# jhoobergs/Thesis-pbrt-v3

Measured on AMD Instinct MI355X. Metric: Mrays/s, higher is better.
Workload: dtype f32; 1 GPU; Sponza-class atrium STAND-IN (311,728 tris, matte+plastic, point light; the reference ships no Sponza geometry) 700x700, halton 1024 spp, path maxdepth 5, bvh; spp_total=1024, tiles=16x16 round-robin over 1 GPU(s), parallelism=tile-dp1, film_merge=none (single GPU)

## Files before the change

### thesis-pbrt-v3_amd/__init__.py

```python
import ctypes as C
import os

import numpy as np

_HERE = os.path.dirname(os.path.abspath(__file__))
LIB_PATH = os.environ.get("HPRT_LIB") or os.path.join(_HERE, "lib", "libhprt.so")


class HprtError(RuntimeError):
    def __init__(self, code, msg):
        super().__init__("hprt error %d: %s" % (code, msg))
        self.code = code


E_INVALID, E_IO, E_PARSE, E_NO_DEVICE, E_DEVICE, E_UNSUPPORTED = -1, -2, -3, -4, -5, -6
RENDER_COUNT_WORK = 1
RENDER_PIXEL_STATS = 2
RENDER_COUNT_TRACED = 4
RENDER_TRACE_ALL = 8
RENDER_EXPORT_FOREIGN = 16
ACCEL_BVH, ACCEL_KDTREE, ACCEL_RBSP = 0, 1, 2
ACCEL_BSP = ACCEL_RBSP
KD_MAX_DEPTH = 64
RBSP_MAX_DEPTH = 64
# ... 247 lines not shown
        "hprt_scene_reserve": (C.c_int, [vp, P(RenderDesc)]),
        "hprt_film_records_read": (C.c_int, [vp, vp, sz, P(sz)]),
        "hprt_film_records_merge": (C.c_int, [vp, sz, vp, sz]),
        "hprt_model_accelerator": (C.c_int, [vp, vp, sz]),
        "hprt_kdtree_build": (C.c_int, [vp, P(vp)]),
        "hprt_kdtree_build_from_bounds": (C.c_int, [sz, vp, vp, C.c_int, C.c_int, C.c_float, C.c_int, C.c_int, P(vp)]),
        "hprt_kdtree_info": (C.c_int, [vp, P(u32)]),
        "hprt_kdtree_copy": (C.c_int, [vp, vp, vp]),
        "hprt_kdtree_destroy": (None, [vp]),
        "hprt_scene_attach_kdtree": (C.c_int, [vp, vp]),
        "hprt_kdinst_build": (C.c_int, [vp, P(vp)]),
        "hprt_kdinst_info": (C.c_int, [vp, P(u32)]),
        "hprt_kdinst_object_info": (C.c_int, [vp, u32, P(u32)]),
        "hprt_kdinst_copy": (C.c_int, [vp, vp, vp]),
        "hprt_kdinst_object_copy": (C.c_int, [vp, u32, vp, vp]),
        "hprt_kdinst_destroy": (None, [vp]),
        "hprt_scene_attach_kdinst": (C.c_int, [vp, vp]),
        "hprt_write_pixel_stats_accel": (C.c_int, [cp, vp, C.c_int, C.c_int, C.c_int]),
        "hprt_rbsp_build": (C.c_int, [vp, vp, P(vp)]),
        "hprt_rbsp_build_from_triangles": (C.c_int, [sz, vp, vp, P(vp)]),
        "hprt_rbsp_info": (C.c_int, [vp, P(u32)]),
        "hprt_rbsp_copy": (C.c_int, [vp, vp, vp, vp]),
        "hprt_rbsp_destroy": (None, [vp]),
        "hprt_scene_attach_rbsp": (C.c_int, [vp, vp]),
        "hprt_rbspkd_build": (C.c_int, [vp, vp, P(vp)]),
        "hprt_rbspkd_build_from_triangles": (C.c_int, [sz, vp, vp, P(vp)]),
        "hprt_rbspkd_info": (C.c_int, [vp, P(u32)]),
        "hprt_rbspkd_copy": (C.c_int, [vp, vp, vp, vp]),
        "hprt_rbspkd_destroy": (None, [vp]),
        "hprt_scene_attach_rbspkd": (C.c_int, [vp, vp]),
        "hprt_rbspinst_build": (C.c_int, [vp, vp, P(vp)]),
        "hprt_rbspkdinst_build": (C.c_int, [vp, vp, P(vp)]),
        "hprt_rbspinst_info": (C.c_int, [vp, P(u32)]),
        "hprt_rbspinst_object_info": (C.c_int, [vp, u32, P(u32)]),
        "hprt_rbspinst_copy": (C.c_int, [vp, vp, vp, vp]),
        "hprt_rbspinst_object_copy": (C.c_int, [vp, u32, vp, vp]),
        "hprt_rbspinst_destroy": (None, [vp]),
        "hprt_scene_attach_rbspinst": (C.c_int, [vp, vp]),
        "hprt_rbsp_build_device": (C.c_int, [vp, vp, vp, vp, P(vp)]),
        "hprt_rbsp_build_from_triangles_device": (C.c_int, [sz, vp, vp, vp, vp, P(vp)]),
        "hprt_rbspkd_build_device": (C.c_int, [vp, vp, vp, vp, P(vp)]),
        "hprt_rbspkd_build_from_triangles_device": (C.c_int, [sz, vp, vp, vp, vp, P(vp)]),
        "hprt_bsppaper_build_device": (C.c_int, [vp, vp, vp, vp, P(vp)]),
        "hprt_bsppaper_build_from_triangles_device": (C.c_int, [sz, vp, vp, vp, vp, P(vp)]),
        "hprt_bsppaperkd_build_device": (C.c_int, [vp, vp, vp, vp, P(vp)]),
        "hprt_bsppaperkd_build_from_triangles_device": (C.c_int, [sz, vp, vp, vp, vp, P(vp)]),
        "hprt_bsppaper_build": (C.c_int, [vp, vp, P(vp)]),
        "hprt_bsppaper_build_from_triangles": (C.c_int, [sz, vp, vp, P(vp)]),
        "hprt_bsppaper_info": (C.c_int, [vp, P(u32)]),
        "hprt_bsppaper_copy": (C.c_int, [vp, vp, vp]),
        "hprt_bsppaper_destroy": (None, [vp]),
        "hprt_scene_attach_bsppaper": (C.c_int, [vp, vp]),
        "hprt_bsppaperkd_build": (C.c_int, [vp, vp, P(vp)]),
        "hprt_bsppaperkd_build_from_triangles": (C.c_int, [sz, vp, vp, P(vp)]),
        "hprt_bsppaperkd_info": (C.c_int, [vp, P(u32)]),
        "hprt_bsppaperkd_copy": (C.c_int, [vp, vp, vp]),
        "hprt_bsppaperkd_destroy": (None, [vp]),
        "hprt_scene_attach_bsppaperkd": (C.c_int, [vp, vp]),
        "hprt_bsppaperinst_build": (C.c_int, [vp, vp, P(vp)]),
        "hprt_bsppaperkdinst_build": (C.c_int, [vp, vp, P(vp)]),
        "hprt_bsppaperinst_info": (C.c_int, [vp, P(u32)]),
        "hprt_bsppaperinst_object_info": (C.c_int, [vp, u32, P(u32)]),
        "hprt_bsppaperinst_copy": (C.c_int, [vp, vp, vp]),
        "hprt_bsppaperinst_object_copy": (C.c_int, [vp, u32, vp, vp]),
        "hprt_bsppaperinst_destroy": (None, [vp]),
        "hprt_scene_attach_bsppaperinst": (C.c_int, [vp, vp]),
        "hprt_bspnode_build": (C.c_int, [vp, vp, P(vp)]),
        "hprt_bspnode_build_from_triangles": (C.c_int, [sz, vp, vp, P(vp)]),
        "hprt_bspnodekd_build": (C.c_int, [vp, vp, P(vp)]),
        "hprt_bspnodekd_build_from_triangles": (C.c_int, [sz, vp, vp, P(vp)]),
        "hprt_bspnode_build_device": (C.c_int, [vp, vp, vp, vp, P(vp)]),
        "hprt_bspnode_build_from_triangles_device": (C.c_int, [sz, vp, vp, vp, vp, P(vp)]),
        "hprt_bspnodekd_build_device": (C.c_int, [vp, vp, vp, vp, P(vp)]),
        "hprt_bspnodekd_build_from_triangles_device": (C.c_int, [sz, vp, vp, vp, vp, P(vp)]),
        "hprt_scene_kd_counters": (C.c_int, [vp, vp]),
        "hprt_pixel_kd_stats_read": (C.c_int, [vp, vp, sz]),
        "hprt_write_pixel_stats_rbspkd": (C.c_int, [cp, vp, vp, C.c_int, C.c_int]),
    }
    debug = {}
    for prefix in ("kdinst", "rbspinst", "bsppaperinst"):
        debug["hprt_debug_%s_bounds" % prefix] = (C.c_int, [vp, C.c_int, vp])
        debug["hprt_debug_%s_set_tree" % prefix] = (C.c_int, [vp, C.c_int, sz, vp, sz, vp, vp])
    debug["hprt_debug_halton_index"] = (C.c_int, [P(RenderOptions), sz, vp, vp, vp, vp, vp, vp])
    for name, (res, args) in list(sig.items()) + list(debug.items()):
        fn = getattr(lib, name)
        fn.restype = res
        fn.argtypes = args
    return lib, sorted(sig)


lib, EXPORTS = _load()


def _check(rc):
    if rc != 0:
        raise HprtError(rc, lib.hprt_last_error().decode("utf-8", "replace"))


def _ptr(a):
    return None if a is None else a.ctypes.data_as(C.c_void_p)


def version():
    return lib.hprt_version().decode()


_probe_lib = None


def _probe():
    global _probe_lib
    if _probe_lib is None:
        path = os.path.join(os.path.dirname(LIB_PATH), "libhprt_probe.so")
        if not os.path.exists(path):
            raise ImportError("hprt: %s is missing — run `python thesis-pbrt-v3_amd/build.py`" % path)
        p = C.CDLL(path)
        p.hprt_debug_device_halton.restype = C.c_int
        p.hprt_debug_device_halton.argtypes = [C.c_void_p, C.c_int, C.c_int, C.c_int, C.c_int, C.c_size_t, C.c_void_p, C.c_void_p, C.c_void_p]
        _probe_lib = p
    return _probe_lib


def debug_halton_index(opt, px, py, sample):
    px = np.ascontiguousarray(px, np.int32); py = np.ascontiguousarray(py, np.int32); sample = np.ascontiguousarray(sample, np.int64)
    a = np.zeros(px.shape[0], np.uint64); b = np.zeros(px.shape[0], np.uint64); bounds = np.zeros(4, np.int32)
    _check(lib.hprt_debug_halton_index(C.byref(opt), px.shape[0], _ptr(px), _ptr(py), _ptr(sample), _ptr(a), _ptr(b), _ptr(bounds)))
    return a, b, tuple(int(v) for v in bounds)


class Model:

    def __init__(self, handle):
        self._h = handle

    @staticmethod
    def parse(path, subst=None):
        kv = []
        for k, v in (subst or {}).items():
            kv += [k.encode(), v.encode()]
        arr = (C.c_char_p * max(1, len(kv)))(*kv)
        h = C.c_void_p()
        _check(lib.hprt_model_parse(path.encode(), arr, len(kv) // 2, C.byref(h)))
        return Model(h)

    @staticmethod
    def load(path):
        h = C.c_void_p()
        _check(lib.hprt_model_load(path.encode(), C.byref(h)))
        return Model(h)

    def save(self, path, compact=False):
        _check((lib.hprt_model_save_compact if compact else lib.hprt_model_save)(self._h, path.encode()))

    @property
    def options(self):
        o = RenderOptions()
        _check(lib.hprt_model_get_options(self._h, C.byref(o)))
        return o

    @options.setter
    def options(self, o):
        _check(lib.hprt_model_set_options(self._h, C.byref(o)))

    def counts(self):
        c = (C.c_uint64 * 7)()
        _check(lib.hprt_model_counts(self._h, c))
        return dict(zip(("shapes", "primitives", "triangles", "spheres", "materials", "lights", "textures"), [int(x) for x in c]))

    def texture(self, index):
        info = (C.c_int32 * 5)(); ma = C.c_float()
        _check(lib.hprt_model_texture_info(self._h, index, info, C.byref(ma)))
        levels = []
        for k in range(info[0]):
            wh = (C.c_int32 * 2)()
            _check(lib.hprt_model_texture_level(self._h, index, k, wh, None))
            a = np.zeros((wh[1], wh[0], 3), np.float32)
            _check(lib.hprt_model_texture_level(self._h, index, k, wh, _ptr(a)))
            levels.append(a)
        return {"levels": info[0], "trilinear": bool(info[1]), "wrap": info[2], "max_anisotropy": ma.value}, levels

    @property
    def accelerator(self):
        buf = C.create_string_buffer(256)
        _check(lib.hprt_model_accelerator(self._h, buf, 256))
        return buf.value.decode()

    def warnings(self):
        w = lib.hprt_model_warnings(self._h).decode()
        return [x for x in w.split("\n") if x]

    def __del__(self):
        if getattr(self, "_h", None) and lib is not None:
            lib.hprt_model_destroy(self._h)
            self._h = None


class Bvh:

    def __init__(self, model=None, handle=None):
        if handle is None:
            handle = C.c_void_p()
            _check(lib.hprt_bvh_build(model._h, C.byref(handle)))
        self._h = handle
# ... 387 lines not shown
    return (BspNodeKd if fastkd else BspNode)(model, accelerator, **kw), ("attach_bsppaperkd" if fastkd else "attach_bsppaper")


class Scene:

    def __init__(self, model, bvh, device=-1):
        h = C.c_void_p()
        _check(lib.hprt_scene_create_from_model(model._h, bvh._h, device, C.byref(h)))
        self._h = h
        self._model = model

    @staticmethod
    def from_desc(desc, device=-1):
        h = C.c_void_p()
        _check(lib.hprt_scene_create(C.byref(desc), device, C.byref(h)))
        sc = Scene.__new__(Scene)
        sc._h = h
        sc._model = None
        return sc

    def attach_kdtree(self, kdtree):
        _check(lib.hprt_scene_attach_kdtree(self._h, kdtree._h))
        self._kdtree = kdtree

    def attach_kdinst(self, kdinst):
        _check(lib.hprt_scene_attach_kdinst(self._h, kdinst._h))
        self._kdinst = kdinst

    def attach_rbspinst(self, rbspinst):
        _check(lib.hprt_scene_attach_rbspinst(self._h, rbspinst._h))
        self._rbspinst = rbspinst

    def attach_bsppaperinst(self, bsppaperinst):
        _check(lib.hprt_scene_attach_bsppaperinst(self._h, bsppaperinst._h))
        self._bsppaperinst = bsppaperinst

    def attach_rbsp(self, rbsp):
        _check(lib.hprt_scene_attach_rbsp(self._h, rbsp._h))
        self._rbsp = rbsp

    def attach_rbspkd(self, rbspkd):
        _check(lib.hprt_scene_attach_rbspkd(self._h, rbspkd._h))
        self._rbspkd = rbspkd

    def attach_bsppaper(self, bsppaper):
        _check(lib.hprt_scene_attach_bsppaper(self._h, bsppaper._h))
        self._bsppaper = bsppaper

    def attach_bsppaperkd(self, bsppaperkd):
        _check(lib.hprt_scene_attach_bsppaperkd(self._h, bsppaperkd._h))
        self._bsppaperkd = bsppaperkd

    def kd_counters(self):
        out = np.zeros(2, np.uint64)
        _check(lib.hprt_scene_kd_counters(self._h, _ptr(out)))
        return int(out[0]), int(out[1])

    def intersect(self, o, d, tmax, count=False):
        o = np.ascontiguousarray(o, np.float32); d = np.ascontiguousarray(d, np.float32)
        tmax = np.ascontiguousarray(tmax, np.float32)
        n = tmax.shape[0]
        t = np.zeros(n, np.float32); prim = np.zeros(n, np.int32); bary = np.zeros((n, 3), np.float32)
        ctr = np.zeros(4, np.uint64) if count else None
        _check(lib.hprt_intersect(self._h, n, _ptr(o), _ptr(d), _ptr(tmax), _ptr(t), _ptr(prim), _ptr(bary), _ptr(ctr)))
        return (t, prim, bary, ctr) if count else (t, prim, bary)

    def intersect_instanced(self, o, d, tmax, count=False):
        o = np.ascontiguousarray(o, np.float32); d = np.ascontiguousarray(d, np.float32)
        tmax = np.ascontiguousarray(tmax, np.float32)
        n = tmax.shape[0]
        t = np.zeros(n, np.float32); prim = np.zeros(n, np.int32); inst = np.zeros(n, np.int32); bary = np.zeros((n, 3), np.float32)
        ctr = np.zeros(4, np.uint64) if count else None
        _check(lib.hprt_intersect_instanced(self._h, n, _ptr(o), _ptr(d), _ptr(tmax), _ptr(t), _ptr(prim), _ptr(inst), _ptr(bary), _ptr(ctr)))
        return (t, prim, inst, bary, ctr) if count else (t, prim, inst, bary)

    def occluded(self, o, d, tmax, count=False):
        o = np.ascontiguousarray(o, np.float32); d = np.ascontiguousarray(d, np.float32)
        tmax = np.ascontiguousarray(tmax, np.float32)
        n = tmax.shape[0]
        occ = np.zeros(n, np.uint8)
        ctr = np.zeros(4, np.uint64) if count else None
        _check(lib.hprt_occluded(self._h, n, _ptr(o), _ptr(d), _ptr(tmax), _ptr(occ), _ptr(ctr)))
        return (occ, ctr) if count else occ

    def intersect_device(self, n, rays7_ptr, t_ptr, prim_ptr, bary_ptr=None, stream=None):
        _check(lib.hprt_intersect_device(self._h, n, rays7_ptr, t_ptr, prim_ptr, bary_ptr, stream))

    def occluded_device(self, n, rays7_ptr, occ_ptr, stream=None):
        _check(lib.hprt_occluded_device(self._h, n, rays7_ptr, occ_ptr, stream))

    def render(self, opt=None, tile_begin=0, tile_end=0, tile_stride=1, spp_chunk=0, count_work=False, film_ptr=None,
               stream=None, pixel_stats=False, count_traced=False, trace_all=False, export_foreign=False):
        opt = opt or self._model.options
        desc = RenderDesc()
        desc.opt = opt
        desc.tile_begin, desc.tile_end, desc.tile_stride = tile_begin, tile_end, tile_stride
        desc.spp_chunk = spp_chunk
        desc.flags = (RENDER_COUNT_WORK if count_work else 0) | (RENDER_PIXEL_STATS if pixel_stats else 0) | \
                     (RENDER_COUNT_TRACED if count_traced else 0) | (RENDER_TRACE_ALL if trace_all else 0) | \
                     (RENDER_EXPORT_FOREIGN if export_foreign else 0)
        self._film_shape = tuple(int(v) for v in (opt.film_bounds()[3] - opt.film_bounds()[1], opt.film_bounds()[2] - opt.film_bounds()[0]))
        st = RenderStats()
        _check(lib.hprt_render(self._h, C.byref(desc), film_ptr, stream, C.byref(st)))
        film = None
        if film_ptr is None:
            x0, y0, x1, y1 = opt.film_bounds()
            film = np.zeros((y1 - y0, x1 - x0, 4), np.float32)
            _check(lib.hprt_film_read(self._h, _ptr(film), film.shape[0] * film.shape[1]))
        return film, st.as_dict()

    def reserve(self, opt=None, tile_begin=0, tile_end=0, tile_stride=1, spp_chunk=0):
        desc = RenderDesc()
        desc.opt = opt or self._model.options
        desc.tile_begin, desc.tile_end, desc.tile_stride, desc.spp_chunk, desc.flags = tile_begin, tile_end, tile_stride, spp_chunk, 0
        _check(lib.hprt_scene_reserve(self._h, C.byref(desc)))

    def debug_poison(self, byte):
        lib.hprt_debug_poison_workspace.argtypes = [C.c_void_p, C.c_int]
        _check(lib.hprt_debug_poison_workspace(self._h, -1 if byte is None else int(byte)))

    def debug_device_halton(self, bounds_w, bounds_h, index, dim, sample_pixel_center=False, use_lds=False):
        index = np.ascontiguousarray(index, np.uint64); dim = np.ascontiguousarray(dim, np.int32)
        assert index.shape == dim.shape and index.ndim == 1
        out = np.zeros(index.shape[0], np.float32)
        _check(_probe().hprt_debug_device_halton(self._h, int(bounds_w), int(bounds_h), int(bool(sample_pixel_center)), int(bool(use_lds)),
                                                 index.shape[0], _ptr(index), _ptr(dim), _ptr(out)))
        return out

    def film_records(self):
        n = C.c_size_t()
        _check(lib.hprt_film_records_read(self._h, None, 0, C.byref(n)))
        out = np.zeros(n.value, FILM_RECORD)
        if n.value:
            _check(lib.hprt_film_records_read(self._h, _ptr(out), n.value, C.byref(n)))
        return out

    def pixel_stats(self):
        h, w = self._film_shape
        out = np.zeros((h, w, 7), np.uint64)
        _check(lib.hprt_pixel_stats_read(self._h, _ptr(out), h * w))
        return out

    def pixel_kd_stats(self):
        h, w = self._film_shape
        out = np.zeros((2, h, w), np.uint64)
        _check(lib.hprt_pixel_kd_stats_read(self._h, _ptr(out), h * w))
        return out

    def sample_radiance(self, px, py, sample, opt=None):
        opt = opt or self._model.options
        px = np.ascontiguousarray(px, np.int32); py = np.ascontiguousarray(py, np.int32)
        sample = np.ascontiguousarray(sample, np.int64)
        L = np.zeros((px.shape[0], 3), np.float32)
        _check(lib.hprt_sample_radiance(self._h, C.byref(opt), px.shape[0], _ptr(px), _ptr(py), _ptr(sample), _ptr(L)))
        return L

    def __del__(self):
        if getattr(self, "_h", None) and lib is not None:
            lib.hprt_scene_destroy(self._h)
            self._h = None


class Comm:

    @staticmethod
    def unique_id():
# ... 77 lines not shown
```

### thesis-pbrt-v3_amd/build.py

```python
import concurrent.futures
import os
import shutil
import subprocess
import sys

HERE = os.path.dirname(os.path.abspath(__file__))
CSRC = os.path.join(HERE, "csrc")
OBJ = os.path.join(HERE, "build")
LIB = os.path.join(HERE, "lib")
HOST_SRCS = ["pbrt_frontend.cpp", "loop_subdiv.cpp", "scene_io.cpp", "texture_io.cpp", "bvh_builder.cpp", "kdtree_builder.cpp", "rbsp_builder.cpp", "bsppaper_builder.cpp", "bspnode_builder.cpp", "bvhold_builder.cpp", "wide_bvh.cpp", "halton_tables.cpp", "capi_host.cpp"]
HIPCC_HOST_SRCS = ["scene_layout.cpp"]
HIP_SRCS = ["device/kernels.hip", "device/kd_walk.hip", "device/rbsp_walk.hip", "device/rbspkd_walk.hip", "device/bsppaper_walk.hip", "device/bsppaperkd_walk.hip", "device/kdinst_walk.hip", "device/kdop_cost.hip", "device/rbspinst_walk.hip", "device/bsppaperinst_walk.hip", "device/bsp_cost.hip", "device/bspnode_cost.hip", "device/hlbvh_build.hip", "capi_device.hip", "capi_gather.hip"]
CUIDS = {"device/kernels.hip": "a6cd736c50efffab", "device/kd_walk.hip": "5c0d2e7f41b3a916", "device/rbsp_walk.hip": "3e91a5c07d2b84f6",
         "device/rbspkd_walk.hip": "7a4f0c2e9b61d385", "device/bsppaper_walk.hip": "c52e8b1d06f3a794",
         "device/bsppaperkd_walk.hip": "e8136d4a9f07c2b5", "device/kdinst_walk.hip": "4d9b27f1a60c8e53", "device/kdop_cost.hip": "b7e20a5c93d1f468",
         "device/rbspinst_walk.hip": "9f3c61d8b2047ae5", "device/bsppaperinst_walk.hip": "2c7e5a90d4b18f63", "device/bsp_cost.hip": "6b1f94c3e7a0d258",
         "device/bspnode_cost.hip": "d3a7150c8e4f92b6", "device/hlbvh_build.hip": "58e2c9a4f1b7063d",
         "capi_device.hip": "1b24418c11488d5c", "capi_gather.hip": "89501e8167866ce2"}
PROBE_SRCS = ["device/halton_probe.hip"]
CUIDS["device/halton_probe.hip"] = "f04b8d61c2a79e35"
COMMON = ["-O3", "-std=c++17", "-fPIC", "-ffp-contract=off", "-fno-fast-math", "-Wall", "-Wno-unused-function"]


def _hipcc():
    for c in (shutil.which("hipcc"), "/opt/rocm/bin/hipcc"):
        if c and os.path.exists(c):
            return c
    raise RuntimeError("hipcc not found")


def _newer(src_files, out):
    if not os.path.exists(out):
        return True
    t = os.path.getmtime(out)
    return any(os.path.getmtime(f) > t for f in src_files)


def _headers():
    hs = []
    for root, _, files in os.walk(CSRC):
        hs += [os.path.join(root, f) for f in files if f.endswith(".h")]
    hs.append(os.path.join(HERE, "..", "include", "hprt.h"))
    return hs


def build(verbose=False, force=False):
    os.makedirs(OBJ, exist_ok=True)
    os.makedirs(LIB, exist_ok=True)
    hipcc = _hipcc()
    headers = _headers()
    jobs = []
    for s in HOST_SRCS + HIPCC_HOST_SRCS:
        src = os.path.join(CSRC, s)
        obj = os.path.join(OBJ, s.replace("/", "_") + ".o")
        cmd = [hipcc if s in HIPCC_HOST_SRCS else "g++"] + COMMON + ["-c", src, "-o", obj]
        jobs.append((src, obj, cmd))
    for s in HIP_SRCS + PROBE_SRCS:
        src = os.path.join(CSRC, s)
        obj = os.path.join(OBJ, s.replace("/", "_") + ".o")
        cmd = [hipcc, "--offload-arch=gfx950"] + COMMON + ["-Wno-unused-result", "-cuid=" + CUIDS[s], "-c", src, "-o", obj]
        jobs.append((src, obj, cmd))

    def run(job):
        src, obj, cmd = job
        if not force and not _newer([src, os.path.abspath(__file__)] + headers, obj):
            return None
        r = subprocess.run(cmd, capture_output=True, text=True)
        if r.returncode != 0:
            raise RuntimeError("compile failed: %s\n%s\n%s" % (" ".join(cmd), r.stdout, r.stderr))
        return r.stderr

    with concurrent.futures.ThreadPoolExecutor(max_workers=4) as ex:
        for out in ex.map(run, jobs):
            if verbose and out:
                print(out)
    lib = os.path.join(LIB, "libhprt.so")
    probe_objs = [j[1] for j in jobs[len(jobs) - len(PROBE_SRCS):]]
    objs = [j[1] for j in jobs[:len(jobs) - len(PROBE_SRCS)]]
    if force or _newer(objs, lib):
        cmd = [hipcc, "--offload-arch=gfx950", "-shared", "-o", lib] + objs + ["-lz", "-L/opt/rocm/lib", "-lrccl"]
        r = subprocess.run(cmd, capture_output=True, text=True)
        if r.returncode != 0:
            raise RuntimeError("link failed: %s\n%s" % (" ".join(cmd), r.stderr))
    probe = os.path.join(LIB, "libhprt_probe.so")
    if force or _newer(probe_objs + [lib], probe):
        cmd = [hipcc, "--offload-arch=gfx950", "-shared", "-o", probe] + probe_objs + ["-L" + LIB, "-lhprt", "-Wl,-rpath,$ORIGIN"]
        r = subprocess.run(cmd, capture_output=True, text=True)
        if r.returncode != 0:
            raise RuntimeError("link failed: %s\n%s" % (" ".join(cmd), r.stderr))
    return lib


if __name__ == "__main__":
    print(build(verbose="-v" in sys.argv, force="-f" in sys.argv))
```

### thesis-pbrt-v3_amd/csrc/capi_device.hip

```cpp
#include <hip/hip_runtime.h>
#include <algorithm>
#include <cassert>
#include <chrono>
#include <cmath>
#include <cstring>
#include <functional>
#include <map>
#include <memory>
#include <string>
#include <vector>
#include "../../include/hprt.h"
#include "device/kernels.h"
#include "halton_tables.h"
#include "host_transform.h"
#include "hprt_internal.h"
#include "device_state.h"
#include "scene_layout.h"
#include "wide_bvh.h"

using namespace hprt;


namespace {

// ... 59 lines not shown
    cam->dxCamera = xf_point(cam->rasterToCamera, vec3(1, 0, 0)) - xf_point(cam->rasterToCamera, vec3(0, 0, 0));
    cam->dyCamera = xf_point(cam->rasterToCamera, vec3(0, 1, 0)) - xf_point(cam->rasterToCamera, vec3(0, 0, 0));
}

int CheckDepth(int maxDepth) {
    if (5 + 8 * ((int64_t)maxDepth + 1) > 1000)
        return SetError(HPRT_E_UNSUPPORTED, "maxdepth above 123: a path could pass the 1,000 sampler dimensions of the reference's Halton tables");
    return HPRT_OK;
}

struct FrameSetup {
    FilmGeom fg; int ntx, nty; HaltonLayout hal; RenderParams rp;
    std::vector<uint32_t> pixelXY; std::vector<uint64_t> pixelOffset;
    std::vector<int32_t> localIndex;
    int W, H;
    uint64_t offX[128], offY[128];
};
int SetupFrame(const HprtRenderOptions &o, FrameSetup *f) {
    if (o.xres <= 0 || o.yres <= 0 || o.xres > 32768 || o.yres > 32768) return SetError(HPRT_E_INVALID, "film resolution out of range");
    if (o.filter_radius[0] != 0.5f || o.filter_radius[1] != 0.5f)
        return SetError(HPRT_E_UNSUPPORTED, "only the box filter with radius 0.5 is in the hot-path scope (SURVEY.md §2)");
    FilmGeom &fg = f->fg;
    fg.cx0 = (int)std::ceil(o.xres * o.crop[0]); fg.cx1 = (int)std::ceil(o.xres * o.crop[1]);
    fg.cy0 = (int)std::ceil(o.yres * o.crop[2]); fg.cy1 = (int)std::ceil(o.yres * o.crop[3]);
    fg.rx = o.filter_radius[0]; fg.ry = o.filter_radius[1];
    fg.sx0 = (int)std::floor((float)fg.cx0 + 0.5f - fg.rx); fg.sy0 = (int)std::floor((float)fg.cy0 + 0.5f - fg.ry);
    fg.sx1 = (int)std::ceil((float)fg.cx1 - 0.5f + fg.rx); fg.sy1 = (int)std::ceil((float)fg.cy1 - 0.5f + fg.ry);
    fg.maxSampleLuminance = o.max_sample_luminance;
    f->W = fg.cx1 - fg.cx0; f->H = fg.cy1 - fg.cy0;
    if (f->W <= 0 || f->H <= 0) return SetError(HPRT_E_INVALID, "empty crop window");
    f->ntx = (fg.sx1 - fg.sx0 + 15) / 16; f->nty = (fg.sy1 - fg.sy0 + 15) / 16;
    f->hal = MakeHaltonLayout(fg.sx1 - fg.sx0, fg.sy1 - fg.sy0);
    const uint64_t base = (uint64_t)HaltonPixelOffset(f->hal, 0, 0), stride = (uint64_t)std::max(1, f->hal.sampleStride);
    for (int m = 0; m < 128; ++m) {
        f->offX[m] = (uint64_t)HaltonPixelOffset(f->hal, m, 0);
        f->offY[m] = ((uint64_t)HaltonPixelOffset(f->hal, 0, m) + stride - base) % stride;
    }
    return HPRT_OK;
}
uint64_t TilePixelOffset(const FrameSetup &f, int x, int y) {
    const uint64_t stride = (uint64_t)std::max(1, f.hal.sampleStride);
    return f.hal.sampleStride > 1 ? (f.offX[((x % 128) + 128) % 128] + f.offY[((y % 128) + 128) % 128]) % stride : 0ull;
}
void AddTilePixels(FrameSetup *f, int tile) {
    const FilmGeom &fg = f->fg;
    int tx = tile % f->ntx, ty = tile / f->ntx;
    int x0 = fg.sx0 + tx * 16, x1 = std::min(x0 + 16, fg.sx1), y0 = fg.sy0 + ty * 16, y1 = std::min(y0 + 16, fg.sy1);
    for (int y = y0; y < y1; ++y)
        for (int x = x0; x < x1; ++x) {
            f->localIndex[(size_t)(y - fg.cy0) * f->W + (x - fg.cx0)] = (int32_t)f->pixelXY.size();
            f->pixelXY.push_back((uint32_t)x | ((uint32_t)y << 16));
            f->pixelOffset.push_back(TilePixelOffset(*f, x, y));
        }
}

}

extern "C" {

int hprt_scene_create(const HprtSceneDesc *d, int device, HprtScene **out) try {
    if (!d || !out) return SetError(HPRT_E_INVALID, "hprt_scene_create: null argument");
    SceneLayout L;
    if (int rc = BuildSceneLayout(*d, &L)) return rc;
    int dev;
    if (int rc = CheckDevice(device, &dev)) return rc;
    std::unique_ptr<HprtScene> sc(new HprtScene());
    sc->device = dev; sc->nPrims = L.nPrims;
    sc->topOrder = std::move(L.topOrder); sc->objectOrder = std::move(L.objectOrder); sc->objectPrimBase = std::move(L.objectPrimBase);
    sc->instanceObject = std::move(L.instanceObject); sc->instanced = L.instanced; sc->hasSubstrateBin = L.hasSubstrateBin;
    const std::vector<uint16_t> &perms = HaltonPermutations();
    std::vector<int32_t> primes(PrimeTable().begin(), PrimeTable().end()), primeSums(PrimeSumTable().begin(), PrimeSumTable().end());
    std::vector<uint64_t> magic(primes.size());
    for (size_t i = 0; i < primes.size(); ++i) magic[i] = 0xffffffffffffffffull / (uint64_t)primes[i] + 1ull;
    HIP_TRY(upload(sc->nodes, L.pairs)); HIP_TRY(upload(sc->tris, L.tris)); HIP_TRY(upload(sc->primVtx, L.primVtx));
    HIP_TRY(upload(sc->primN, L.primN)); HIP_TRY(upload(sc->vUV, L.vUV)); HIP_TRY(upload(sc->vS, L.vS));
    HIP_TRY(upload(sc->shapes, L.shapes)); HIP_TRY(upload(sc->materials, L.materials)); HIP_TRY(upload(sc->lights, L.lights));
    HIP_TRY(upload(sc->spheres, L.spheres)); HIP_TRY(upload(sc->instances, L.instances)); HIP_TRY(upload(sc->topEntry, L.topEntry));
    HIP_TRY(upload(sc->topEntryWide, L.topEntryWide)); HIP_TRY(upload(sc->lightFunc, L.lightFunc)); HIP_TRY(upload(sc->lightCdf, L.lightCdf));
    HIP_TRY(upload(sc->perms, perms)); HIP_TRY(upload(sc->primes, primes)); HIP_TRY(upload(sc->primeSums, primeSums));
    HIP_TRY(upload(sc->primeMagic, magic));
    HIP_TRY(upload(sc->textures, L.textures)); HIP_TRY(upload(sc->mipLevels, L.mipLevels)); HIP_TRY(upload(sc->texels, L.texels)); HIP_TRY(upload(sc->weightLut, L.weightLut));
    HIP_TRY(upload(sc->wide, L.wide)); HIP_TRY(upload(sc->leafBox, L.leafBox));
    HIP_TRY(upload(sc->envLights, L.envLights)); HIP_TRY(upload(sc->envData, L.envData));
    HIP_TRY(sc->counters.alloc(sizeof(DevCounters)));
    HIP_TRY(hipMemset(sc->counters.p, 0, sizeof(DevCounters)));
    HIP_TRY(sc->deepStack.alloc((size_t)HPRT_SPILL_STACK * HPRT_DEEP_THREADS * sizeof(uint2)));
    HIP_TRY(sc->workCounter.alloc(256));
    DevScene &dv = sc->dev;
    dv.pairs = sc->nodes.as<DevPair>(); dv.nPairs = (uint32_t)L.pairs.size();
    dv.wide = L.wide.empty() ? nullptr : sc->wide.as<DevWide>(); dv.nWide = (uint32_t)L.wide.size(); dv.leafBox = sc->leafBox.as<float4>();
    dv.tris = sc->tris.as<float4>(); dv.nPrims = L.nPrims;
    dv.primVtx = sc->primVtx.as<uint32_t>();
    dv.primN = sc->primN.as<float4>(); dv.vUV = sc->vUV.as<float>(); dv.vS = sc->vS.as<float>();
    dv.shapes = sc->shapes.as<DevShape>(); dv.nShapes = d->n_shapes;
    dv.materials = sc->materials.as<DevMaterial>();
    dv.lights = sc->lights.as<DevLight>(); dv.nLights = d->n_lights;
    dv.spheres = sc->spheres.as<DevSphere>(); dv.nSpheres = (uint32_t)L.spheres.size();
    dv.envLights = sc->envLights.as<DevEnvLight>(); dv.envData = sc->envData.as<float>(); dv.nEnvLights = (uint32_t)L.envLights.size();
    dv.textures = d->n_textures ? sc->textures.as<DevTexture>() : nullptr; dv.mipLevels = sc->mipLevels.as<DevMipLevel>();
    dv.texels = sc->texels.as<float>(); dv.weightLut = sc->weightLut.as<float>();
    dv.instances = sc->instances.as<DevInstance>(); dv.nInstances = d->n_instances;
    dv.topEntry = L.topEntry.empty() ? nullptr : sc->topEntry.as<float4>(); dv.nTopPrims = (uint32_t)L.topEntry.size();
    dv.topEntryWide = L.topEntryWide.empty() ? nullptr : sc->topEntryWide.as<float4>();
    dv.lightFunc = sc->lightFunc.as<float>(); dv.lightCdf = sc->lightCdf.as<float>(); dv.lightFuncInt = L.funcInt;
    dv.deepStack = sc->deepStack.as<uint2>();
    dv.perms = sc->perms.as<uint16_t>(); dv.primes = sc->primes.as<int32_t>(); dv.primeSums = sc->primeSums.as<int32_t>();
    dv.primeMagic = sc->primeMagic.as<uint64_t>();
    dv.worldRadius = L.worldRadius;
    dv.spatial = 0; dv.voxFunc = dv.voxCdf = dv.voxFuncInt = nullptr;
    dv.voxSlot = nullptr; dv.voxRequest = nullptr; dv.voxRequestCount = nullptr;
    for (int a = 0; a < 3; ++a) { dv.voxN[a] = L.voxN[a]; dv.wbMin[a] = L.wbMin[a]; dv.wbMax[a] = L.wbMax[a]; }
    if (L.lightStrategy == 2) {
        const uint64_t nVox = (uint64_t)dv.voxN[0] * (uint64_t)dv.voxN[1] * (uint64_t)dv.voxN[2];
        const uint64_t denseMaxFloats = [] { const char *e = getenv("HPRT_VOXEL_DENSE_MAX_MB"); return e ? (uint64_t)atoll(e) * (1ull << 18) : (1ull << 28); }();
        const uint64_t rowFloats = 2ull * d->n_lights + 2ull;
        const bool dense = nVox * rowFloats <= denseMaxFloats;
        uint64_t rows = nVox;
        if (!dense) {
            const uint64_t poolFloats = [] { const char *e = getenv("HPRT_VOXEL_POOL_MB"); return (e ? (uint64_t)atoll(e) : 4096ull) * (1ull << 18); }();
            rows = std::max<uint64_t>(1, std::min<uint64_t>(nVox, poolFloats / rowFloats));
        }
        HIP_TRY(sc->voxFunc.alloc(rows * d->n_lights * sizeof(float)));
        HIP_TRY(sc->voxCdf.alloc(rows * (d->n_lights + 1ull) * sizeof(float)));
        HIP_TRY(sc->voxFuncInt.alloc(rows * sizeof(float)));
        std::vector<float> ri(5 * 128);
        VoxelSamplePoints(ri.data());
        HIP_TRY(upload(sc->voxRi, ri));
        dv.spatial = 1;
        dv.voxFunc = sc->voxFunc.as<float>(); dv.voxCdf = sc->voxCdf.as<float>(); dv.voxFuncInt = sc->voxFuncInt.as<float>();
        sc->nVoxels = (uint32_t)nVox; sc->voxRows = (uint32_t)rows; sc->voxRowsUsed = 0;
        if (dense) LaunchVoxelDistributions(nullptr, dv, sc->voxRi.as<float>(), (uint32_t)nVox, sc->voxFunc.as<float>(), sc->voxCdf.as<float>(), sc->voxFuncInt.as<float>());
        else {
            HIP_TRY(sc->voxSlot.alloc(nVox * sizeof(int32_t)));
            HIP_TRY(hipMemset(sc->voxSlot.p, 0xff, nVox * sizeof(int32_t)));
            HIP_TRY(sc->voxRequest.alloc(nVox * sizeof(uint32_t)));
            HIP_TRY(sc->voxRequestCount.alloc(256));
            HIP_TRY(hipMemset(sc->voxRequestCount.p, 0, 256));
            dv.voxSlot = sc->voxSlot.as<int32_t>(); dv.voxRequest = sc->voxRequest.as<uint32_t>(); dv.voxRequestCount = sc->voxRequestCount.as<uint32_t>();
        }
        HIP_TRY(hipGetLastError());
        HIP_TRY(hipDeviceSynchronize());
    }
    HIP_TRY(hipHostMalloc((void **)&sc->hostCounts, (4096 + 256) * sizeof(uint32_t)));
    *out = sc.release();
    return HPRT_OK;
} catch (...) { return hprt::HandleException(); }

__attribute__((visibility("default"))) int hprt_debug_scene_walk(HprtScene *s) { return s && s->walk == HprtScene::Walk::Bvh && hprt::WideWalkInUse(s->dev) ? 1 : 0; }
__attribute__((visibility("default"))) int hprt_debug_shade_counts(HprtScene *s, int on, uint64_t *out2) {
    if (!s) return HPRT_E_INVALID;
    if (out2) { out2[0] = s->shadeDeferred; out2[1] = s->shadeRetried; }
    if (on && !s->shadeCountsOn) s->shadeDeferred = s->shadeRetried = s->shadeSpeculated = s->shadeRepaired = s->shadeFull = 0;
    s->shadeCountsOn = on != 0;
    return HPRT_OK;
}
__attribute__((visibility("default"))) int hprt_debug_speculated_counts(HprtScene *s, uint64_t *out3) {
    if (!s || !out3) return HPRT_E_INVALID;
    out3[0] = s->shadeSpeculated; out3[1] = s->shadeRepaired; out3[2] = s->shadeFull;
    return HPRT_OK;
}
static int g_speculateLight = -1;
static bool SpeculateLightEnabled() {
    static const bool fromEnv = [] { const char *e = getenv("HPRT_SPECULATE_LIGHT"); return !(e && atoi(e) == 0); }();
    return g_speculateLight < 0 ? fromEnv : g_speculateLight != 0;
}
__attribute__((visibility("default"))) int hprt_debug_speculate_light(int on) { const int was = SpeculateLightEnabled() ? 1 : 0; g_speculateLight = on; return was; }
static int g_foldRepair = -1;
static bool FoldRepairEnabled() {
    static const bool fromEnv = [] { const char *e = getenv("HPRT_FOLD_REPAIR"); return !(e && atoi(e) == 0); }();
    return g_foldRepair < 0 ? fromEnv : g_foldRepair != 0;
}
__attribute__((visibility("default"))) int hprt_debug_fold_repair(int on) { const int was = FoldRepairEnabled() ? 1 : 0; g_foldRepair = on; return was; }
__attribute__((visibility("default"))) int hprt_debug_poison_workspace(HprtScene *s, int byte) { if (!s) return HPRT_E_INVALID; s->poisonByte = byte < 0 ? -1 : (byte & 255); return HPRT_OK; }
__attribute__((visibility("default"))) int hprt_debug_capture_rays(HprtScene *s, int bounce, int kind, float *d_out7, size_t cap) {
    if (!s || kind < 0 || kind > 2 || cap > 0x7fffffffull) return HPRT_E_INVALID;
    s->capture.bounce = bounce; s->capture.kind = kind; s->capture.out7 = d_out7; s->capture.cap = cap; s->capture.n = 0;
    return HPRT_OK;
}
static int ApiStreams(HprtScene *s, size_t n, RayStream *rays, HitStream *hits);
static bool CountsKdShare(const HprtScene *s) {
    return s->walk == HprtScene::Walk::RbspKd || s->walk == HprtScene::Walk::BspPaperKd || s->walk == HprtScene::Walk::RbspKdInst ||
           s->walk == HprtScene::Walk::BspPaperKdInst;
}
static void Trace(HprtScene *s, hipStream_t st, bool anyHit, bool count, const uint32_t *queue, const uint32_t *countPtr, uint32_t countImm,
                  uint32_t gridItems, const RayStream &rays, const HitStream &hits, uint8_t *occ, DevCounters *counters, uint32_t *workCounter,
                  uint4 *rayStats = nullptr) {
    switch (s->walk) {
    case HprtScene::Walk::Kd: LaunchKdTrace(st, s->dev, s->kd, anyHit, count, queue, countPtr, countImm, gridItems, rays, hits, occ, counters, workCounter, rayStats); break;
    case HprtScene::Walk::Rbsp: LaunchRbspTrace(st, s->dev, s->rbsp, anyHit, count, queue, countPtr, countImm, gridItems, rays, hits, occ, counters, workCounter, rayStats); break;
    case HprtScene::Walk::RbspKd:
        LaunchRbspKdTrace(st, s->dev, DevRbspKd{s->rbsp, s->kdShare.as<unsigned long long>()}, anyHit, count, queue, countPtr, countImm, gridItems, rays,
                          hits, occ, counters, workCounter, rayStats);
        break;
    case HprtScene::Walk::BspPaper:
        LaunchBspPaperTrace(st, s->dev, s->bsppaper, anyHit, count, queue, countPtr, countImm, gridItems, rays, hits, occ, counters, workCounter, rayStats);
        break;
    case HprtScene::Walk::BspPaperKd:
        LaunchBspPaperKdTrace(st, s->dev, DevBspPaperKd{s->bsppaper, s->kdShare.as<unsigned long long>()}, anyHit, count, queue, countPtr, countImm,
                              gridItems, rays, hits, occ, counters, workCounter, rayStats);
        break;
    case HprtScene::Walk::KdInst:
        LaunchKdInstTrace(st, s->dev, s->kdinst, anyHit, count, queue, countPtr, countImm, gridItems, rays, hits, occ, counters, workCounter, rayStats);
        break;
    case HprtScene::Walk::RbspInst:
    case HprtScene::Walk::RbspKdInst:
        LaunchRbspInstTrace(st, s->dev, s->rbspinst, s->walk == HprtScene::Walk::RbspKdInst, anyHit, count, queue, countPtr, countImm, gridItems, rays, hits, occ,
                            counters, workCounter, rayStats);
        break;
    case HprtScene::Walk::BspPaperInst:
    case HprtScene::Walk::BspPaperKdInst:
        LaunchBspPaperInstTrace(st, s->dev, s->bsppaperinst, s->walk == HprtScene::Walk::BspPaperKdInst, anyHit, count, queue, countPtr, countImm, gridItems, rays,
                                hits, occ, counters, workCounter, rayStats);
        break;
    case HprtScene::Walk::Bvh: LaunchTrace(st, s->dev, anyHit, count, queue, countPtr, countImm, gridItems, rays, hits, occ, counters, workCounter, rayStats); break;
    }
}
__attribute__((visibility("default"))) int hprt_debug_trace_queued(HprtScene *s, size_t n, const float *d_rays7, const uint32_t *d_queue, int anyHit,
                                                                    float *d_scratch7, float ms[2]) try {
    if (!s || !d_rays7 || !d_queue || !d_scratch7 || !ms || n == 0 || n > 0x7ffffff0ull) return SetError(HPRT_E_INVALID, "hprt_debug_trace_queued: bad argument");
    HIP_TRY(hipSetDevice(s->device));
    SceneCall call(s, nullptr);
    RayStream rays; HitStream hits;
    if (int rc = ApiStreams(s, n, &rays, &hits)) return rc;
    DevBuf occ; HIP_TRY(occ.alloc(n));
    hipEvent_t e[3];
    for (auto &x : e) HIP_TRY(hipEventCreate(&x));
    LaunchPackRays(nullptr, d_rays7, (uint32_t)n, rays);
    HIP_TRY(hipEventRecord(e[0], nullptr));
    LaunchCaptureRays(nullptr, d_queue, (uint32_t)n, rays, d_scratch7, (uint32_t)n);
    HIP_TRY(hipEventRecord(e[1], nullptr));
    HitStream none; none.a = nullptr; none.b = nullptr;
    Trace(s, nullptr, anyHit != 0, false, d_queue, nullptr, (uint32_t)n, (uint32_t)n, rays, anyHit ? none : hits, anyHit ? occ.as<uint8_t>() : nullptr, nullptr, s->workCounter.as<uint32_t>());
    HIP_TRY(hipEventRecord(e[2], nullptr));
    HIP_TRY(hipDeviceSynchronize());
    HIP_TRY(hipEventElapsedTime(&ms[0], e[0], e[1])); HIP_TRY(hipEventElapsedTime(&ms[1], e[1], e[2]));
    for (auto &x : e) (void)hipEventDestroy(x);
    return HPRT_OK;
} catch (...) { return hprt::HandleException(); }
__attribute__((visibility("default"))) long long hprt_debug_captured(HprtScene *s) { return s ? (long long)s->capture.n : -1; }
__attribute__((visibility("default"))) int hprt_debug_stream_copy(int device, size_t bytes, int iters, double *best_gbs, double *mean_gbs) try {
    if (!best_gbs || !mean_gbs || iters < 1 || iters > 1000 || bytes < (1u << 20) || bytes > (64ull << 30)) return SetError(HPRT_E_INVALID, "hprt_debug_stream_copy: bad argument");
    int dev = 0;
    if (int rc = CheckDevice(device, &dev)) return rc;
    HIP_TRY(hipSetDevice(dev));
    DevBuf a, b;
    HIP_TRY(a.alloc(bytes)); HIP_TRY(b.alloc(bytes));
    HIP_TRY(hipMemset(a.p, 1, bytes)); HIP_TRY(hipMemset(b.p, 2, bytes));
    const size_t n = bytes / 16;
    hipEvent_t e0, e1;
    HIP_TRY(hipEventCreate(&e0)); HIP_TRY(hipEventCreate(&e1));
    LaunchStreamCopy(nullptr, a.as<float4>(), b.as<float4>(), n);
    HIP_TRY(hipDeviceSynchronize());
    double best = 0, sum = 0;
    for (int i = 0; i < iters; ++i) {
        HIP_TRY(hipEventRecord(e0, nullptr));
        LaunchStreamCopy(nullptr, a.as<float4>(), b.as<float4>(), n);
        HIP_TRY(hipEventRecord(e1, nullptr));
        HIP_TRY(hipEventSynchronize(e1));
        float ms = 0; HIP_TRY(hipEventElapsedTime(&ms, e0, e1));
        const double g = 2.0 * (double)(n * 16) / ((double)ms * 1e-3) / 1e9;
        best = std::max(best, g); sum += g;
    }
    (void)hipEventDestroy(e0); (void)hipEventDestroy(e1);
    *best_gbs = best; *mean_gbs = sum / iters;
    return HPRT_OK;
} catch (...) { return hprt::HandleException(); }
__attribute__((visibility("default"))) int hprt_debug_gather_probe(int device, int log2_records, int iters_per_lane, int launches, double *best_grecords_s, double *mean_grecords_s) try {
    if (!best_grecords_s || !mean_grecords_s || log2_records < 8 || log2_records > 26 || iters_per_lane < 1 || iters_per_lane > 100000 || launches < 1 || launches > 100)
        return SetError(HPRT_E_INVALID, "hprt_debug_gather_probe: bad argument");
    int dev = 0;
    if (int rc = CheckDevice(device, &dev)) return rc;
    HIP_TRY(hipSetDevice(dev));
    hipDeviceProp_t prop;
    HIP_TRY(hipGetDeviceProperties(&prop, dev));
    const uint32_t blocks = (uint32_t)prop.multiProcessorCount * 6u * 4u;
    DevBuf table, sink;
    const size_t bytes = (size_t)64 << log2_records;
    HIP_TRY(table.alloc(bytes)); HIP_TRY(sink.alloc(16));
    HIP_TRY(hipMemset(table.p, 0x5b, bytes));
    hipEvent_t e0, e1;
    HIP_TRY(hipEventCreate(&e0)); HIP_TRY(hipEventCreate(&e1));
    LaunchGatherProbe(nullptr, table.as<uint4>(), (uint32_t)log2_records, std::max(1, iters_per_lane / 10), blocks, sink.as<uint32_t>());
    HIP_TRY(hipDeviceSynchronize());
    double best = 0, sum = 0;
    for (int i = 0; i < launches; ++i) {
        HIP_TRY(hipEventRecord(e0, nullptr));
        LaunchGatherProbe(nullptr, table.as<uint4>(), (uint32_t)log2_records, iters_per_lane, blocks, sink.as<uint32_t>());
        HIP_TRY(hipEventRecord(e1, nullptr));
        HIP_TRY(hipEventSynchronize(e1));
        float ms = 0; HIP_TRY(hipEventElapsedTime(&ms, e0, e1));
        const double g = (double)blocks * 256.0 * (double)iters_per_lane / ((double)ms * 1e-3) / 1e9;
        best = std::max(best, g); sum += g;
    }
    (void)hipEventDestroy(e0); (void)hipEventDestroy(e1);
    *best_grecords_s = best; *mean_grecords_s = sum / launches;
    return HPRT_OK;
} catch (...) { return hprt::HandleException(); }

__global__ void k_debug_math(int fn, const float *x, const float *y, size_t n, double *o0, double *o1) {
// ... 417 lines not shown
int RunBatch(HprtScene *s, hipStream_t st, const RenderParams &rpIn, const Workspace &w, const QueueSet &qa, const QueueSet &qb,
             const BinSet &bins, uint32_t s0, uint32_t nSlots, bool count, EventTimer &ev, BatchTimers *bt, HprtRenderStats *stats,
             uint32_t *pixelStats = nullptr, const IrregularSink *irregular = nullptr) {
    uint4 *rayStats = pixelStats ? s->rayStats.as<uint4>() : nullptr;
    RenderParams rp = rpIn;
    rp.speculate = SpeculateLightEnabled() && !pixelStats && !rayStats && nSlots <= SPEC_MAX_PATHS ? 1 : 0;
    assert(!rp.speculate || nSlots <= SPEC_MAX_PATHS);
    rp.foldRepair = rp.speculate && FoldRepairEnabled() && !s->shadeCountsOn ? 1 : 0;
    uint32_t *specCounts = rp.speculate && s->shadeCountsOn ? s->queueCounts.as<uint32_t>() + kSpecCountsAt : nullptr;
    if (specCounts) HIP_TRY(hipMemsetAsync(specCounts, 0, 2 * sizeof(uint32_t), st));
    uint32_t *pixelKd = pixelStats && CountsKdShare(s) ? s->pixelKdLocal.as<uint32_t>() : nullptr;
    uint32_t *wcPath = s->workCounter.as<uint32_t>();
    LaunchGenerate(st, s->dev, rp, w.path[0], s0, nSlots, irregular);
    const uint32_t *activeQ = nullptr; uint32_t active = nSlots;
    QueueSet q[2] = {qa, qb};
    DevCounters *ctr = s->counters.as<DevCounters>();
    std::vector<std::pair<hipEvent_t, hipEvent_t>> evExt, evOcc;
    auto tracePath = [&](int bounce) -> int {
        const PathStream &in = w.path[bounce & 1];
        hipEvent_t e0 = ev.get(), e1 = ev.get();
        HIP_TRY(hipEventRecord(e0, st));
        Trace(s, st, false, count, activeQ, nullptr, active, active, in.ray, w.hit, nullptr, ctr, wcPath, rayStats);
        if (pixelStats) LaunchPixelStats(st, rayStats, bounce == 0 ? nullptr : in.beta, activeQ, nullptr, active, active, rp.nPix, false, pixelStats);
        if (pixelKd) LaunchPixelKdStats(st, rayStats, bounce == 0 ? nullptr : in.beta, activeQ, nullptr, active, active, rp.nPix, false, pixelKd);
        HIP_TRY(hipEventRecord(e1, st));
        evExt.push_back({e0, e1}); bt->extendRays += active; ++bt->extendLaunches;
        stats->rays += active;
        return HPRT_OK;
    };
    if (active > 0) { int rc = tracePath(0); if (rc != HPRT_OK) return rc; }
    for (int bounce = 0; active > 0; ++bounce) {
        const QueueSet &cur = q[bounce & 1];
        const PathStream &in = w.path[bounce & 1], &out = w.path[(bounce + 1) & 1];
        VertexStreams vs = w.vs;
        vs.pendBeta = w.pend[bounce & 1]; vs.pendPrev = w.pend[(bounce + 1) & 1];
        HIP_TRY(hipMemsetAsync(cur.nextCount, 0, 256 * sizeof(uint32_t), st));
        HIP_TRY(hipMemsetAsync(bins.count, 0, 8 * BIN_STRIDE * sizeof(uint32_t), st));
        LaunchBin(st, s->dev, in, w.hit, activeQ, nullptr, active, active, rp.maxDepth, bounce, bins, w.Lfinal, vs, rp.foldRepair != 0);
        HIP_TRY(hipMemcpyAsync(bins.count + 5 * BIN_STRIDE, bins.count + 2 * BIN_STRIDE, sizeof(uint32_t), hipMemcpyDeviceToDevice, st));
        static const int order[5] = {BIN_MATTE, BIN_PLASTIC, BIN_SUBSTRATE, BIN_GENERIC, BIN_TEXTURED};
        for (int k = 0; k < (s->dev.textures ? 5 : 4); ++k) {
            const int mode = order[k];
            if (mode == (int)BIN_SUBSTRATE && !s->hasSubstrateBin) continue;
            LaunchShade(st, mode, s->dev, rp, in, w.hit, active, s0, out, vs, cur, bins, w.Lfinal, bounce == 0);
        }
        HIP_TRY(hipMemcpyAsync(s->hostCounts + 4096, cur.nextCount, 256 * sizeof(uint32_t), hipMemcpyDeviceToHost, st));
        if (s->shadeCountsOn) {
            HIP_TRY(hipMemcpyAsync(s->hostCounts + 12, bins.count + 2 * BIN_STRIDE, sizeof(uint32_t), hipMemcpyDeviceToHost, st));
            HIP_TRY(hipMemcpyAsync(s->hostCounts + 13, bins.count + 5 * BIN_STRIDE, sizeof(uint32_t), hipMemcpyDeviceToHost, st));
        }
        if (s->dev.voxSlot) {
            HIP_TRY(hipMemcpyAsync(s->hostCounts + 16, bins.count + 6 * BIN_STRIDE, 2 * BIN_STRIDE * sizeof(uint32_t), hipMemcpyDeviceToHost, st));
            HIP_TRY(hipMemcpyAsync(s->hostCounts + 15, s->dev.voxRequestCount, sizeof(uint32_t), hipMemcpyDeviceToHost, st));
            HIP_TRY(hipStreamSynchronize(st));
            const uint32_t nRetry[2] = {s->hostCounts[16], s->hostCounts[16 + BIN_STRIDE]}, nReq = s->hostCounts[15];
            if (s->shadeCountsOn) s->shadeRetried += (uint64_t)nRetry[0] + nRetry[1];
            if (nRetry[0] + nRetry[1] > 0) {
                if ((uint64_t)s->voxRowsUsed + nReq > s->voxRows)
                    return SetError(HPRT_E_UNSUPPORTED, "spatial light distribution: the paths touch more voxels than the row pool holds (" + std::to_string(s->voxRows) +
                                                        " rows of " + std::to_string(s->dev.nLights) + " lights; HPRT_VOXEL_POOL_MB raises it, or use \"power\" / \"uniform\")");
                LaunchVoxelFill(st, s->dev, s->voxRi.as<float>(), nReq, s->voxRowsUsed, s->voxFunc.as<float>(), s->voxCdf.as<float>(), s->voxFuncInt.as<float>());
                s->voxRowsUsed += nReq;
                HIP_TRY(hipMemsetAsync(s->dev.voxRequestCount, 0, sizeof(uint32_t), st));
                for (int r = 0; r < 2; ++r)
                    if (nRetry[r]) LaunchShade(st, 2 + r, s->dev, rp, in, w.hit, nRetry[r], s0, out, vs, cur, bins, w.Lfinal, bounce == 0, true);
                HIP_TRY(hipMemcpyAsync(s->hostCounts + 4096, cur.nextCount, 256 * sizeof(uint32_t), hipMemcpyDeviceToHost, st));
            }
        }
        HIP_TRY(hipStreamSynchronize(st));
        if (s->shadeCountsOn) s->shadeDeferred += s->hostCounts[12] - s->hostCounts[13];
        const uint32_t nNext = s->hostCounts[4096], nShadow = s->hostCounts[4096 + 64], nMis = s->hostCounts[4096 + 128], nResolve = s->hostCounts[4096 + 192];
        const uint32_t nEnd = s->hostCounts[4096 + 32];
        if (s->capture.out7 && s->capture.bounce == bounce && s0 == 0) {
            const uint32_t *cq = s->capture.kind == 0 ? cur.next : s->capture.kind == 1 ? cur.shadow : cur.mis;
            const uint32_t cn = s->capture.kind == 0 ? nNext : s->capture.kind == 1 ? nShadow : nMis;
            const RayStream &cs = s->capture.kind == 0 ? out.ray : s->capture.kind == 1 ? vs.shadow : vs.mis;
            LaunchCaptureRays(st, cq, cn, cs, s->capture.out7, (uint32_t)s->capture.cap);
            s->capture.n = std::min<size_t>(cn, s->capture.cap);
        }
        if (nShadow) {
            hipEvent_t a = ev.get(), b = ev.get();
            HIP_TRY(hipEventRecord(a, st));
            HitStream none; none.a = nullptr; none.b = nullptr;
            Trace(s, st, true, count, cur.shadow, nullptr, nShadow, nShadow, vs.shadow, none, vs.occluded, ctr, wcPath, rayStats);
            if (pixelStats) LaunchPixelStats(st, rayStats, vs.pendBeta, cur.shadow, nullptr, nShadow, nShadow, rp.nPix, true, pixelStats);
            if (pixelKd) LaunchPixelKdStats(st, rayStats, vs.pendBeta, cur.shadow, nullptr, nShadow, nShadow, rp.nPix, true, pixelKd);
            HIP_TRY(hipEventRecord(b, st));
            evOcc.push_back({a, b}); bt->occludedRays += nShadow; ++bt->occludedLaunches;
            stats->shadow_rays += nShadow;
        }
        if (nMis) {
            hipEvent_t a = ev.get(), b = ev.get();
            HIP_TRY(hipEventRecord(a, st));
            Trace(s, st, false, count, cur.mis, nullptr, nMis, nMis, vs.mis, vs.misHit, nullptr, ctr, wcPath, rayStats);
            if (pixelStats) LaunchPixelStats(st, rayStats, vs.pendBeta, cur.mis, nullptr, nMis, nMis, rp.nPix, false, pixelStats);
            if (pixelKd) LaunchPixelKdStats(st, rayStats, vs.pendBeta, cur.mis, nullptr, nMis, nMis, rp.nPix, false, pixelKd);
            HIP_TRY(hipEventRecord(b, st));
            evExt.push_back({a, b}); bt->extendRays += nMis; ++bt->extendLaunches;
            stats->rays += nMis;
        }
        activeQ = cur.next; active = nNext;
        if (active > 0 && bounce > rp.maxDepth) return SetError(HPRT_E_DEVICE, "internal error: paths are still active beyond maxdepth");
        if (nResolve) LaunchResolve(st, s->dev, vs, out.L, w.Lfinal, cur.resolve, cur.resolveCount, nResolve);
        if (rp.foldRepair) { if (nEnd) LaunchRepair(st, vs, out.L, w.Lfinal, cur.end, nEnd, nullptr); }
        else if (rp.speculate && nShadow) LaunchRepair(st, vs, out.L, w.Lfinal, cur.shadow, nShadow, specCounts);
        if (s->shadeCountsOn) s->shadeFull += nResolve;
        if (active > 0) { int rc = tracePath(bounce + 1); if (rc != HPRT_OK) return rc; }
    }
    HIP_TRY(hipGetLastError());
    if (specCounts) HIP_TRY(hipMemcpyAsync(s->hostCounts + 256, specCounts, 2 * sizeof(uint32_t), hipMemcpyDeviceToHost, st));
    HIP_TRY(hipStreamSynchronize(st));
    if (specCounts) { s->shadeSpeculated += s->hostCounts[256]; s->shadeRepaired += s->hostCounts[257]; }
    for (auto &p : evExt) { float ms = 0; if (hipEventElapsedTime(&ms, p.first, p.second) == hipSuccess) bt->extendMs += ms; }
    for (auto &p : evOcc) { float ms = 0; if (hipEventElapsedTime(&ms, p.first, p.second) == hipSuccess) bt->occludedMs += ms; }
    ev.reset();
    return HPRT_OK;
}

constexpr size_t kQueueWordsPerSlot = 10 + 1 + 2 * N_BINS;
int EnsureWorkspace(HprtScene *s, size_t nSlots, Workspace *ps, QueueSet *qa, QueueSet *qb, BinSet *bins) {
    const bool instances = s->dev.nInstances != 0u;
    HIP_TRY(s->planes.alloc(PlaneBytes(nSlots, instances)));
    CarvePlanes(s->planes.as<char>(), nSlots, instances, ps);
    HIP_TRY(s->queues.alloc(kQueueWordsPerSlot * nSlots * sizeof(uint32_t) + 4096));
    HIP_TRY(s->queueCounts.alloc(2048 * sizeof(uint32_t)));
    uint32_t *qbase = s->queues.as<uint32_t>(), *cbase = s->queueCounts.as<uint32_t>();
    QueueSet *qs[2] = {qa, qb};
    for (int k = 0; k < 2; ++k) {
        qs[k]->next = qbase + (5 * k + 0) * nSlots; qs[k]->shadow = qbase + (5 * k + 1) * nSlots;
        qs[k]->mis = qbase + (5 * k + 2) * nSlots; qs[k]->resolve = qbase + (5 * k + 3) * nSlots; qs[k]->end = qbase + (5 * k + 4) * nSlots;
        qs[k]->nextCount = cbase + 256 * k; qs[k]->shadowCount = cbase + 256 * k + 64; qs[k]->misCount = cbase + 256 * k + 128; qs[k]->resolveCount = cbase + 256 * k + 192;
        qs[k]->endCount = cbase + 256 * k + 32;
    }
    bins->aux = qbase + 10 * nSlots;
    for (int k = 0; k < (int)N_BINS; ++k) bins->q[k] = reinterpret_cast<uint2 *>(qbase + (11 + 2 * k) * nSlots + (nSlots & 1u));
    bins->count = cbase + 512;
    bins->retry[0] = bins->retry[1] = nullptr;
    if (s->dev.voxSlot) {
        HIP_TRY(s->retryQueues.alloc(2 * nSlots * sizeof(uint2) + 256));
        bins->retry[0] = s->retryQueues.as<uint2>(); bins->retry[1] = bins->retry[0] + nSlots;
    }
    return HPRT_OK;
}

int PoisonWorkspace(HprtScene *s) {
    if (s->poisonByte < 0) return HPRT_OK;
    hprt::DevBuf *bufs[] = {&s->planes, &s->queues, &s->Lall, &s->deepStack, &s->rayStats, &s->irregular};
    for (hprt::DevBuf *b : bufs) if (b->p && b->bytes) HIP_TRY(hipMemset(b->p, s->poisonByte, b->bytes));
    HIP_TRY(hipDeviceSynchronize());
    return HPRT_OK;
}

int ChooseBatch(HprtScene *s, int32_t sppChunk, uint32_t nPix, uint32_t spp, uint32_t *out) {
    uint32_t chunk;
    if (sppChunk > 0) chunk = (uint32_t)sppChunk;
    else {
        size_t freeB = 0, totalB = 0;
        HIP_TRY(hipMemGetInfo(&freeB, &totalB));
        freeB += s->planes.bytes + s->queues.bytes;
        const size_t perPath = PlaneBytesPerSlot(s->dev.nInstances != 0u) + kQueueWordsPerSlot * sizeof(uint32_t);
        static const size_t capM = [] { const char *e = getenv("HPRT_BATCH_MPATHS"); return e ? (size_t)atoi(e) : (size_t)256; }();
        const size_t budget = std::min<size_t>(capM << 20, std::max<size_t>(freeB / 2 / perPath, 1ull << 20));
        chunk = std::max<uint32_t>(1u, (uint32_t)(budget / std::max<uint32_t>(nPix, 1u)));
        if ((uint64_t)chunk * nPix > 0x7fffffffull) chunk = (uint32_t)(0x7fffffffull / nPix);
        chunk = std::max(1u, std::min(chunk, spp));
        const uint32_t nBatches = (spp + chunk - 1) / chunk;
        chunk = (spp + nBatches - 1) / nBatches;
// ... 327 lines not shown
```

### thesis-pbrt-v3_amd/csrc/capi_host.cpp

```cpp
#include <algorithm>
#include <new>
#include <stdexcept>
#include <cmath>
#include <limits>
#include <vector>
#include <cstdio>
#include <cstring>
#include <map>
#include <memory>
#include <string>
#include <type_traits>
#include "../../include/hprt.h"
#include "bsp_cost_device.h"
#include "bspnode_cost_device.h"
#include "bspnode_builder.h"
#include "bvh_builder.h"
#include "halton_tables.h"
#include "hlbvh_build_device.h"
#include "hprt_internal.h"
#include "kdop_cost_device.h"
#include "scene_model.h"
#include "hprt_math.h"
#include "wide_bvh.h"

using namespace hprt;

namespace hprt {
thread_local std::string g_lastError;
int SetError(int code, const std::string &msg) { g_lastError = msg; return code; }
int HandleException() {
    try { throw; }
    catch (const std::bad_alloc &) { return SetError(HPRT_E_INVALID, "out of memory (or a size in the input that cannot be real)"); }
    catch (const std::length_error &e) { return SetError(HPRT_E_INVALID, std::string("a size in the input cannot be real: ") + e.what()); }
    catch (const std::exception &e) { return SetError(HPRT_E_INVALID, std::string("unexpected exception: ") + e.what()); }
    catch (...) { return SetError(HPRT_E_INVALID, "unexpected exception"); }
}
}

namespace {

void RbspModelPrims(const HprtModel *m, std::vector<float> *lo, std::vector<float> *hi, std::vector<float> *tri9, std::vector<uint8_t> *isTri) {
    ComputePrimBounds(m->sc, {}, lo, hi);
    const size_t n = lo->size() / 3;
    tri9->assign(9 * n, 0.f);
    isTri->assign(n, 0);
    size_t k = 0;
    for (const TopItem &ti : m->sc.top) {
        const ShapeDesc &sh = m->sc.shapes[ti.index];
        if (sh.kind != kTriangleMesh) { ++k; continue; }
        const MeshData &md = sh.mesh;
        for (uint32_t tr = 0; tr < md.nTris(); ++tr, ++k) {
            for (int v = 0; v < 3; ++v) memcpy(&(*tri9)[9 * k + 3 * v], &md.P[3 * (size_t)md.indices[3 * tr + v]], 12);
            (*isTri)[k] = 1;
        }
    }
}
void RbspTriangleBounds(size_t n, const float *p9, std::vector<float> *lo, std::vector<float> *hi) {
    lo->resize(3 * n); hi->resize(3 * n);
    for (size_t i = 0; i < n; ++i)
        for (int d = 0; d < 3; ++d) {
            const float a = p9[9 * i + d], b = p9[9 * i + 3 + d], c = p9[9 * i + 6 + d];
            const float l = std::min(a, b), h = std::max(a, b);
            (*lo)[3 * i + d] = std::min(l, c); (*hi)[3 * i + d] = std::max(h, c);
        }
}
template <typename Opts, typename Sink>
struct BuildHook {
    bool device = false;
    const Opts *opts = nullptr;
    HprtBuildDeviceStats *stats = nullptr;
    Sink sink = nullptr; void *user = nullptr; uint32_t maxNodes = 0;
};
constexpr uint32_t kDeviceMinCandidates = 1024;
struct HookState { BuildDeviceStats bs; int rc = HPRT_OK; uint32_t seen = 0; };
template <typename Request, typename Hook, typename Open, typename Cost, typename Emit>
int InstallHook(const Hook *hook, CostHook<Request> *p, HookState *st, Open open, Cost cost, Emit emit) {
    if (hook && hook->device) {
        if (hook->stats) *hook->stats = HprtBuildDeviceStats{0, 0, 0, 0, 0.0};
        if (const int rc = open()) return rc;
        p->costMinCandidates = hook->opts && hook->opts->min_candidates ? hook->opts->min_candidates : kDeviceMinCandidates;
        p->stats = &st->bs;
        p->costFn = cost;
    } else if (hook && hook->sink) {
        p->costMinCandidates = 1;
        p->costFn = [=](const Request &rq, std::string *) -> int {
            if (st->seen >= hook->maxNodes) return 1;
            memset(rq.overflow, 1, rq.n);
            return 0;
        };
        p->costDone = [=](const Request &rq) { emit(st->seen++, rq); };
    }
    return HPRT_OK;
}
std::string TooDeepMessage(const std::string &what, uint32_t depth, uint32_t todoMax = 0) {
    std::string msg = what + " of depth " + std::to_string(depth) + " is deeper than the device walk's todo list";
    if (todoMax) msg += " (" + std::to_string(todoMax) + " entries); lower \"maxdepth\"";
    return msg;
}
template <typename Hook, typename Handle>
int FinishBuild(const Hook *hook, const HookState &st, const std::string &err, const char *what, uint32_t todoMax, std::unique_ptr<Handle> &t, Handle **out) {
    if (hook && hook->stats)
        *hook->stats = HprtBuildDeviceStats{st.bs.nodesDevice, st.bs.candidatesDevice, st.bs.candidatesRecosted, st.bs.nodesHost, st.bs.secondsDevice};
    if (st.rc != HPRT_OK) return SetError(st.rc, err);
    if (!err.empty()) return SetError(HPRT_E_UNSUPPORTED, err);
    if (t->tree.depth > todoMax) return SetError(HPRT_E_UNSUPPORTED, TooDeepMessage(what, t->tree.depth, todoMax));
    *out = t.release();
// ... 1622 lines not shown
        float *px = xyzw + 4 * (size_t)rec[i].dest_pixel;
        px[0] += rec[i].xyz[0]; px[1] += rec[i].xyz[1]; px[2] += rec[i].xyz[2]; px[3] += rec[i].weight;
    }
    return HPRT_OK;
} catch (...) { return hprt::HandleException(); }

__attribute__((visibility("default"))) int hprt_debug_host_selftest(int failures[2]) try {
    if (!failures) return HPRT_E_INVALID;
    const float inf = std::numeric_limits<float>::infinity();
    int f = 0;
    if (!(next_up(-0.f) > 0.f)) ++f;
    if (!(next_down(0.f) < 0.f)) ++f;
    if (!(next_up(inf) == inf)) ++f;
    if (!(next_down(inf) < inf)) ++f;
    if (!(next_down(-inf) == -inf)) ++f;
    if (!(next_up(-inf) > -inf)) ++f;
    uint64_t state = 0x853c49e6748fea9bULL; const uint64_t inc = 0xda3e39cb94b95bdbULL;
    auto next32 = [&]() {
        uint64_t old = state;
        state = old * 0x5851f42d4c957f2dULL + inc;
        uint32_t xs = (uint32_t)(((old >> 18u) ^ old) >> 27u), rot = (uint32_t)(old >> 59u);
        return (xs >> rot) | (xs << ((~rot + 1u) & 31));
    };
    for (int i = 0; i < 100000; ++i) {
        float v;
        do { v = u2f(next32()); } while (std::isnan(v));
        if (std::isinf(v)) continue;
        if (std::nextafter(v, inf) != next_up(v)) ++f;
        if (std::nextafter(v, -inf) != next_down(v)) ++f;
    }
    failures[0] = f;
    f = 0;
    const float func[4] = {0, 1.f, 0.f, 3.f};
    float cdf[5], funcInt;
    dist1d_build(func, 4, cdf, &funcInt);
    float pdf;
    const float us[7] = {0.f, 0.125f, .24999f, .250001f, 0.625f, 0x1.fffffep-1f, 1.f};
    const int want[7] = {1, 1, 1, 3, 3, 3, 3};
    for (int k = 0; k < 7; ++k) {
        if (dist1d_sample_discrete(cdf, func, funcInt, 4, us[k], &pdf) != want[k]) ++f;
        if (pdf != (want[k] == 1 ? 0.25f : 0.75f)) ++f;
    }
    float u = .25f, uMax = .25f;
    for (int i = 0; i < 20; ++i) { u = next_down(u); uMax = next_up(uMax); }
    for (; u < uMax; u = next_up(u)) {
        int interval = dist1d_sample_discrete(cdf, func, funcInt, 4, u, &pdf);
        if (interval == 3) break;
        if (interval != 1) ++f;
    }
    if (!(u < uMax)) ++f;
    for (; u <= uMax; u = next_up(u))
        if (dist1d_sample_discrete(cdf, func, funcInt, 4, u, &pdf) != 3) ++f;
    failures[1] = f;
    return HPRT_OK;
} catch (...) { return hprt::HandleException(); }

__attribute__((visibility("default"))) int hprt_debug_wide_build(const void *nodes32, uint32_t n_nodes, void *out64, size_t cap, size_t *n_out, int *stack_need) try {
    if (!nodes32 || !n_out || !stack_need) return SetError(HPRT_E_INVALID, "hprt_debug_wide_build: null argument");
    const BvhNode *nd = (const BvhNode *)nodes32;
    const char *bad = CheckBvhNodes(nd, n_nodes, UINT32_MAX, nullptr);
    if (*bad) return SetError(HPRT_E_INVALID, std::string("hprt_debug_wide_build: ") + bad);
    std::vector<int32_t> leafRef(n_nodes, WIDE_NONE);
    for (uint32_t i = 0; i < n_nodes; ++i)
        if ((nd[i].countAxis & 3u) == 3u) leafRef[i] = (int32_t)(~(uint32_t)nd[i].offset & ~WIDE_LEAF_BOXED);
    std::vector<DevWide> wide;
    if (!BuildWide(nd, n_nodes, leafRef.data(), &wide, stack_need)) return SetError(HPRT_E_UNSUPPORTED, "the tree does not fit the four-wide grid");
    *n_out = wide.size();
    if (out64 && cap >= wide.size()) memcpy(out64, wide.data(), wide.size() * sizeof(DevWide));
    return HPRT_OK;
} catch (...) { return hprt::HandleException(); }

__attribute__((visibility("default"))) int hprt_debug_shape_inline(const HprtSceneDesc *d, uint32_t *tags, uint32_t *prim_shape, size_t prim_cap, size_t *n_prims,
                                                                    uint32_t *shape_flags, int32_t *shape_material, size_t shape_cap, size_t *n_shapes) try {
    if (!d || !n_prims || !n_shapes) return SetError(HPRT_E_INVALID, "hprt_debug_shape_inline: null argument");
    std::vector<uint32_t> t, ps, sf;
    std::vector<int32_t> smat;
    if (int rc = LayoutTagsForDebug(*d, &t, &ps, &sf, &smat)) return rc;
    *n_prims = t.size(); *n_shapes = sf.size();
    if (tags && prim_shape && prim_cap >= t.size()) { memcpy(tags, t.data(), 4 * t.size()); memcpy(prim_shape, ps.data(), 4 * ps.size()); }
    if (shape_flags && shape_material && shape_cap >= sf.size()) { memcpy(shape_flags, sf.data(), 4 * sf.size()); memcpy(shape_material, smat.data(), 4 * smat.size()); }
    return HPRT_OK;
} catch (...) { return hprt::HandleException(); }

}
```

### thesis-pbrt-v3_amd/csrc/device/dev_intersect.h

```cpp
#pragma once
#include "dev_scene.h"

namespace hprt {

struct DRay { vec3 o, d; float tMax; };

struct RayShear { bool k0, k1; float Sx, Sy, Sz; };
__device__ __forceinline__ RayShear ray_shear(vec3 rd, vec3 invDir) {
    RayShear s;
    const int kz = max_dim(vabs(rd));
    int kx = kz + 1; if (kx == 3) kx = 0;
    int ky = kx + 1; if (ky == 3) ky = 0;
    const float dx = rd.get(kx), dy = rd.get(ky), dz = rd.get(kz);
    s.k0 = kz == 0; s.k1 = kz == 1;
    s.Sx = -dx / dz; s.Sy = -dy / dz; s.Sz = invDir.get(kz);
    return s;
}
__device__ __forceinline__ RayShear ray_shear(vec3 rd) {
    RayShear s;
    const int kz = max_dim(vabs(rd));
    int kx = kz + 1; if (kx == 3) kx = 0;
    int ky = kx + 1; if (ky == 3) ky = 0;
    const float dx = rd.get(kx), dy = rd.get(ky), dz = rd.get(kz);
    s.k0 = kz == 0; s.k1 = kz == 1;
    s.Sx = -dx / dz; s.Sy = -dy / dz; s.Sz = 1.f / dz;
    return s;
}
__device__ __forceinline__ vec3 permute3(vec3 v, bool k0, bool k1) {
    const float a = k1 ? v.z : v.x, b = k1 ? v.x : v.y, c = k1 ? v.y : v.z;
    return vec3(k0 ? v.y : a, k0 ? v.z : b, k0 ? v.x : c);
}
__device__ __forceinline__ bool tri_test(vec3 p0, vec3 p1, vec3 p2, vec3 rayO, float rayTMax, const RayShear &sh, float *b0o,
                                         float *b1o, float *b2o, float *to) {
    vec3 p0t = p0 - rayO, p1t = p1 - rayO, p2t = p2 - rayO;
    p0t = permute3(p0t, sh.k0, sh.k1);
    p1t = permute3(p1t, sh.k0, sh.k1);
    p2t = permute3(p2t, sh.k0, sh.k1);
    const float Sx = sh.Sx, Sy = sh.Sy, Sz = sh.Sz;
    p0t.x += Sx * p0t.z; p0t.y += Sy * p0t.z;
    p1t.x += Sx * p1t.z; p1t.y += Sy * p1t.z;
    p2t.x += Sx * p2t.z; p2t.y += Sy * p2t.z;
    float e0 = p1t.x * p2t.y - p1t.y * p2t.x;
    float e1 = p2t.x * p0t.y - p2t.y * p0t.x;
    float e2 = p0t.x * p1t.y - p0t.y * p1t.x;
    if (e0 == 0.0f || e1 == 0.0f || e2 == 0.0f) {
        double p2txp1ty = (double)p2t.x * (double)p1t.y;
        double p2typ1tx = (double)p2t.y * (double)p1t.x;
        e0 = (float)(p2typ1tx - p2txp1ty);
        double p0txp2ty = (double)p0t.x * (double)p2t.y;
        double p0typ2tx = (double)p0t.y * (double)p2t.x;
        e1 = (float)(p0typ2tx - p0txp2ty);
        double p1txp0ty = (double)p1t.x * (double)p0t.y;
        double p1typ0tx = (double)p1t.y * (double)p0t.x;
        e2 = (float)(p1typ0tx - p1txp0ty);
    }
    if ((e0 < 0 || e1 < 0 || e2 < 0) && (e0 > 0 || e1 > 0 || e2 > 0)) return false;
    float det = e0 + e1 + e2;
    if (det == 0) return false;
    p0t.z *= Sz; p1t.z *= Sz; p2t.z *= Sz;
    float tScaled = e0 * p0t.z + e1 * p1t.z + e2 * p2t.z;
    if (det < 0 && (tScaled >= 0 || tScaled < rayTMax * det)) return false;
    else if (det > 0 && (tScaled <= 0 || tScaled > rayTMax * det)) return false;
    float invDet = 1 / det;
    float b0 = e0 * invDet, b1 = e1 * invDet, b2 = e2 * invDet;
    float t = tScaled * invDet;
    float maxZt = max_comp(vabs(vec3(p0t.z, p1t.z, p2t.z)));
    float deltaZ = gamma_n(3) * maxZt;
    float maxXt = max_comp(vabs(vec3(p0t.x, p1t.x, p2t.x)));
    float maxYt = max_comp(vabs(vec3(p0t.y, p1t.y, p2t.y)));
    float deltaX = gamma_n(5) * (maxXt + maxZt);
    float deltaY = gamma_n(5) * (maxYt + maxZt);
    float deltaE = 2 * (gamma_n(2) * maxXt * maxYt + deltaY * maxXt + deltaX * maxYt);
    float maxE = max_comp(vabs(vec3(e0, e1, e2)));
    float deltaT = 3 * (gamma_n(3) * maxE * maxZt + deltaE * maxZt + deltaZ * maxE) * fabsf(invDet);
    if (t <= deltaT) return false;
    *b0o = b0; *b1o = b1; *b2o = b2; *to = t;
    return true;
}

struct efloat { float v, lo, hi; };
__device__ __forceinline__ efloat ef(float v) { efloat r; r.v = v; r.lo = v; r.hi = v; return r; }
__device__ __forceinline__ efloat ef(float v, float err) {
    efloat r; r.v = v;
    if (err == 0.f) { r.lo = v; r.hi = v; } else { r.lo = next_down(v - err); r.hi = next_up(v + err); }
    return r;
}
#ifdef HPRT_EF_INLINE
#define HPRT_EF_FN __device__ __forceinline__
#else
#define HPRT_EF_FN __device__ __noinline__
#endif
HPRT_EF_FN efloat ef_add(efloat a, efloat b) { efloat r; r.v = a.v + b.v; r.lo = next_down(a.lo + b.lo); r.hi = next_up(a.hi + b.hi); return r; }
HPRT_EF_FN efloat ef_sub(efloat a, efloat b) { efloat r; r.v = a.v - b.v; r.lo = next_down(a.lo - b.hi); r.hi = next_up(a.hi - b.lo); return r; }
HPRT_EF_FN efloat ef_mul(efloat a, efloat b) {
    efloat r; r.v = a.v * b.v;
    float p0 = a.lo * b.lo, p1 = a.hi * b.lo, p2 = a.lo * b.hi, p3 = a.hi * b.hi;
    r.lo = next_down(sel_min(sel_min(p0, p1), sel_min(p2, p3)));
    r.hi = next_up(sel_max(sel_max(p0, p1), sel_max(p2, p3)));
    return r;
}
HPRT_EF_FN efloat ef_div(efloat a, efloat b) {
    efloat r; r.v = a.v / b.v;
    if (b.lo < 0 && b.hi > 0) { r.lo = -HPRT_INF; r.hi = HPRT_INF; }
    else {
        float d0 = a.lo / b.lo, d1 = a.hi / b.lo, d2 = a.lo / b.hi, d3 = a.hi / b.hi;
        r.lo = next_down(sel_min(sel_min(d0, d1), sel_min(d2, d3)));
        r.hi = next_up(sel_max(sel_max(d0, d1), sel_max(d2, d3)));
    }
    return r;
}
__device__ __forceinline__ bool ef_quadratic(efloat A, efloat B, efloat C, efloat *t0, efloat *t1) {
    double discrim = (double)B.v * (double)B.v - 4. * (double)A.v * (double)C.v;
    if (discrim < 0.) return false;
    double rootDiscrim = sqrt(discrim);
    efloat fr = ef((float)rootDiscrim, (float)((double)HPRT_MACHINE_EPS * rootDiscrim));
    efloat q;
    if (B.v < 0) q = ef_mul(ef(-.5f), ef_sub(B, fr));
    else q = ef_mul(ef(-.5f), ef_add(B, fr));
    *t0 = ef_div(q, A);
    *t1 = ef_div(C, q);
    if (t0->v > t1->v) { efloat tmp = *t0; *t0 = *t1; *t1 = tmp; }
    return true;
}

__device__ __forceinline__ bool sphere_phi_exceeds(const DevSphere &s, vec3 pHit) {
    if (s.phiMax > 6.283f) {
        if (pHit.y >= 0.f) return false;
        if (pHit.x <= 0.f) return false;
        if (-pHit.y > 1e-3f * pHit.x) return false;
    }
    float phi = det_atan2f(pHit.y, pHit.x);
    if (phi < 0) phi += 2 * HPRT_PI;
    return phi > s.phiMax;
}

__device__ __forceinline__ bool sphere_may_hit(const DevSphere &s, const DRay &r) {
    vec3 oErr;
    vec3 o = xf_point_err(s.w2o, r.o, &oErr);
    const vec3 d = xf_vector(s.w2o, r.d);
    const float len2 = length2(d);
    if (len2 > 0) { const float dt = dot(vabs(d), oErr) / len2; o = o + d * dt; }
    const float a = (d.x * d.x + d.y * d.y) + d.z * d.z;
    const float b = 2.f * ((d.x * o.x + d.y * o.y) + d.z * o.z);
    const float c = ((o.x * o.x + o.y * o.y) + o.z * o.z) - s.radius * s.radius;
    const double discrim = (double)b * (double)b - 4. * (double)a * (double)c;
    if (discrim < 0.) return false;
    const float fr = (float)sqrt(discrim);
    const float q = b < 0 ? -.5f * (b - fr) : -.5f * (b + fr);
    float t0 = q / a, t1 = c / q;
    if (t0 > t1) { const float tmp = t0; t0 = t1; t1 = tmp; }
    if (t0 > r.tMax || t1 <= 0) return false;
    return true;
}

__device__ __noinline__ bool sphere_test(const DevSphere &s, const DRay &r, DRay *rayObj, vec3 *pHitOut, float *phiOut,
                                         float *tOut) {
    vec3 oErr, dErr;
    vec3 o = xf_point_err(s.w2o, r.o, &oErr);
    vec3 d = xf_vector_err(s.w2o, r.d, &dErr);
    float len2 = length2(d);
// ... 68 lines not shown
```

### thesis-pbrt-v3_amd/csrc/device/kernels.h

```cpp
#pragma once
#include <hip/hip_runtime.h>
#include <algorithm>
#include <type_traits>
#include "dev_shading.h"

namespace hprt {

struct RayStream { float4 *a, *b; };
struct HitStream { float4 *a; float2 *b; };
__device__ __forceinline__ void hit_store(const HitStream &h, uint32_t slot, int32_t word, float b0, float b1, float b2, float t, int32_t inst) {
    h.a[slot] = make_float4(b0, b1, b2, __int_as_float(word));
    if (h.b) h.b[slot] = make_float2(t, __int_as_float(inst));
}
__device__ __forceinline__ void hit_store_miss(const HitStream &h, uint32_t slot, float tMax) { hit_store(h, slot, -1, 0.f, 0.f, 0.f, tMax, -1); }
__device__ __forceinline__ float4 hit_load(const HitStream &h, uint32_t slot) { return h.a[slot]; }
__device__ __forceinline__ float2 hit_load_aux(const HitStream &h, uint32_t slot) { return h.b[slot]; }
__device__ __forceinline__ float2 hit_no_aux() { return make_float2(0.f, __int_as_float(-1)); }
__host__ __device__ __forceinline__ int32_t hit_word(const float4 &rec) { return __builtin_bit_cast(int32_t, rec.w); }
__host__ __device__ __forceinline__ float hit_b0(const float4 &rec) { return rec.x; }
__host__ __device__ __forceinline__ float hit_b1(const float4 &rec) { return rec.y; }
__host__ __device__ __forceinline__ float hit_b2(const float4 &rec) { return rec.z; }
__host__ __device__ __forceinline__ float hit_t(const float2 &aux) { return aux.x; }
__host__ __device__ __forceinline__ int32_t hit_inst(const float2 &aux) { return __builtin_bit_cast(int32_t, aux.y); }
struct PathStream {
    RayStream ray;
    float4 *beta;
    float4 *L;
};
enum : uint32_t { RAY_DIM_MASK = 0xffffu, RAY_BOUNCE_SHIFT = 16u, RAY_BOUNCE_MASK = 0x3fffu, RAY_FOLD_MARK = 0x40000000u, RAY_SPECULAR = 0x80000000u };
struct VertexStreams {
    RayStream shadow; uint8_t *occluded;
    RayStream mis; HitStream misHit;
    float4 *pendLight;
    float4 *pendMis;
    float4 *pendBeta;
    const float4 *pendPrev;
};
enum : uint32_t { SPEC_RECORD = 0x80000000u, SPEC_END = 0x40000000u, SPEC_ID_MASK = 0x0fffffffu, SPEC_MAX_PATHS = 1u << 28 };
struct QueueSet {
    uint32_t *next, *shadow, *mis, *resolve, *end;
    uint32_t *nextCount, *shadowCount, *misCount, *resolveCount, *endCount;
};
enum : uint32_t { BIN_STRIDE = 64u };
struct BinSet { uint2 *q[5]; uint32_t *aux; uint32_t *count; uint2 *retry[2]; };
struct RenderParams {
    DevCamera cam;
    DevHalton hal;
    const uint32_t *pixelXY;
    const uint64_t *pixelOffset;
    uint32_t nPix;
    int32_t maxDepth;
    float rrThreshold;
    float invSqrtSpp;
    int32_t cullMis;
    int32_t speculate;
    int32_t foldRepair;
};
struct FilmGeom {
    int32_t cx0, cy0, cx1, cy1;
    int32_t sx0, sy0, sx1, sy1;
    float rx, ry;
    float maxSampleLuminance;
};
struct IrregularSample { uint32_t pix, sample; int16_t x0, x1, y0, y1; };
struct IrregularSink { FilmGeom fg; uint32_t *count; uint32_t capacity; IrregularSample *out; };
struct FilmExtras {
    const uint32_t *ownBegin; const uint32_t *ownSrcPix; const uint32_t *ownSample; const uint8_t *ownIsPre;
    uint32_t nForeignDest;
    const uint32_t *foreignDestFilmIndex; const uint32_t *foreignDestBegin; const uint32_t *foreignGroupBegin;
    const uint32_t *foreignSrcPix; const uint32_t *foreignSample;
};

struct FilmRecord { uint32_t dest, srcTile; float xyz[3]; float w; };

bool WideWalkInUse(const DevScene &sc);
void LaunchTrace(hipStream_t st, const DevScene &sc, bool anyHit, bool count, const uint32_t *queue, const uint32_t *countPtr,
                 uint32_t countImm, uint32_t gridItems, const RayStream &rays, const HitStream &hits, uint8_t *occ,
                 DevCounters *counters, uint32_t *workCounter, uint4 *rayStats = nullptr);
template <uint32_t BLOCK, uint32_t WAVES, uint32_t QUAD_WAVES, typename Launch>
void LaunchTreeWalk(hipStream_t st, const DevScene &sc, bool anyHit, bool count, uint32_t gridItems, uint32_t *workCounter, Launch launch) {
    if (gridItems == 0) return;
    (void)hipMemsetAsync(workCounter, 0, sizeof(uint32_t), st);
    const bool quad = sc.nSpheres != 0u;
    const dim3 grid(std::min((uint32_t)(((size_t)gridItems + BLOCK - 1) / BLOCK), 256u * (quad ? QUAD_WAVES : WAVES))), block(BLOCK);
    auto pickQuad = [&](auto a, auto c) { if (quad) launch(grid, block, a, c, std::true_type{}); else launch(grid, block, a, c, std::false_type{}); };
    auto pickCount = [&](auto a) { if (count) pickQuad(a, std::true_type{}); else pickQuad(a, std::false_type{}); };
    if (anyHit) pickCount(std::true_type{}); else pickCount(std::false_type{});
}
void LaunchPixelStats(hipStream_t st, const uint4 *rayStats, const float4 *ids, const uint32_t *queue, const uint32_t *countPtr,
                      uint32_t countImm, uint32_t gridItems, uint32_t nPix, bool anyHit, uint32_t *pix);
void LaunchPixelStatsToFilm(hipStream_t st, const uint32_t *pix, const uint32_t *pixelXY, uint32_t nPix, uint32_t spp, int cx0, int cy0, int width,
                            unsigned long long *out7);
void LaunchGenerate(hipStream_t st, const DevScene &sc, const RenderParams &rp, const PathStream &out, uint32_t s0, uint32_t nSlots,
                    const IrregularSink *irr = nullptr);
void LaunchBin(hipStream_t st, const DevScene &sc, const PathStream &in, const HitStream &hit, const uint32_t *queue,
               const uint32_t *countPtr, uint32_t countImm, uint32_t gridItems, int32_t maxDepth, int32_t bounces, const BinSet &bins,
               float4 *Lfinal, const VertexStreams &vs, bool foldRepair);
void LaunchShade(hipStream_t st, int mode, const DevScene &sc, const RenderParams &rp, const PathStream &in, const HitStream &hit,
                 uint32_t gridItems, uint32_t s0, const PathStream &out, const VertexStreams &vs, const QueueSet &q,
                 const BinSet &bins, float4 *Lfinal, bool firstBounce, bool retryPass = false);
void LaunchResolve(hipStream_t st, const DevScene &sc, const VertexStreams &vs, float4 *L, float4 *Lfinal, const uint32_t *queue,
                   const uint32_t *countPtr, uint32_t gridItems);
void LaunchRepair(hipStream_t st, const VertexStreams &vs, float4 *L, float4 *Lfinal, const uint32_t *queue, uint32_t n, uint32_t *counts);
void LaunchStoreRadiance(hipStream_t st, const float4 *Lfinal, float *LallR, float *LallG, float *LallB, uint32_t nPix, uint32_t s0,
                         uint32_t nSlots);
void LaunchPackRays(hipStream_t st, const float *rays7, uint32_t n, const RayStream &out);
void LaunchUnpackHits(hipStream_t st, const HitStream &hits, uint32_t n, float *t, int32_t *prim, float *bary3);
void LaunchFindIrregular(hipStream_t st, const DevScene &sc, const RenderParams &rp, const FilmGeom &fg, uint32_t spp, uint32_t *count,
                         uint32_t capacity, IrregularSample *out);
void LaunchFilmOwn(hipStream_t st, const RenderParams &rp, const FilmGeom &fg, const float *LallR, const float *LallG, const float *LallB,
                   uint32_t spp, const FilmExtras &ex, float *film);
void LaunchFilmForeign(hipStream_t st, const RenderParams &rp, const FilmGeom &fg, const float *LallR, const float *LallG,
                       const float *LallB, const FilmExtras &ex, float *film);
void LaunchFilmForeignExport(hipStream_t st, const RenderParams &rp, const FilmGeom &fg, const float *LallR, const float *LallG,
                             const float *LallB, const FilmExtras &ex, uint32_t nGroups, const uint32_t *groupDest, const uint32_t *groupTile,
                             FilmRecord *out);
void LaunchVoxelDistributions(hipStream_t st, const DevScene &sc, const float *ri, uint32_t nVox, float *func, float *cdf, float *funcInt);
void LaunchVoxelFill(hipStream_t st, const DevScene &sc, const float *ri, uint32_t n, uint32_t rowBase, float *func, float *cdf, float *funcInt);
void LaunchStreamCopy(hipStream_t st, const float4 *src, float4 *dst, size_t n);
void LaunchGatherProbe(hipStream_t st, const uint4 *records, uint32_t log2Records, int itersPerLane, uint32_t blocks, uint32_t *sink);
void LaunchCaptureRays(hipStream_t st, const uint32_t *queue, uint32_t n, const RayStream &rays, float *out7, uint32_t cap);
void LaunchFilmApplyRecords(hipStream_t st, const FilmRecord *rec, const uint32_t *destBegin, uint32_t nDest, float *film);

}
```

### thesis-pbrt-v3_amd/csrc/device/kernels.hip

```cpp
#include <hip/hip_runtime.h>
#include <algorithm>
#include <cstdio>
#include <cstdlib>
#include <string>
#include "dev_shading.h"
#include "kernels.h"
#ifndef HPRT_QUAD_ANY_WAVES
#define HPRT_QUAD_ANY_WAVES 5
#endif
#define HPRT_QUAD_CLOSEST_WAVES 4
#ifndef HPRT_LDS_STACK_QUAD_ANY
#define HPRT_LDS_STACK_QUAD_ANY 12
#endif
#define HPRT_LDS_STACK_INST_ANY 7
#define HPRT_LDS_STACK_INST_CLOSEST 9
#ifndef HPRT_ANY_WAVES
#define HPRT_ANY_WAVES 7
#endif
#ifndef HPRT_CLOSEST_WAVES
#define HPRT_CLOSEST_WAVES 6
#endif
#ifndef HPRT_LDS_STACK_CLOSEST
#define HPRT_LDS_STACK_CLOSEST 12
#endif

namespace hprt {

typedef unsigned int u32x4 __attribute__((ext_vector_type(4)));
typedef unsigned int u32x2 __attribute__((ext_vector_type(2)));
typedef float f32x2 __attribute__((ext_vector_type(2)));

__device__ __forceinline__ uint32_t wave_append(uint32_t *counter, bool pred) {
    const unsigned long long mask = __ballot(pred);
    if (mask == 0ull) return 0u;
    const uint32_t lane = __lane_id();
    const uint32_t prefix = __builtin_amdgcn_mbcnt_hi((uint32_t)(mask >> 32), __builtin_amdgcn_mbcnt_lo((uint32_t)mask, 0u));
    const int leader = __ffsll((long long)mask) - 1;
    uint32_t base = 0u;
    if ((int)lane == leader) base = atomicAdd(counter, (uint32_t)__popcll(mask));
    base = __shfl(base, leader);
    return base + prefix;
}

struct BlockAppendLds { uint32_t waveCount[5][16]; uint32_t base[5]; };
template <int NQ>
__device__ __forceinline__ void block_append(BlockAppendLds *lds, uint32_t *const counter[NQ], const bool pred[NQ], uint32_t pos[NQ]) {
    const uint32_t lane = __lane_id(), wave = threadIdx.x >> 6, nWaves = (blockDim.x + 63) >> 6;
    unsigned long long mask[NQ];
#pragma unroll
    for (int k = 0; k < NQ; ++k) {
        mask[k] = __ballot(pred[k]);
        if (lane == 0) lds->waveCount[k][wave] = (uint32_t)__popcll(mask[k]);
    }
    __syncthreads();
    if (threadIdx.x < NQ) {
        const int k = threadIdx.x;
        uint32_t total = 0;
        for (uint32_t w = 0; w < nWaves; ++w) { const uint32_t c = lds->waveCount[k][w]; lds->waveCount[k][w] = total; total += c; }
        lds->base[k] = total ? atomicAdd(counter[k], total) : 0u;
    }
    __syncthreads();
#pragma unroll
    for (int k = 0; k < NQ; ++k)
        pos[k] = lds->base[k] + lds->waveCount[k][wave] +
                 __builtin_amdgcn_mbcnt_hi((uint32_t)(mask[k] >> 32), __builtin_amdgcn_mbcnt_lo((uint32_t)mask[k], 0u));
}

struct TraceTune { int refillBelow, parkLimit, stepLimit, sphereLimit, primMin; };
static TraceTune DefaultTraceTune(bool anyHit) {
    TraceTune t = anyHit ? TraceTune{40, 24, 10, 4, 3} : TraceTune{52, 24, 6, 4, 8};
    if (const char *e = getenv(anyHit ? "HPRT_TRACE_TUNE_ANY" : "HPRT_TRACE_TUNE"))
        sscanf(e, "%d,%d,%d,%d,%d", &t.refillBelow, &t.parkLimit, &t.stepLimit, &t.sphereLimit, &t.primMin);
    return t;
}

__device__ __forceinline__ bool slab_test(float lox, float hix, float loy, float hiy, float loz, float hiz, vec3 ro, vec3 invDir,
                                          bool negX, bool negY, bool negZ, float robust, float *tEntry) {
    float tMin = ((negX ? hix : lox) - ro.x) * invDir.x;
    float tMax = ((negX ? lox : hix) - ro.x) * invDir.x;
    const float tyMin = ((negY ? hiy : loy) - ro.y) * invDir.y;
    float tyMax = ((negY ? loy : hiy) - ro.y) * invDir.y;
    tMax *= robust; tyMax *= robust;
    bool ok = !(tMin > tyMax || tyMin > tMax);
    if (tyMin > tMin) tMin = tyMin;
    if (tyMax < tMax) tMax = tyMax;
    const float tzMin = ((negZ ? hiz : loz) - ro.z) * invDir.z;
    float tzMax = ((negZ ? loz : hiz) - ro.z) * invDir.z;
    tzMax *= robust;
    ok = ok && !(tMin > tzMax || tzMin > tMax);
    if (tzMin > tMin) tMin = tzMin;
    if (tzMax < tMax) tMax = tzMax;
    *tEntry = tMin;
    return ok && (tMax > 0);
}

__device__ __forceinline__ void slab_test_pair(f32x2 nx, f32x2 fx, f32x2 ny, f32x2 fy, f32x2 nz, f32x2 fz, float rox, float roy, float roz,
                                               float ivx, float ivy, float ivz, float robust, bool *s0, bool *s1, float *t0, float *t1) {
    f32x2 tMin = (nx - rox) * ivx;
    f32x2 tMax = (fx - rox) * ivx;
    const f32x2 tyMin = (ny - roy) * ivy;
    f32x2 tyMax = (fy - roy) * ivy;
    tMax = tMax * robust; tyMax = tyMax * robust;
    const f32x2 tzMin = (nz - roz) * ivz;
    f32x2 tzMax = (fz - roz) * ivz;
    tzMax = tzMax * robust;
    bool ok0 = !(tMin.x > tyMax.x || tyMin.x > tMax.x), ok1 = !(tMin.y > tyMax.y || tyMin.y > tMax.y);
    if (tyMin.x > tMin.x) tMin.x = tyMin.x;
    if (tyMin.y > tMin.y) tMin.y = tyMin.y;
    if (tyMax.x < tMax.x) tMax.x = tyMax.x;
    if (tyMax.y < tMax.y) tMax.y = tyMax.y;
    ok0 = ok0 && !(tMin.x > tzMax.x || tzMin.x > tMax.x); ok1 = ok1 && !(tMin.y > tzMax.y || tzMin.y > tMax.y);
    if (tzMin.x > tMin.x) tMin.x = tzMin.x;
    if (tzMin.y > tMin.y) tMin.y = tzMin.y;
    if (tzMax.x < tMax.x) tMax.x = tzMax.x;
    if (tzMax.y < tMax.y) tMax.y = tzMax.y;
    *t0 = tMin.x; *t1 = tMin.y;
    *s0 = ok0 && (tMax.x > 0); *s1 = ok1 && (tMax.y > 0);
}

__device__ unsigned long long g_traceProf[32];
#ifdef HPRT_SHADE_PROF
__device__ unsigned long long g_shadeProf[4 * 8];
__device__ unsigned long long g_shadeLanes[4 * 8 * 2];
#define SP_MARK(k) do { asm volatile("s_waitcnt vmcnt(0) lgkmcnt(0)" ::: "memory"); const unsigned long long t_ = clock64(); spT[k] += t_ - spLast; spLast = t_; \
                        const unsigned long long m_ = __ballot(1); if (__lane_id() == (uint32_t)(__ffsll((long long)m_) - 1)) { atomicAdd(&g_shadeLanes[(MODE * 8 + k) * 2], (unsigned long long)__popcll(m_)); atomicAdd(&g_shadeLanes[(MODE * 8 + k) * 2 + 1], 1ull); } } while (0)
#else
#define SP_MARK(k) do { } while (0)
#endif

template <bool ANY_HIT, int MODE, bool INST, bool QUAD>
__global__ __launch_bounds__(HPRT_TRACE_BLOCK, MODE == 0 ? (QUAD ? (ANY_HIT ? HPRT_QUAD_ANY_WAVES : HPRT_QUAD_CLOSEST_WAVES) : ANY_HIT ? HPRT_ANY_WAVES : HPRT_CLOSEST_WAVES) : 1024 / HPRT_TRACE_BLOCK) void k_trace(DevScene sc, const uint32_t *queue, const uint32_t *countPtr,
                                                            uint32_t countImm, RayStream rays, HitStream hits, uint8_t *occ,
                                                            DevCounters *counters, uint4 *rayStats, uint32_t *workCounter, uint32_t chunk,
                                                            TraceTune tune) {
    constexpr bool COUNT = MODE == 1, PROF = MODE == 2;
    constexpr bool PACKED = !QUAD;
    constexpr bool FREE_ORDER = ANY_HIT && MODE == 0;
#ifdef HPRT_DEFER_LEAF
    constexpr bool DEFER = FREE_ORDER && !INST && !QUAD;
#else
    constexpr bool DEFER = false;
#endif
    int pend = REF_NONE;
    constexpr bool HPRT_INLINE_PRETEST = true;
    unsigned long long pf[13] = {0, 0, 0, 0, 0, 0, 0, 0, 0, 0, 0, 0, 0};
    unsigned int pfPush = 0u, pfSpill = 0u;
    const unsigned long long pfStart = PROF ? clock64() : 0ull;
    constexpr int LDS_N = MODE != 0 ? HPRT_LDS_STACK
                        : !INST ? (QUAD ? (ANY_HIT ? HPRT_LDS_STACK_QUAD_ANY : HPRT_LDS_STACK) : ANY_HIT ? HPRT_LDS_STACK_ANY : HPRT_LDS_STACK_CLOSEST)
                                : (QUAD ? HPRT_LDS_STACK_QUAD_ANY : ANY_HIT ? HPRT_LDS_STACK_INST_ANY : HPRT_LDS_STACK_INST_CLOSEST);
    __shared__ uint2 stackMem[LDS_N * HPRT_TRACE_BLOCK];
    uint2 *const ldsStack = &stackMem[threadIdx.x];
    __shared__ float worldRayMem[INST ? 6 * HPRT_TRACE_BLOCK : 1];
    float *const worldRay = &worldRayMem[INST ? threadIdx.x : 0];
    const uint32_t n = countPtr ? *countPtr : countImm;
    const uint32_t lane = __lane_id();
    const auto pairRsrc = __builtin_amdgcn_make_buffer_rsrc((void *)sc.pairs, 0, (int)(sc.nPairs * 64u), 0x00020000);
    const auto triRsrc = __builtin_amdgcn_make_buffer_rsrc((void *)sc.tris, 0, (int)(sc.nPrims * 48u), 0x00020000);
    const auto entryRsrc = __builtin_amdgcn_make_buffer_rsrc((void *)(INST ? sc.topEntry : nullptr), 0, (int)(INST ? sc.nTopPrims * 16u : 0u), 0x00020000);
    const float robust = 1 + 2 * gamma_n(3);
    TraceCount cnt = {0u, 0u, 0u, 0u, 0u};
    unsigned int snapEntered = 0u, snapLeaf = 0u, snapPrim = 0u;
    bool active = false, hit = false;
    uint32_t slot = 0;
    vec3 ro, invDir;
    float rayTMax = 0.f;
    RayShear shear; shear.k0 = shear.k1 = false; shear.Sx = shear.Sy = shear.Sz = 0.f;
    bool ngX = false, ngY = false, ngZ = false;
    uint32_t negMask = 0u;
    int sp = 0, cur = REF_NONE;
    int32_t prim = -1; float hb0 = 0.f, hb1 = 0.f, hb2 = 0.f;
    uint32_t wait = 0u, waitInfo = 0u;
    int inst = -1, hitInst = -1;
    bool instHit = false;
    uint32_t instPrim = 0u;
    float savedTMax = 0.f;
// ... 1262 lines not shown
    for (uint32_t e = ex.foreignGroupBegin[g]; e < ex.foreignGroupBegin[g + 1]; ++e) {
        const size_t o = (size_t)ex.foreignSample[e] * rp.nPix + ex.foreignSrcPix[e];
        c = c + clamp_luminance(rgb(LallR[o], LallG[o], LallB[o]), fg.maxSampleLuminance) * 1.0f * 1.0f;
        w += 1.f;
    }
    FilmRecord r;
    r.dest = groupDest[g]; r.srcTile = groupTile[g];
    rgb_to_xyz(c, r.xyz);
    r.w = w;
    out[g] = r;
}
__global__ __launch_bounds__(64) void k_film_apply_records(const FilmRecord *rec, const uint32_t *destBegin, uint32_t nDest, float *filmXYZW) {
    const uint32_t d = blockIdx.x * blockDim.x + threadIdx.x;
    if (d >= nDest) return;
    const size_t fo = 4 * (size_t)rec[destBegin[d]].dest;
    for (uint32_t k = destBegin[d]; k < destBegin[d + 1]; ++k) {
        filmXYZW[fo] += rec[k].xyz[0]; filmXYZW[fo + 1] += rec[k].xyz[1]; filmXYZW[fo + 2] += rec[k].xyz[2]; filmXYZW[fo + 3] += rec[k].w;
    }
}

__global__ __launch_bounds__(256) void k_voxel_contrib(DevScene sc, const float *ri, uint32_t nVox, float *contrib, const uint32_t *voxList) {
    const size_t g = (size_t)blockIdx.x * blockDim.x + threadIdx.x;
    const uint32_t n = sc.nLights;
    if (g >= (size_t)nVox * n) return;
    const uint32_t row = (uint32_t)(g / n), j = (uint32_t)(g % n);
    const uint32_t v = voxList ? voxList[row] : row;
    int pi[3]; pi[2] = (int)(v % (uint32_t)sc.voxN[2]); pi[1] = (int)((v / (uint32_t)sc.voxN[2]) % (uint32_t)sc.voxN[1]); pi[0] = (int)(v / ((uint32_t)sc.voxN[2] * (uint32_t)sc.voxN[1]));
    float vMin[3], vMax[3];
#pragma unroll
    for (int a = 0; a < 3; ++a) {
        const float t0 = (float)pi[a] / (float)sc.voxN[a], t1 = (float)(pi[a] + 1) / (float)sc.voxN[a];
        vMin[a] = (1 - t0) * sc.wbMin[a] + t0 * sc.wbMax[a];
        vMax[a] = (1 - t1) * sc.wbMin[a] + t1 * sc.wbMax[a];
    }
    const DevLight light = sc.lights[j];
    float acc = 0.f;
    for (int i = 0; i < 128; ++i) {
        DevIt ref;
        ref.p = vec3((1 - ri[i]) * vMin[0] + ri[i] * vMax[0], (1 - ri[128 + i]) * vMin[1] + ri[128 + i] * vMax[1], (1 - ri[256 + i]) * vMin[2] + ri[256 + i] * vMax[2]);
        ref.pErr = vec3(); ref.n = vec3();
        vec3 wi; float pdf = 0.f; DevIt pl;
        const rgb Li = light_sample<true>(sc, light, ref, ri[384 + i], ri[512 + i], &wi, &pdf, &pl);
        if (pdf > 0) acc += luminance(Li) / pdf;
    }
    contrib[g] = acc;
}
__global__ __launch_bounds__(256) void k_voxel_dist(uint32_t nLights, uint32_t nVox, float *func, float *cdf, float *funcInt) {
    const uint32_t v = blockIdx.x * blockDim.x + threadIdx.x;
    if (v >= nVox) return;
    float *f = func + (size_t)v * nLights, *c = cdf + (size_t)v * (nLights + 1);
    float sum = 0.f;
    for (uint32_t i = 0; i < nLights; ++i) sum += f[i];
    const float avg = sum / (float)(128ull * nLights);
    const float minContrib = (avg > 0) ? (float)(.001 * (double)avg) : 1.f;
    for (uint32_t i = 0; i < nLights; ++i) f[i] = sel_max(f[i], minContrib);
    const int n = (int)nLights;
    c[0] = 0;
    for (int i = 1; i < n + 1; ++i) c[i] = c[i - 1] + f[i - 1] / n;
    const float fi = c[n];
    if (fi == 0) for (int i = 1; i < n + 1; ++i) c[i] = float(i) / float(n);
    else for (int i = 1; i < n + 1; ++i) c[i] /= fi;
    funcInt[v] = fi;
}

__global__ void k_fill_u32(uint32_t *p, uint32_t v, size_t n) {
    const size_t i = (size_t)blockIdx.x * blockDim.x + threadIdx.x;
    if (i < n) p[i] = v;
}

static inline uint32_t blocks_for(size_t n, uint32_t bs) { return (uint32_t)((n + bs - 1) / bs); }

static int g_wideWalk = -1;
static bool WideWalkEnabled() {
    static const bool fromEnv = [] { const char *e = getenv("HPRT_WIDE_WALK"); return !(e && atoi(e) == 0); }();
    return g_wideWalk < 0 ? fromEnv : g_wideWalk != 0;
}
static int g_traceProfileMode = -1;
static bool TraceProfileEnabled() {
    static const bool fromEnv = getenv("HPRT_TRACE_PROFILE") != nullptr;
    return g_traceProfileMode < 0 ? fromEnv : g_traceProfileMode != 0;
}
extern "C" __attribute__((visibility("default"))) int hprt_debug_trace_profile_mode(int on) { const int was = TraceProfileEnabled() ? 1 : 0; g_traceProfileMode = on; return was; }
bool WideWalkInUse(const DevScene &sc) { return sc.wide != nullptr && WideWalkEnabled(); }
extern "C" __attribute__((visibility("default"))) int hprt_debug_wide_walk(int on) { const int was = WideWalkEnabled() ? 1 : 0; g_wideWalk = on; return was; }
void LaunchTrace(hipStream_t st, const DevScene &sc, bool anyHit, bool count, const uint32_t *queue, const uint32_t *countPtr,
                 uint32_t countImm, uint32_t gridItems, const RayStream &rays, const HitStream &hits, uint8_t *occ,
                 DevCounters *counters, uint32_t *workCounter, uint4 *rayStats) {
    if (gridItems == 0) return;
    (void)hipMemsetAsync(workCounter, 0, sizeof(uint32_t), st);
    static const uint32_t blockCap = [] { const char *e = getenv("HPRT_TRACE_MAX_BLOCKS"); return e ? (uint32_t)std::max(1, atoi(e)) : 0xffffffffu; }();
    static const uint32_t anyPerCu = [] { const char *e = getenv("HPRT_TRACE_ANY_PER_CU"); return e ? (uint32_t)std::min((int)(HPRT_DEEP_THREADS / (256u * HPRT_TRACE_BLOCK)), std::max(1, atoi(e))) : (uint32_t)HPRT_ANY_WAVES; }();
    const bool profile = TraceProfileEnabled();
    const bool plain = !count && !profile;
    const bool hasQuad = sc.nSpheres != 0u;
    static const uint32_t closestPerCu = [] { const char *e = getenv("HPRT_TRACE_CLOSEST_PER_CU"); return e ? (uint32_t)std::min(7, std::max(1, atoi(e))) : (uint32_t)HPRT_CLOSEST_WAVES; }();
    const uint32_t perCu = !plain ? 4u : hasQuad ? (anyHit ? (uint32_t)HPRT_QUAD_ANY_WAVES : (uint32_t)HPRT_QUAD_CLOSEST_WAVES) : (anyHit ? anyPerCu : closestPerCu);
    const uint32_t maxBlocks = std::min(256u * perCu, blockCap);
    static_assert(HPRT_DEEP_THREADS >= 256u * HPRT_TRACE_BLOCK * HPRT_ANY_WAVES && HPRT_DEEP_THREADS >= 256u * HPRT_TRACE_BLOCK * HPRT_CLOSEST_WAVES &&
                  HPRT_DEEP_THREADS >= 256u * HPRT_TRACE_BLOCK * HPRT_QUAD_ANY_WAVES, "the deep-stack area must cover the largest trace grid");
    dim3 grid(std::min(blocks_for(gridItems, HPRT_TRACE_BLOCK), maxBlocks)), block(HPRT_TRACE_BLOCK);
    const uint32_t nWaves = grid.x * (HPRT_TRACE_BLOCK / 64);
    static const uint32_t chunkMax = [] { const char *e = getenv("HPRT_TRACE_CHUNK_MAX"); return e ? (uint32_t)atoi(e) : 512u; }();
    static const uint32_t chunkDiv = [] { const char *e = getenv("HPRT_TRACE_CHUNK_DIV"); return e ? (uint32_t)atoi(e) : 4u; }();
    uint32_t chunk = gridItems / (nWaves * chunkDiv);
    chunk = std::max(64u, std::min(chunkMax, chunk)) & ~63u;
    static const TraceTune tuneClosest = DefaultTraceTune(false), tuneAny = DefaultTraceTune(true);
    TraceTune tune = anyHit ? tuneAny : tuneClosest;
    static const bool tuneFromEnv = getenv("HPRT_TRACE_TUNE") != nullptr;
    if (!anyHit && !tuneFromEnv && sc.nPairs > 100000u) { tune.parkLimit = 32; tune.stepLimit = 14; tune.primMin = 12; }
    const bool inst = sc.nInstances != 0u, quad = sc.nSpheres != 0u;
    static const bool tuneAnyFromEnv = getenv("HPRT_TRACE_TUNE_ANY") != nullptr;
    if (inst && !anyHit && !tuneFromEnv) { tune.parkLimit = 32; tune.stepLimit = 10; tune.primMin = 12; }
    if (inst && anyHit && !tuneAnyFromEnv) { tune.refillBelow = 48; tune.parkLimit = 32; tune.stepLimit = 10; tune.primMin = 6; }
    if (!count && sc.wide != nullptr && WideWalkEnabled()) {
        static const uint32_t wClosestPerCu = [] { const char *e = getenv("HPRT_WALK4_CLOSEST_PER_CU"); return e ? (uint32_t)std::min((int)HPRT_WALK4_CLOSEST_WAVES, std::max(1, atoi(e))) : (uint32_t)HPRT_WALK4_CLOSEST_WAVES; }();
        static const uint32_t wAnyPerCu = [] { const char *e = getenv("HPRT_WALK4_ANY_PER_CU"); return e ? (uint32_t)std::min((int)HPRT_WALK4_ANY_WAVES, std::max(1, atoi(e))) : (uint32_t)HPRT_WALK4_ANY_WAVES; }();
        static const TraceTune wTuneClosest = [] { TraceTune t{52, 32, 8, 4, 12}; if (const char *e = getenv("HPRT_WALK4_TUNE")) sscanf(e, "%d,%d,%d,%d,%d", &t.refillBelow, &t.parkLimit, &t.stepLimit, &t.sphereLimit, &t.primMin); return t; }();
        static const TraceTune wTuneAny = [] { TraceTune t{52, 28, 6, 4, 4}; if (const char *e = getenv("HPRT_WALK4_TUNE_ANY")) sscanf(e, "%d,%d,%d,%d,%d", &t.refillBelow, &t.parkLimit, &t.stepLimit, &t.sphereLimit, &t.primMin); return t; }();
        const uint32_t wPerCu = profile ? 4u : quad ? (anyHit ? (uint32_t)HPRT_QUAD_ANY_WAVES : (uint32_t)HPRT_QUAD_CLOSEST_WAVES) : inst ? (anyHit ? (uint32_t)HPRT_WALK4_INST_ANY_WAVES : (uint32_t)HPRT_WALK4_INST_CLOSEST_WAVES) : anyHit ? wAnyPerCu : wClosestPerCu;
        const uint32_t wBlocks = std::min(256u * wPerCu, blockCap);
        dim3 wGrid(std::min(blocks_for(gridItems, HPRT_TRACE_BLOCK), wBlocks));
        const uint32_t wWaves = wGrid.x * (HPRT_TRACE_BLOCK / 64);
        uint32_t wChunk = gridItems / (wWaves * chunkDiv);
        wChunk = std::max(64u, std::min(chunkMax, wChunk)) & ~63u;
        TraceTune wTune = anyHit ? wTuneAny : wTuneClosest;
        static const bool wTuneEnv = getenv("HPRT_WALK4_TUNE") != nullptr, wTuneAnyEnv = getenv("HPRT_WALK4_TUNE_ANY") != nullptr;
        if (inst && !anyHit && !wTuneEnv) wTune = TraceTune{52, 40, 14, 4, 16};
        if (inst && anyHit && !wTuneAnyEnv) wTune = TraceTune{48, 40, 14, 4, 8};
#define HPRT_WALK4_LAUNCH(A, P, I, Q) hipLaunchKernelGGL((k_walk4<A, P, I, Q>), wGrid, block, 0, st, sc, queue, countPtr, countImm, rays, hits, occ, workCounter, wChunk, wTune)
#define HPRT_WALK4_PICK(A) do { if (profile) { if (inst) HPRT_WALK4_LAUNCH(A, true, true, true); else HPRT_WALK4_LAUNCH(A, true, false, true); } \
                                else if (inst) { if (quad) HPRT_WALK4_LAUNCH(A, false, true, true); else HPRT_WALK4_LAUNCH(A, false, true, false); } \
                                else { if (quad) HPRT_WALK4_LAUNCH(A, false, false, true); else HPRT_WALK4_LAUNCH(A, false, false, false); } } while (0)
        if (anyHit) HPRT_WALK4_PICK(true); else HPRT_WALK4_PICK(false);
#undef HPRT_WALK4_PICK
#undef HPRT_WALK4_LAUNCH
        return;
    }
#define HPRT_TRACE_LAUNCH(A, M, I, Q) hipLaunchKernelGGL((k_trace<A, M, I, Q>), grid, block, 0, st, sc, queue, countPtr, countImm, rays, hits, occ, counters, rayStats, workCounter, chunk, tune)
#define HPRT_TRACE_PICK(A, M) do { if (inst) { if (quad || M == 2) HPRT_TRACE_LAUNCH(A, M, true, true); else HPRT_TRACE_LAUNCH(A, M, true, (M == 2)); } \
                                   else { if (quad || M == 2) HPRT_TRACE_LAUNCH(A, M, false, true); else HPRT_TRACE_LAUNCH(A, M, false, (M == 2)); } } while (0)
    if (anyHit) {
        if (count) HPRT_TRACE_PICK(true, 1); else if (profile) HPRT_TRACE_PICK(true, 2); else HPRT_TRACE_PICK(true, 0);
    } else {
        if (count) HPRT_TRACE_PICK(false, 1); else if (profile) HPRT_TRACE_PICK(false, 2); else HPRT_TRACE_PICK(false, 0);
    }
#undef HPRT_TRACE_PICK
#undef HPRT_TRACE_LAUNCH
}
#ifdef HPRT_SHADE_PROF
extern "C" __attribute__((visibility("default"))) int hprt_debug_shade_profile(unsigned long long out[24 + 48]) {
    if (hipMemcpyFromSymbol(out, HIP_SYMBOL(g_shadeProf), sizeof(unsigned long long) * 24) != hipSuccess) return -1;
    return hipMemcpyFromSymbol(out + 24, HIP_SYMBOL(g_shadeLanes), sizeof(unsigned long long) * 48) == hipSuccess ? 0 : -1;
}
#endif
extern "C" __attribute__((visibility("default"))) int hprt_debug_trace_profile(unsigned long long out[32], int reset) {
    if (hipMemcpyFromSymbol(out, HIP_SYMBOL(g_traceProf), sizeof(unsigned long long) * 32) != hipSuccess) return -1;
    if (reset) { unsigned long long z[32] = {0}; if (hipMemcpyToSymbol(HIP_SYMBOL(g_traceProf), z, sizeof(z)) != hipSuccess) return -1; }
    return 0;
}
void LaunchGenerate(hipStream_t st, const DevScene &sc, const RenderParams &rp, const PathStream &out, uint32_t s0, uint32_t nSlots,
                    const IrregularSink *irr) {
    IrregularSink sink; memset(&sink, 0, sizeof(sink));
    if (irr) sink = *irr;
    if (nSlots) hipLaunchKernelGGL(k_generate, dim3(blocks_for(nSlots, 256)), dim3(256), 0, st, sc, rp, out, s0, nSlots, sink);
}
void LaunchBin(hipStream_t st, const DevScene &sc, const PathStream &in, const HitStream &hit, const uint32_t *queue,
// ... 174 lines not shown
```

### thesis-pbrt-v3_amd/csrc/device_state.h

```cpp
#pragma once
#include <hip/hip_runtime.h>
#include <algorithm>
#include <mutex>
#include <string>
#include <vector>
#include "../../include/hprt.h"
#include "device/kernels.h"
#include "device/kd_walk.h"
#include "device/rbsp_walk.h"
#include "device/rbspkd_walk.h"
#include "device/bsppaper_walk.h"
#include "device/bsppaperkd_walk.h"
#include "device/kdinst_walk.h"
#include "device/rbspinst_walk.h"
#include "device/bsppaperinst_walk.h"
#include "hprt_internal.h"

#define HIP_TRY(expr)                                                                                   \
    do {                                                                                                \
        hipError_t e__ = (expr);                                                                        \
        if (e__ != hipSuccess)                                                                          \
            return hprt::SetError(HPRT_E_DEVICE, std::string(#expr) + ": " + hipGetErrorString(e__));   \
    } while (0)

namespace hprt {

struct DevBuf {
    void *p = nullptr; size_t bytes = 0;
    ~DevBuf() { if (p) (void)hipFree(p); }
    hipError_t alloc(size_t n) {
        if (p && bytes >= n) return hipSuccess;
        if (p) { (void)hipFree(p); p = nullptr; bytes = 0; }
        if (n == 0) return hipSuccess;
        hipError_t e = hipMalloc(&p, n);
        if (e == hipSuccess) bytes = n;
        return e;
    }
    template <typename T> T *as() const { return (T *)p; }
};
template <typename T> hipError_t upload(DevBuf &b, const std::vector<T> &v) {
    hipError_t e = b.alloc(std::max<size_t>(v.size() * sizeof(T), 16));
    if (e != hipSuccess || v.empty()) return e;
    return hipMemcpy(b.p, v.data(), v.size() * sizeof(T), hipMemcpyHostToDevice);
}

}

struct HprtScene;
namespace hprt {
struct SceneCall {
    std::unique_lock<std::mutex> lk; HprtScene *s; hipStream_t st;
    SceneCall(HprtScene *scene, hipStream_t stream);
    void leave_async();
};
}

struct HprtScene {
    int device = 0;
    std::mutex mu;
    hipEvent_t lastUse = nullptr; bool lastUsePending = false;
    hprt::DevScene dev;
    hprt::DevBuf textures, mipLevels, texels, weightLut;
    hprt::DevBuf nodes, tris, primVtx, primN, vUV, vS, shapes, materials, lights, spheres, instances, topEntry, topEntryWide, lightFunc, lightCdf, perms, primes, primeSums, primeMagic;
    hprt::DevBuf envLights, envData;
    hprt::DevBuf wide, leafBox;
    hprt::DevBuf counters, workCounter, deepStack;
    struct Capture { int bounce = -1, kind = 0; float *out7 = nullptr; size_t cap = 0, n = 0; } capture;
    bool shadeCountsOn = false; uint64_t shadeDeferred = 0, shadeRetried = 0;
    uint64_t shadeSpeculated = 0, shadeRepaired = 0, shadeFull = 0;
    int poisonByte = -1;
    hprt::DevBuf voxFunc, voxCdf, voxFuncInt, voxRi;
    hprt::DevBuf voxSlot, voxRequest, voxRequestCount, retryQueues;
    uint32_t voxRows = 0, voxRowsUsed = 0, nVoxels = 0;
    hprt::DevBuf rayStats, pixelStatsLocal, pixelStatsFilm; bool pixelStatsValid = false;
    hprt::DevBuf planes;
    hprt::DevBuf apiRays, apiHits;
    hprt::DevBuf queues, queueCounts;
    hprt::DevBuf pixelXY, pixelOffset, Lall, film, irregular, irregularCount;
    hprt::DevBuf exOwnBegin, exOwnSrc, exOwnSample, exOwnPre, exFDest, exFDestBegin, exFGroupBegin, exFSrc, exFSample;
    hprt::DevBuf foreignRecords, exGroupDest, exGroupTile; uint32_t nForeignRecords = 0; bool foreignExported = false;
    int filmW = 0, filmH = 0;
    float *lastFilm = nullptr;
    uint32_t *hostCounts = nullptr;
    size_t filmPixels = 0;
    uint32_t nPrims = 0;
    enum class Walk { Bvh, Kd, Rbsp, RbspKd, BspPaper, BspPaperKd, KdInst, RbspInst, RbspKdInst, BspPaperInst, BspPaperKdInst } walk = Walk::Bvh;
    hprt::DevBuf treeNodes, treePrims, treeAxes; hprt::DevKd kd{}; hprt::DevRbsp rbsp{}; hprt::DevBspPaper bsppaper{};
    hprt::DevBuf kdShare, pixelKdLocal, pixelKdFilm; bool pixelKdValid = false;
    std::vector<uint32_t> topOrder; bool instanced = false;
    bool hasSubstrateBin = false;
    hprt::DevBuf instEntries; hprt::DevKdInst kdinst{}; hprt::DevRbspInst rbspinst{}; hprt::DevBspPaperInst bsppaperinst{};
    std::vector<std::vector<uint32_t>> objectOrder; std::vector<uint32_t> objectPrimBase; std::vector<int32_t> instanceObject;
    ~HprtScene() { if (hostCounts) (void)hipHostFree(hostCounts); if (lastUse) (void)hipEventDestroy(lastUse); }
};

inline hprt::SceneCall::SceneCall(HprtScene *scene, hipStream_t stream) : lk(scene->mu), s(scene), st(stream) {
    if (s->lastUsePending && s->lastUse) (void)hipStreamWaitEvent(st, s->lastUse, 0);
}
inline void hprt::SceneCall::leave_async() {
    if (!s->lastUse && hipEventCreateWithFlags(&s->lastUse, hipEventDisableTiming) != hipSuccess) { s->lastUse = nullptr; (void)hipStreamSynchronize(st); s->lastUsePending = false; return; }
    s->lastUsePending = hipEventRecord(s->lastUse, st) == hipSuccess;
    if (!s->lastUsePending) (void)hipStreamSynchronize(st);
}
```

### thesis-pbrt-v3_amd/csrc/scene_layout.cpp

```cpp
#include <algorithm>
#include <cmath>
#include <cstdlib>
#include <cstring>
#include <utility>
#include "scene_layout.h"
#include "bvh_builder.h"
#include "device/dev_intersect.h"
#include "hprt_internal.h"
#include "wide_bvh.h"

namespace hprt {
namespace {

float RoughnessToAlpha(float roughness) {
    roughness = sel_max(roughness, (float)1e-3);
    float x = std::log(roughness);
    return 1.62142f + 0.819955f * x + 0.1734f * x * x + 0.0171201f * x * x * x + 0.000640711f * x * x * x * x;
}

bool TriangleIsBogus(vec3 p0, vec3 p1, vec3 p2, const float *uv0, const float *uv1, const float *uv2) {
    float u0x = 0, u0y = 0, u1x = 1, u1y = 0, u2x = 1, u2y = 1;
    if (uv0) { u0x = uv0[0]; u0y = uv0[1]; u1x = uv1[0]; u1y = uv1[1]; u2x = uv2[0]; u2y = uv2[1]; }
    float duv02x = u0x - u2x, duv02y = u0y - u2y, duv12x = u1x - u2x, duv12y = u1y - u2y;
    vec3 dp02 = p0 - p2, dp12 = p1 - p2;
// ... 387 lines not shown
    if (d->n_nodes) {
        const BvhNode &root = ((const BvhNode *)d->nodes)[0];
        wbLo = vec3(root.bmin[0], root.bmin[1], root.bmin[2]); wbHi = vec3(root.bmax[0], root.bmax[1], root.bmax[2]);
        vec3 c = div_by(wbLo + wbHi, 2.f);
        bool inside = c.x >= wbLo.x && c.x <= wbHi.x && c.y >= wbLo.y && c.y <= wbHi.y && c.z >= wbLo.z && c.z <= wbHi.z;
        L.worldRadius = inside ? dist(c, wbHi) : 0.f;
    }
    for (int a = 0; a < 3; ++a) { L.wbMin[a] = wbLo.get(a); L.wbMax[a] = wbHi.get(a); }
    L.lightFunc.assign(std::max<uint32_t>(1, d->n_lights), 1.f); L.lightCdf.assign(d->n_lights + 1, 0.f);
    if (L.lightStrategy == 1)
        for (uint32_t l = 0; l < d->n_lights; ++l) {
            const HprtLightDesc &in = d->lights[l];
            const rgb I(in.I[0], in.I[1], in.I[2]);
            rgb power;
            if (in.type == 0) power = I * (4 * HPRT_PI);
            else if (in.type == 1) power = I * HPRT_PI * L.worldRadius * L.worldRadius;
            else if (in.type == 3) power = HPRT_PI * L.worldRadius * L.worldRadius * HostMipLookupWidth(d->textures[in.texture], .5f, .5f, .5f);
            else {
                const HprtShapeDesc &ls = d->shapes[in.shape];
                float area;
                if (ls.kind == 1) area = ls.phi_max * ls.radius * (ls.z_max - ls.z_min);
                else {
                    const int32_t *v = &ls.indices[3 * (size_t)((int32_t)l - ls.area_light)];
                    const vec3 p0(ls.P[3 * v[0]], ls.P[3 * v[0] + 1], ls.P[3 * v[0] + 2]), p1(ls.P[3 * v[1]], ls.P[3 * v[1] + 1], ls.P[3 * v[1] + 2]),
                               p2(ls.P[3 * v[2]], ls.P[3 * v[2] + 1], ls.P[3 * v[2] + 2]);
                    area = (float)(0.5 * (double)length(cross(p1 - p0, p2 - p0)));
                }
                power = I * (float)(in.two_sided ? 2 : 1) * area * HPRT_PI;
            }
            L.lightFunc[l] = luminance(power);
        }
    if (d->n_lights) dist1d_build(L.lightFunc.data(), (int)d->n_lights, L.lightCdf.data(), &L.funcInt);
    if (L.lightStrategy == 2) {
        const vec3 diag = wbHi - wbLo;
        const int me = (diag.x > diag.y && diag.x > diag.z) ? 0 : (diag.y > diag.z ? 1 : 2);
        const float bmax = diag.get(me);
        for (int a = 0; a < 3; ++a) L.voxN[a] = std::max(1, int(std::round(diag.get(a) / bmax * 64)));
    }
    return HPRT_OK;
}

int LayoutPairs(Work &w) {
    SceneLayout &L = w.L;
    L.pairs.resize((size_t)w.pairBase[w.aggs.size()]);
    for (size_t ai = 0; ai < w.aggs.size(); ++ai) {
        const Agg &g = w.aggs[ai];
        if (g.nNodes == 0) continue;
        const BvhNode *nd = g.nodes;
        std::vector<int32_t> ref(g.nNodes);
        int32_t nextPair = (int32_t)w.pairBase[ai] + 1;
        for (uint32_t i = 0; i < g.nNodes; ++i) {
            if ((nd[i].countAxis & 3u) == 3u) {
                ref[i] = ~(int32_t)(w.primBase[ai] + (uint32_t)nd[i].offset);
                const size_t last = (size_t)w.primBase[ai] + (uint32_t)nd[i].offset + (nd[i].countAxis >> 2) - 1u;
                L.tris[3 * last].w = u2f(f2u(L.tris[3 * last].w) | TAG_LAST);
            } else ref[i] = nextPair++;
        }
        auto fill = [&](DevPair &p, uint32_t c0, uint32_t c1, uint32_t meta) {
            const BvhNode &a = nd[c0], &b = nd[c1];
            p.x[0] = a.bmin[0]; p.x[1] = b.bmin[0]; p.x[2] = a.bmax[0]; p.x[3] = b.bmax[0];
            p.y[0] = a.bmin[1]; p.y[1] = b.bmin[1]; p.y[2] = a.bmax[1]; p.y[3] = b.bmax[1];
            p.z[0] = a.bmin[2]; p.z[1] = b.bmin[2]; p.z[2] = a.bmax[2]; p.z[3] = b.bmax[2];
            p.ref0 = ref[c0]; p.ref1 = ref[c1]; p.meta = meta; p.pad = 0u;
        };
        fill(L.pairs[w.pairBase[ai]], 0u, 0u, PAIR_SINGLE);
        for (uint32_t i = 0; i < g.nNodes; ++i) {
            if ((nd[i].countAxis & 3u) == 3u) continue;
            fill(L.pairs[(size_t)ref[i]], i + 1u, (uint32_t)nd[i].offset, nd[i].countAxis & 3u);
        }
    }
    return HPRT_OK;
}

int LayoutWide(Work &w) {
    SceneLayout &L = w.L;
    w.wideBase.assign(w.aggs.size(), -1);
    bool wideOk = L.nPrims < (1u << 28);
    int wideNeedTop = 0, wideNeedObject = 0;
    for (size_t ai = 0; ai < w.aggs.size() && wideOk; ++ai) {
        const Agg &g = w.aggs[ai];
        if (g.nNodes == 0) continue;
        const BvhNode *nd = g.nodes;
        std::vector<int32_t> leafRefW(g.nNodes, WIDE_NONE);
        if (L.leafBox.empty()) L.leafBox.assign(2 * (size_t)L.nPrims, make_float4(0.f, 0.f, 0.f, 0.f));
        for (uint32_t i = 0; i < g.nNodes; ++i) {
            if ((nd[i].countAxis & 3u) != 3u) continue;
            const uint32_t firstPrim = w.primBase[ai] + (uint32_t)nd[i].offset, count = nd[i].countAxis >> 2;
            bool single = count == 1u && (f2u(L.tris[3 * (size_t)firstPrim].w) & TAG_KIND_MASK) == 0u;
            if (single) {
                const float4 *v = &L.tris[3 * (size_t)firstPrim];
                const float c[3][3] = {{v[0].x, v[1].x, v[2].x}, {v[0].y, v[1].y, v[2].y}, {v[0].z, v[1].z, v[2].z}};
                for (int a = 0; a < 3 && single; ++a) {
                    bool posZero = false, negZero = false;
                    for (int k = 0; k < 3; ++k) { if (c[a][k] != c[a][k]) single = false; if (c[a][k] == 0.f) { if (f2u(c[a][k]) >> 31) negZero = true; else posZero = true; } }
                    const float mn = std::min(std::min(c[a][0], c[a][1]), c[a][2]), mx = std::max(std::max(c[a][0], c[a][1]), c[a][2]);
                    if ((posZero && negZero) || f2u(mn) != f2u(nd[i].bmin[a]) || f2u(mx) != f2u(nd[i].bmax[a])) single = false;
                }
            }
            uint32_t r = ~firstPrim;
            if (!single) r &= ~WIDE_LEAF_BOXED;
            leafRefW[i] = (int32_t)r;
            for (uint32_t k = 0; k < count; ++k) {
                L.leafBox[2 * (size_t)(firstPrim + k)] = make_float4(nd[i].bmin[0], nd[i].bmin[1], nd[i].bmin[2], nd[i].bmax[0]);
                L.leafBox[2 * (size_t)(firstPrim + k) + 1] = make_float4(nd[i].bmax[1], nd[i].bmax[2], 0.f, 0.f);
            }
        }
        int need = 0;
        w.wideBase[ai] = (int32_t)L.wide.size();
        if (!BuildWide(nd, g.nNodes, leafRefW.data(), &L.wide, &need)) wideOk = false;
        if (ai == 0) wideNeedTop = need; else wideNeedObject = std::max(wideNeedObject, need);
    }
    if (!wideOk || wideNeedTop + (w.d.n_instances ? 1 + wideNeedObject : 0) > HPRT_WIDE_STACK_MAX || w.wideBase[0] != 0) { L.wide.clear(); L.leafBox.clear(); }
    return HPRT_OK;
}

int LayoutInstances(Work &w) {
    const HprtSceneDesc *d = &w.d;
    SceneLayout &L = w.L;
    L.instances.resize(d->n_instances);
    for (uint32_t i = 0; i < d->n_instances; ++i) {
        const HprtInstanceDesc &in = d->instances[i];
        DevInstance &o = L.instances[i];
        memcpy(o.i2w.m, in.instance_to_world, 64); memcpy(o.w2i.m, in.world_to_instance, 64);
        const size_t ai = 1 + (size_t)in.object;
        o.root = w.aggs[ai].nPrims > 1 ? (int32_t)w.pairBase[ai] : ~(int32_t)w.primBase[ai];
        bool ident = true;
        for (int r = 0; r < 4; ++r) for (int c = 0; c < 4; ++c) if (o.i2w.m[r][c] != (r == c ? 1.f : 0.f)) ident = false;
        o.identity = ident ? 1u : 0u; o.pad[0] = o.pad[1] = 0u;
        if (!L.wide.empty()) o.pad[0] = w.aggs[ai].nPrims > 1 ? (uint32_t)w.wideBase[ai] : ((~(uint32_t)w.primBase[ai]) & ~WIDE_LEAF_FIRST);
    }
    if (!d->n_instances) return HPRT_OK;
    const uint32_t nTop = w.aggs[0].nPrims;
    L.topEntry.assign(nTop, make_float4(0.f, 0.f, 0.f, 0.f));
    if (!L.wide.empty()) L.topEntryWide.assign(nTop, make_float4(0.f, 0.f, 0.f, 0.f));
    for (uint32_t oi = 0; oi < nTop; ++oi) {
        float4 *r = &L.tris[3 * ((size_t)w.primBase[0] + oi)];
        const uint32_t tag = f2u(r[0].w);
        if ((tag & TAG_KIND_MASK) != TAG_INSTANCE) continue;
        const DevInstance &in = L.instances[f2u(r[2].w)];
        const float (*m)[4] = in.w2i.m;
        if (!(m[3][0] == 0.f && m[3][1] == 0.f && m[3][2] == 0.f && m[3][3] == 1.f)) continue;
        r[0] = make_float4(m[0][0], m[0][1], m[0][2], u2f(tag | TAG_INST_INLINE));
        r[1] = make_float4(m[1][0], m[1][1], m[1][2], r[1].w);
        r[2] = make_float4(m[2][0], m[2][1], m[2][2], r[2].w);
        L.topEntry[oi] = make_float4(m[0][3], m[1][3], m[2][3], u2f((uint32_t)in.root));
        if (!L.wide.empty()) L.topEntryWide[oi] = make_float4(m[0][3], m[1][3], m[2][3], u2f(in.pad[0]));
    }
    return HPRT_OK;
}

}

int BuildSceneLayout(const HprtSceneDesc &d, SceneLayout *out) {
    Work w{d, *out};
    w.inlineMaterialMax = TAG_MATERIAL_MAX;
    if (const char *e = getenv("HPRT_INLINE_MATERIAL_MAX")) { const long v = atol(e); w.inlineMaterialMax = v < 0 ? 0u : (uint32_t)std::min<long>(v, (long)TAG_MATERIAL_MAX); }
    for (int (*stage)(Work &) : {ValidateArrays, ValidateShapes, GatherAggregates, CheckAggregates, ValidateLights}) if (int rc = stage(w)) return rc;
    out->nPrims = w.primBase.back();
    out->topOrder.assign(d.prim_order, d.prim_order + d.n_prims);
    out->instanced = d.n_instances != 0;
    for (uint32_t k = 0; k < d.n_objects; ++k) {
        out->objectOrder.emplace_back(d.objects[k].prim_order, d.objects[k].prim_order + d.objects[k].n_prims);
        out->objectPrimBase.push_back(w.primBase[1 + (size_t)k]);
    }
    for (uint32_t i = 0; i < d.n_instances; ++i) out->instanceObject.push_back(d.instances[i].object);
    for (int (*stage)(Work &) : {LayoutShapes, LayoutPrimitives, LayoutMaterials, LayoutTextures, LayoutLights, LayoutEnvLights,
                                 LayoutLightDistribution, LayoutPairs, LayoutWide, LayoutInstances})
        if (int rc = stage(w)) return rc;
    return HPRT_OK;
}

int LayoutTagsForDebug(const HprtSceneDesc &d, std::vector<uint32_t> *tags, std::vector<uint32_t> *primShape, std::vector<uint32_t> *shapeFlags,
                       std::vector<int32_t> *shapeMaterial) {
    SceneLayout L;
    if (int rc = BuildSceneLayout(d, &L)) return rc;
    for (uint32_t i = 0; i < L.nPrims; ++i) { tags->push_back(f2u(L.tris[3 * (size_t)i].w)); primShape->push_back(f2u(L.tris[3 * (size_t)i + 1].w)); }
    for (const DevShape &s : L.shapes) { shapeFlags->push_back(s.flags); shapeMaterial->push_back(s.material); }
    return HPRT_OK;
}

void VoxelSamplePoints(float *out) {
    const int bases[5] = {2, 3, 5, 7, 11};
    for (int b = 0; b < 5; ++b)
        for (uint32_t i = 0; i < 128; ++i) {
            float v;
            if (b == 0) {
                uint32_t n = i;
                n = (n << 16) | (n >> 16); n = ((n & 0x00ff00ffu) << 8) | ((n & 0xff00ff00u) >> 8); n = ((n & 0x0f0f0f0fu) << 4) | ((n & 0xf0f0f0f0u) >> 4);
                n = ((n & 0x33333333u) << 2) | ((n & 0xccccccccu) >> 2); n = ((n & 0x55555555u) << 1) | ((n & 0xaaaaaaaau) >> 1);
                v = (float)((double)n * 0x1p-32);
            } else {
                const int base = bases[b];
                const float invBase = (float)1 / (float)base;
                uint64_t reversedDigits = 0, a = i;
                float invBaseN = 1;
                while (a) { uint64_t next = a / base, digit = a - next * base; reversedDigits = reversedDigits * base + digit; invBaseN *= invBase; a = next; }
                v = sel_min((float)reversedDigits * invBaseN, HPRT_ONE_MINUS_EPS);
            }
            out[128 * b + i] = v;
        }
}

}

extern "C" __attribute__((visibility("default"))) int hprt_debug_voxel_points(float out[640]) { if (!out) return HPRT_E_INVALID; hprt::VoxelSamplePoints(out); return HPRT_OK; }
```

### thesis-pbrt-v3_amd/csrc/scene_layout.h

```cpp
#pragma once
#include <cstdint>
#include <vector>
#include "../../include/hprt.h"
#include "device/dev_scene.h"

namespace hprt {

struct SceneLayout {
    std::vector<DevPair> pairs;
    std::vector<DevWide> wide;
    std::vector<float4> leafBox, tris, primN;
    std::vector<uint32_t> primVtx;
    std::vector<float> vUV, vS;
    std::vector<DevShape> shapes;
    std::vector<DevSphere> spheres;
    std::vector<DevMaterial> materials;
    std::vector<DevTexture> textures;
    std::vector<DevMipLevel> mipLevels;
    std::vector<float> texels, weightLut;
    std::vector<DevLight> lights;
    std::vector<DevEnvLight> envLights;
    std::vector<float> envData;
    std::vector<DevInstance> instances;
    std::vector<float4> topEntry, topEntryWide;
    std::vector<float> lightFunc, lightCdf;
    float funcInt = 0.f, worldRadius = 0.f;
    float wbMin[3] = {0, 0, 0}, wbMax[3] = {0, 0, 0};
    int lightStrategy = 0;
    int voxN[3] = {1, 1, 1};
    uint32_t nPrims = 0;
    std::vector<uint32_t> topOrder;
    std::vector<std::vector<uint32_t>> objectOrder;
    std::vector<uint32_t> objectPrimBase;
    std::vector<int32_t> instanceObject;
    bool instanced = false, hasSubstrateBin = false;
};

int BuildSceneLayout(const HprtSceneDesc &d, SceneLayout *out);

void VoxelSamplePoints(float *out);

}
```

Measured before the change: 6331 Mrays/s.

## Add light-centered cube-map shadow grid for point-light occlusion rays

Builds a cube-map grid around the single point light at scene load. Each cell lists the triangles that can occlude rays leaving through that direction, sorted by a distance key. Shadow rays in path rendering then use a dedicated grid kernel instead of BVH any-hit traversal, which is meant to cut traversal cost for occlusion queries. This adds build time and memory, and the result depends on conservative margins for correctness. Eligibility checks fall back to the BVH when the lists grow too large.

Result: faster. 6564 Mrays/s, median of 6 (+3.7%).

```diff
diff --git a/thesis-pbrt-v3_amd/__init__.py b/thesis-pbrt-v3_amd/__init__.py
--- a/thesis-pbrt-v3_amd/__init__.py
+++ b/thesis-pbrt-v3_amd/__init__.py
@@ -353,6 +353,10 @@
         debug["hprt_debug_%s_bounds" % prefix] = (C.c_int, [vp, C.c_int, vp])
         debug["hprt_debug_%s_set_tree" % prefix] = (C.c_int, [vp, C.c_int, sz, vp, sz, vp, vp])
     debug["hprt_debug_halton_index"] = (C.c_int, [P(RenderOptions), sz, vp, vp, vp, vp, vp, vp])
+    debug["hprt_debug_shadow_grid"] = (C.c_int, [C.c_int])
+    debug["hprt_debug_shadow_grid_info"] = (C.c_int, [vp, vp])
+    debug["hprt_debug_shadow_grid_occluded"] = (C.c_int, [vp, sz, vp, vp, vp])
+    debug["hprt_debug_shadow_grid_build"] = (C.c_int, [sz, vp, vp, C.c_uint32, vp, vp, sz, vp, sz])
     for name, (res, args) in list(sig.items()) + list(debug.items()):
         fn = getattr(lib, name)
         fn.restype = res
@@ -390,6 +394,27 @@
         p.hprt_debug_device_halton.argtypes = [C.c_void_p, C.c_int, C.c_int, C.c_int, C.c_int, C.c_size_t, C.c_void_p, C.c_void_p, C.c_void_p]
         _probe_lib = p
     return _probe_lib
+
+
+SG_SINGLE, SG_PRIM_MASK = 0x80000000, 0x0fffffff
+
+
+def debug_shadow_grid(on):
+    return lib.hprt_debug_shadow_grid(int(on))
+
+
+def shadow_grid_build(p9, light, res):
+    p9 = np.ascontiguousarray(p9, np.float32).reshape(-1, 9)
+    light = np.ascontiguousarray(light, np.float32)
+    info = np.zeros(6, np.float64)
+    _check(lib.hprt_debug_shadow_grid_build(p9.shape[0], _ptr(p9), _ptr(light), int(res), _ptr(info), None, 0, None, 0))
+    R, n_entries = int(info[0]), int(info[1])
+    cell_start = np.zeros(6 * R * R + 1, np.uint32); entries = np.zeros((max(1, n_entries), 2), np.uint32)
+    _check(lib.hprt_debug_shadow_grid_build(p9.shape[0], _ptr(p9), _ptr(light), int(res), _ptr(info), _ptr(cell_start), cell_start.size, _ptr(entries), entries.shape[0]))
+    entries = entries[:n_entries]
+    return {"R": R, "eps": float(info[3]), "near": int(info[2]), "longest": int(info[4]), "seconds": float(info[5]), "cell_start": cell_start,
+            "prim": (entries[:, 0] & SG_PRIM_MASK).astype(np.int64), "single": (entries[:, 0] & SG_SINGLE) != 0, "key": (entries[:, 1] & np.uint32(0xffff0000)).view(np.float32),
+            "rect": np.stack([(entries[:, 1] >> s) & 15 for s in (0, 4, 8, 12)], axis=1).astype(np.int64)}
 
 
 def debug_halton_index(opt, px, py, sample):
@@ -943,6 +968,17 @@
         ctr = np.zeros(4, np.uint64) if count else None
         _check(lib.hprt_occluded(self._h, n, _ptr(o), _ptr(d), _ptr(tmax), _ptr(occ), _ptr(ctr)))
         return (occ, ctr) if count else occ
+
+    def shadow_grid_info(self):
+        out = np.zeros(12, np.float64)
+        _check(lib.hprt_debug_shadow_grid_info(self._h, _ptr(out)))
+        return {"eligible": bool(out[0]), "R": int(out[1]), "entries": int(out[2]), "near": int(out[3]), "bytes": int(out[4]), "build_seconds": float(out[5]),
+                "longest": int(out[6]), "mean": float(out[7]), "light": out[8:11].astype(np.float32), "render_launches": int(out[11])}
+
+    def shadow_grid_occluded_device(self, n, rays7_ptr, occ_ptr):
+        ms = C.c_float()
+        _check(lib.hprt_debug_shadow_grid_occluded(self._h, n, rays7_ptr, occ_ptr, C.byref(ms)))
+        return float(ms.value)
 
     def intersect_device(self, n, rays7_ptr, t_ptr, prim_ptr, bary_ptr=None, stream=None):
         _check(lib.hprt_intersect_device(self._h, n, rays7_ptr, t_ptr, prim_ptr, bary_ptr, stream))
diff --git a/thesis-pbrt-v3_amd/build.py b/thesis-pbrt-v3_amd/build.py
--- a/thesis-pbrt-v3_amd/build.py
+++ b/thesis-pbrt-v3_amd/build.py
@@ -8,14 +8,14 @@
 CSRC = os.path.join(HERE, "csrc")
 OBJ = os.path.join(HERE, "build")
 LIB = os.path.join(HERE, "lib")
-HOST_SRCS = ["pbrt_frontend.cpp", "loop_subdiv.cpp", "scene_io.cpp", "texture_io.cpp", "bvh_builder.cpp", "kdtree_builder.cpp", "rbsp_builder.cpp", "bsppaper_builder.cpp", "bspnode_builder.cpp", "bvhold_builder.cpp", "wide_bvh.cpp", "halton_tables.cpp", "capi_host.cpp"]
+HOST_SRCS = ["pbrt_frontend.cpp", "loop_subdiv.cpp", "scene_io.cpp", "texture_io.cpp", "bvh_builder.cpp", "kdtree_builder.cpp", "rbsp_builder.cpp", "bsppaper_builder.cpp", "bspnode_builder.cpp", "bvhold_builder.cpp", "wide_bvh.cpp", "shadow_grid.cpp", "halton_tables.cpp", "capi_host.cpp"]
 HIPCC_HOST_SRCS = ["scene_layout.cpp"]
-HIP_SRCS = ["device/kernels.hip", "device/kd_walk.hip", "device/rbsp_walk.hip", "device/rbspkd_walk.hip", "device/bsppaper_walk.hip", "device/bsppaperkd_walk.hip", "device/kdinst_walk.hip", "device/kdop_cost.hip", "device/rbspinst_walk.hip", "device/bsppaperinst_walk.hip", "device/bsp_cost.hip", "device/bspnode_cost.hip", "device/hlbvh_build.hip", "capi_device.hip", "capi_gather.hip"]
+HIP_SRCS = ["device/kernels.hip", "device/kd_walk.hip", "device/rbsp_walk.hip", "device/rbspkd_walk.hip", "device/bsppaper_walk.hip", "device/bsppaperkd_walk.hip", "device/kdinst_walk.hip", "device/kdop_cost.hip", "device/rbspinst_walk.hip", "device/bsppaperinst_walk.hip", "device/bsp_cost.hip", "device/bspnode_cost.hip", "device/hlbvh_build.hip", "device/shadow_grid.hip", "capi_device.hip", "capi_gather.hip"]
 CUIDS = {"device/kernels.hip": "a6cd736c50efffab", "device/kd_walk.hip": "5c0d2e7f41b3a916", "device/rbsp_walk.hip": "3e91a5c07d2b84f6",
          "device/rbspkd_walk.hip": "7a4f0c2e9b61d385", "device/bsppaper_walk.hip": "c52e8b1d06f3a794",
          "device/bsppaperkd_walk.hip": "e8136d4a9f07c2b5", "device/kdinst_walk.hip": "4d9b27f1a60c8e53", "device/kdop_cost.hip": "b7e20a5c93d1f468",
          "device/rbspinst_walk.hip": "9f3c61d8b2047ae5", "device/bsppaperinst_walk.hip": "2c7e5a90d4b18f63", "device/bsp_cost.hip": "6b1f94c3e7a0d258",
-         "device/bspnode_cost.hip": "d3a7150c8e4f92b6", "device/hlbvh_build.hip": "58e2c9a4f1b7063d",
+         "device/bspnode_cost.hip": "d3a7150c8e4f92b6", "device/hlbvh_build.hip": "58e2c9a4f1b7063d", "device/shadow_grid.hip": "a17c3e58d90b24f6",
          "capi_device.hip": "1b24418c11488d5c", "capi_gather.hip": "89501e8167866ce2"}
 PROBE_SRCS = ["device/halton_probe.hip"]
 CUIDS["device/halton_probe.hip"] = "f04b8d61c2a79e35"
diff --git a/thesis-pbrt-v3_amd/csrc/capi_device.hip b/thesis-pbrt-v3_amd/csrc/capi_device.hip
--- a/thesis-pbrt-v3_amd/csrc/capi_device.hip
+++ b/thesis-pbrt-v3_amd/csrc/capi_device.hip
@@ -165,6 +165,16 @@
     HIP_TRY(upload(sc->textures, L.textures)); HIP_TRY(upload(sc->mipLevels, L.mipLevels)); HIP_TRY(upload(sc->texels, L.texels)); HIP_TRY(upload(sc->weightLut, L.weightLut));
     HIP_TRY(upload(sc->wide, L.wide)); HIP_TRY(upload(sc->leafBox, L.leafBox));
     HIP_TRY(upload(sc->envLights, L.envLights)); HIP_TRY(upload(sc->envData, L.envData));
+    if (L.shadowGrid.eligible) {
+        const ShadowGrid &sg = L.shadowGrid;
+        static_assert(sizeof(SgEntry) == sizeof(uint2), "grid entries are read as 8-byte words");
+        std::vector<SgEntry> padded(sg.entries);
+        padded.push_back(SgEntry{0u, 0u});
+        HIP_TRY(upload(sc->sgCells, sg.cellStart)); HIP_TRY(upload(sc->sgEntries, padded));
+        sc->sg = DevShadowGrid{sc->sgCells.as<uint32_t>(), sc->sgEntries.as<uint2>(), (uint32_t)sg.entries.size(), sg.nNear, sg.R};
+        sc->sgInfo.longest = sg.longest; sc->sgInfo.buildSeconds = sg.buildSeconds; sc->sgInfo.eps = sg.eps; sc->sgInfo.bytes = sg.bytes();
+        for (int a = 0; a < 3; ++a) sc->sgInfo.light[a] = sg.light[a];
+    }
     HIP_TRY(sc->counters.alloc(sizeof(DevCounters)));
     HIP_TRY(hipMemset(sc->counters.p, 0, sizeof(DevCounters)));
     HIP_TRY(sc->deepStack.alloc((size_t)HPRT_SPILL_STACK * HPRT_DEEP_THREADS * sizeof(uint2)));
@@ -298,6 +308,39 @@
     case HprtScene::Walk::Bvh: LaunchTrace(st, s->dev, anyHit, count, queue, countPtr, countImm, gridItems, rays, hits, occ, counters, workCounter, rayStats); break;
     }
 }
+static int g_shadowGrid = -1;
+static bool ShadowGridInUse(const HprtScene *s) {
+    return s->sg.entries != nullptr && g_shadowGrid != 0 && s->walk == HprtScene::Walk::Bvh && hprt::WideWalkInUse(s->dev) && !hprt::TraceProfileInUse();
+}
+__attribute__((visibility("default"))) int hprt_debug_shadow_grid(int on) { const int was = g_shadowGrid; g_shadowGrid = on; return was; }
+__attribute__((visibility("default"))) int hprt_debug_shadow_grid_info(HprtScene *s, double out[12]) {
+    if (!s || !out) return HPRT_E_INVALID;
+    for (int a = 0; a < 3; ++a) out[8 + a] = s->sgInfo.light[a];
+    out[11] = (double)s->sgInfo.renderLaunches;
+    const bool has = s->sg.entries != nullptr;
+    const double nCells = has ? 6.0 * s->sg.R * s->sg.R : 1.0;
+    out[0] = has ? 1 : 0; out[1] = s->sg.R; out[2] = s->sg.nEntries; out[3] = s->sg.nNear; out[4] = (double)s->sgInfo.bytes;
+    out[5] = s->sgInfo.buildSeconds; out[6] = s->sgInfo.longest; out[7] = has ? (s->sg.nEntries - s->sg.nNear) / nCells : 0.0;
+    return HPRT_OK;
+}
+__attribute__((visibility("default"))) int hprt_debug_shadow_grid_occluded(HprtScene *s, size_t n, const float *d_rays7, uint8_t *d_occ, float *ms) try {
+    if (!s || !d_rays7 || !d_occ || n == 0 || n > 0x7ffffff0ull) return SetError(HPRT_E_INVALID, "hprt_debug_shadow_grid_occluded: bad argument");
+    if (!s->sg.entries) return SetError(HPRT_E_UNSUPPORTED, "hprt_debug_shadow_grid_occluded: the scene has no shadow grid");
+    HIP_TRY(hipSetDevice(s->device));
+    SceneCall call(s, nullptr);
+    RayStream rays; HitStream hits;
+    if (int rc = ApiStreams(s, n, &rays, &hits)) return rc;
+    struct Events { hipEvent_t e[2] = {nullptr, nullptr}; ~Events() { for (auto x : e) if (x) (void)hipEventDestroy(x); } } ev;
+    for (auto &x : ev.e) HIP_TRY(hipEventCreate(&x));
+    LaunchPackRays(nullptr, d_rays7, (uint32_t)n, rays);
+    HIP_TRY(hipEventRecord(ev.e[0], nullptr));
+    LaunchShadowGrid(nullptr, s->dev, s->sg, nullptr, nullptr, (uint32_t)n, (uint32_t)n, rays, d_occ, s->workCounter.as<uint32_t>());
+    HIP_TRY(hipEventRecord(ev.e[1], nullptr));
+    HIP_TRY(hipGetLastError());
+    HIP_TRY(hipDeviceSynchronize());
+    if (ms) HIP_TRY(hipEventElapsedTime(ms, ev.e[0], ev.e[1]));
+    return HPRT_OK;
+} catch (...) { return hprt::HandleException(); }
 __attribute__((visibility("default"))) int hprt_debug_trace_queued(HprtScene *s, size_t n, const float *d_rays7, const uint32_t *d_queue, int anyHit,
                                                                     float *d_scratch7, float ms[2]) try {
     if (!s || !d_rays7 || !d_queue || !d_scratch7 || !ms || n == 0 || n > 0x7ffffff0ull) return SetError(HPRT_E_INVALID, "hprt_debug_trace_queued: bad argument");
@@ -881,7 +924,11 @@
             hipEvent_t a = ev.get(), b = ev.get();
             HIP_TRY(hipEventRecord(a, st));
             HitStream none; none.a = nullptr; none.b = nullptr;
-            Trace(s, st, true, count, cur.shadow, nullptr, nShadow, nShadow, vs.shadow, none, vs.occluded, ctr, wcPath, rayStats);
+            if (ShadowGridInUse(s) && !count && !rayStats && rp.cullMis) {
+                LaunchShadowGrid(st, s->dev, s->sg, cur.shadow, nullptr, nShadow, nShadow, vs.shadow, vs.occluded, wcPath);
+                ++s->sgInfo.renderLaunches;
+            }
+            else Trace(s, st, true, count, cur.shadow, nullptr, nShadow, nShadow, vs.shadow, none, vs.occluded, ctr, wcPath, rayStats);
             if (pixelStats) LaunchPixelStats(st, rayStats, vs.pendBeta, cur.shadow, nullptr, nShadow, nShadow, rp.nPix, true, pixelStats);
             if (pixelKd) LaunchPixelKdStats(st, rayStats, vs.pendBeta, cur.shadow, nullptr, nShadow, nShadow, rp.nPix, true, pixelKd);
             HIP_TRY(hipEventRecord(b, st));
diff --git a/thesis-pbrt-v3_amd/csrc/capi_host.cpp b/thesis-pbrt-v3_amd/csrc/capi_host.cpp
--- a/thesis-pbrt-v3_amd/csrc/capi_host.cpp
+++ b/thesis-pbrt-v3_amd/csrc/capi_host.cpp
@@ -22,6 +22,7 @@
 #include "scene_model.h"
 #include "hprt_math.h"
 #include "wide_bvh.h"
+#include "shadow_grid.h"
 
 using namespace hprt;
 
@@ -1810,4 +1811,27 @@
     return HPRT_OK;
 } catch (...) { return hprt::HandleException(); }
 
-}
+__attribute__((visibility("default"))) int hprt_debug_shadow_grid_build(size_t n, const float *p9, const float light[3], uint32_t R, double info6[6],
+                                                                         uint32_t *cell_start, size_t cell_cap, uint32_t *entries, size_t entry_cap) try {
+    if (!n || !p9 || !light || !info6 || R == 0 || n >= (1u << 28)) return SetError(HPRT_E_INVALID, "hprt_debug_shadow_grid_build: bad argument");
+    std::vector<float> tris(12 * n, 0.f);
+    std::vector<uint8_t> single(n, 1);
+    float lo[3] = {HPRT_INF, HPRT_INF, HPRT_INF}, hi[3] = {-HPRT_INF, -HPRT_INF, -HPRT_INF};
+    for (size_t i = 0; i < n; ++i)
+        for (int v = 0; v < 3; ++v)
+            for (int a = 0; a < 3; ++a) {
+                const float x = p9[9 * i + 3 * v + a];
+                tris[12 * i + 4 * v + a] = x;
+                if (x < lo[a]) lo[a] = x;
+                if (x > hi[a]) hi[a] = x;
+            }
+    ShadowGrid g;
+    BuildShadowGrid(tris.data(), single.data(), (uint32_t)n, light, lo, hi, R, (size_t)1 << 27, 0.0, &g);
+    if (!g.eligible) return SetError(HPRT_E_UNSUPPORTED, "hprt_debug_shadow_grid_build: the lists do not fit");
+    info6[0] = g.R; info6[1] = (double)g.entries.size(); info6[2] = g.nNear; info6[3] = g.eps; info6[4] = g.longest; info6[5] = g.buildSeconds;
+    if (cell_start && cell_cap >= g.cellStart.size()) memcpy(cell_start, g.cellStart.data(), 4 * g.cellStart.size());
+    if (entries && entry_cap >= g.entries.size()) memcpy(entries, g.entries.data(), 8 * g.entries.size());
+    return HPRT_OK;
+} catch (...) { return hprt::HandleException(); }
+
+}
diff --git a/thesis-pbrt-v3_amd/csrc/device/dev_intersect.h b/thesis-pbrt-v3_amd/csrc/device/dev_intersect.h
--- a/thesis-pbrt-v3_amd/csrc/device/dev_intersect.h
+++ b/thesis-pbrt-v3_amd/csrc/device/dev_intersect.h
@@ -76,6 +76,26 @@
     if (t <= deltaT) return false;
     *b0o = b0; *b1o = b1; *b2o = b2; *to = t;
     return true;
+}
+
+__device__ __forceinline__ bool slab_test(float lox, float hix, float loy, float hiy, float loz, float hiz, vec3 ro, vec3 invDir,
+                                          bool negX, bool negY, bool negZ, float robust, float *tEntry) {
+    float tMin = ((negX ? hix : lox) - ro.x) * invDir.x;
+    float tMax = ((negX ? lox : hix) - ro.x) * invDir.x;
+    const float tyMin = ((negY ? hiy : loy) - ro.y) * invDir.y;
+    float tyMax = ((negY ? loy : hiy) - ro.y) * invDir.y;
+    tMax *= robust; tyMax *= robust;
+    bool ok = !(tMin > tyMax || tyMin > tMax);
+    if (tyMin > tMin) tMin = tyMin;
+    if (tyMax < tMax) tMax = tyMax;
+    const float tzMin = ((negZ ? hiz : loz) - ro.z) * invDir.z;
+    float tzMax = ((negZ ? loz : hiz) - ro.z) * invDir.z;
+    tzMax *= robust;
+    ok = ok && !(tMin > tzMax || tzMin > tMax);
+    if (tzMin > tMin) tMin = tzMin;
+    if (tzMax < tMax) tMax = tzMax;
+    *tEntry = tMin;
+    return ok && (tMax > 0);
 }
 
 struct efloat { float v, lo, hi; };
diff --git a/thesis-pbrt-v3_amd/csrc/device/kernels.h b/thesis-pbrt-v3_amd/csrc/device/kernels.h
--- a/thesis-pbrt-v3_amd/csrc/device/kernels.h
+++ b/thesis-pbrt-v3_amd/csrc/device/kernels.h
@@ -73,6 +73,7 @@
 
 struct FilmRecord { uint32_t dest, srcTile; float xyz[3]; float w; };
 
+bool TraceProfileInUse();
 bool WideWalkInUse(const DevScene &sc);
 void LaunchTrace(hipStream_t st, const DevScene &sc, bool anyHit, bool count, const uint32_t *queue, const uint32_t *countPtr,
                  uint32_t countImm, uint32_t gridItems, const RayStream &rays, const HitStream &hits, uint8_t *occ,
diff --git a/thesis-pbrt-v3_amd/csrc/device/kernels.hip b/thesis-pbrt-v3_amd/csrc/device/kernels.hip
--- a/thesis-pbrt-v3_amd/csrc/device/kernels.hip
+++ b/thesis-pbrt-v3_amd/csrc/device/kernels.hip
@@ -72,26 +72,6 @@
     if (const char *e = getenv(anyHit ? "HPRT_TRACE_TUNE_ANY" : "HPRT_TRACE_TUNE"))
         sscanf(e, "%d,%d,%d,%d,%d", &t.refillBelow, &t.parkLimit, &t.stepLimit, &t.sphereLimit, &t.primMin);
     return t;
-}
-
-__device__ __forceinline__ bool slab_test(float lox, float hix, float loy, float hiy, float loz, float hiz, vec3 ro, vec3 invDir,
-                                          bool negX, bool negY, bool negZ, float robust, float *tEntry) {
-    float tMin = ((negX ? hix : lox) - ro.x) * invDir.x;
-    float tMax = ((negX ? lox : hix) - ro.x) * invDir.x;
-    const float tyMin = ((negY ? hiy : loy) - ro.y) * invDir.y;
-    float tyMax = ((negY ? loy : hiy) - ro.y) * invDir.y;
-    tMax *= robust; tyMax *= robust;
-    bool ok = !(tMin > tyMax || tyMin > tMax);
-    if (tyMin > tMin) tMin = tyMin;
-    if (tyMax < tMax) tMax = tyMax;
-    const float tzMin = ((negZ ? hiz : loz) - ro.z) * invDir.z;
-    float tzMax = ((negZ ? loz : hiz) - ro.z) * invDir.z;
-    tzMax *= robust;
-    ok = ok && !(tMin > tzMax || tzMin > tMax);
-    if (tzMin > tMin) tMin = tzMin;
-    if (tzMax < tMax) tMax = tzMax;
-    *tEntry = tMin;
-    return ok && (tMax > 0);
 }
 
 __device__ __forceinline__ void slab_test_pair(f32x2 nx, f32x2 fx, f32x2 ny, f32x2 fy, f32x2 nz, f32x2 fz, float rox, float roy, float roz,
@@ -1520,6 +1500,7 @@
 }
 extern "C" __attribute__((visibility("default"))) int hprt_debug_trace_profile_mode(int on) { const int was = TraceProfileEnabled() ? 1 : 0; g_traceProfileMode = on; return was; }
 bool WideWalkInUse(const DevScene &sc) { return sc.wide != nullptr && WideWalkEnabled(); }
+bool TraceProfileInUse() { return TraceProfileEnabled(); }
 extern "C" __attribute__((visibility("default"))) int hprt_debug_wide_walk(int on) { const int was = WideWalkEnabled() ? 1 : 0; g_wideWalk = on; return was; }
 void LaunchTrace(hipStream_t st, const DevScene &sc, bool anyHit, bool count, const uint32_t *queue, const uint32_t *countPtr,
                  uint32_t countImm, uint32_t gridItems, const RayStream &rays, const HitStream &hits, uint8_t *occ,
diff --git a/thesis-pbrt-v3_amd/csrc/device/shadow_grid.h b/thesis-pbrt-v3_amd/csrc/device/shadow_grid.h
--- /dev/null
+++ b/thesis-pbrt-v3_amd/csrc/device/shadow_grid.h
@@ -0,0 +1,11 @@
+#pragma once
+#include "kernels.h"
+
+namespace hprt {
+
+struct DevShadowGrid { const uint32_t *cellStart; const uint2 *entries; uint32_t nEntries, nNear, R; };
+
+void LaunchShadowGrid(hipStream_t st, const DevScene &sc, const DevShadowGrid &g, const uint32_t *queue, const uint32_t *countPtr,
+                      uint32_t countImm, uint32_t gridItems, const RayStream &rays, uint8_t *occ, uint32_t *workCounter);
+
+}
diff --git a/thesis-pbrt-v3_amd/csrc/device/shadow_grid.hip b/thesis-pbrt-v3_amd/csrc/device/shadow_grid.hip
--- /dev/null
+++ b/thesis-pbrt-v3_amd/csrc/device/shadow_grid.hip
@@ -0,0 +1,181 @@
+#include <hip/hip_runtime.h>
+#include <algorithm>
+#include <cstdlib>
+#include "shadow_grid.h"
+#include "dev_intersect.h"
+#include "../shadow_grid.h"
+
+namespace hprt {
+
+typedef unsigned int u32x4 __attribute__((ext_vector_type(4)));
+typedef unsigned int u32x2 __attribute__((ext_vector_type(2)));
+
+#ifndef HPRT_SHADOW_GRID_WAVES
+#define HPRT_SHADOW_GRID_WAVES 5
+#endif
+
+__device__ __forceinline__ uint32_t sg_cell(vec3 d, uint32_t R, float fineScale, uint32_t *sub) {
+    const float x = -d.x, y = -d.y, z = -d.z;
+    const float ax = fabsf(x), ay = fabsf(y), az = fabsf(z);
+    const bool a0 = ax >= ay && ax >= az, a1 = !a0 && ay >= az;
+    const float mj = a0 ? x : a1 ? y : z, a = a0 ? y : a1 ? z : x, b = a0 ? z : a1 ? x : y;
+    const float m = fabsf(mj);
+    const float u = a / m, v = b / m;
+    int fu = (int)floorf((u + 1.f) * fineScale), fv = (int)floorf((v + 1.f) * fineScale);
+    fu = sel_max(0, sel_min(16 * (int)R - 1, fu)); fv = sel_max(0, sel_min(16 * (int)R - 1, fv));
+    const uint32_t face = (a0 ? 0u : a1 ? 2u : 4u) + (mj < 0 ? 1u : 0u);
+    *sub = ((uint32_t)fu & 15u) | (((uint32_t)fv & 15u) << 4);
+    return (face * R + ((uint32_t)fv >> 4)) * R + ((uint32_t)fu >> 4);
+}
+__device__ __forceinline__ bool sg_reaches(uint32_t w, uint32_t sub) {
+    const uint32_t su = sub & 15u, sv = sub >> 4;
+    return su >= (w & 15u) && su <= ((w >> 4) & 15u) && sv >= ((w >> 8) & 15u) && sv <= ((w >> 12) & 15u);
+}
+
+enum : int { SG_IDLE = 0, SG_RAY = 1, SG_HEAD = 2, SG_FIRST = 3, SG_TEST = 4, SG_BOX = 5 };
+
+__global__ __launch_bounds__(HPRT_TRACE_BLOCK, HPRT_SHADOW_GRID_WAVES)
+void k_shadow_grid(DevScene sc, DevShadowGrid g, const uint32_t *queue, const uint32_t *countPtr, uint32_t countImm, RayStream rays, uint8_t *occ,
+                   uint32_t *workCounter, uint32_t chunk, uint32_t refillMin) {
+    const uint32_t n = countPtr ? *countPtr : countImm;
+    const uint32_t lane = __lane_id();
+    const auto triRsrc = __builtin_amdgcn_make_buffer_rsrc((void *)sc.tris, 0, (int)(sc.nPrims * 48u), 0x00020000);
+    const auto boxRsrc = __builtin_amdgcn_make_buffer_rsrc((void *)sc.leafBox, 0, (int)(sc.nPrims * 32u), 0x00020000);
+    const auto entRsrc = __builtin_amdgcn_make_buffer_rsrc((void *)g.entries, 0, (int)((g.nEntries + 1u) * 8u), 0x00020000);
+    const auto cellRsrc = __builtin_amdgcn_make_buffer_rsrc((void *)g.cellStart, 0, (int)((6u * g.R * g.R + 1u) * 4u), 0x00020000);
+    const float robust = 1 + 2 * gamma_n(3);
+    const float fineScale = 8.f * (float)g.R;
+    int st = SG_IDLE;
+    bool hit = false;
+    uint32_t slot = 0u;
+    uint32_t i = 0u, end = 0u, i2 = 0u, end2 = 0u;
+    uint32_t ePrim = 0u;
+    uint32_t sub = 0u;
+    vec3 ro, invDir;
+    float rayTMax = 0.f, lim = 0.f;
+    RayShear shear; shear.k0 = shear.k1 = false; shear.Sx = shear.Sy = shear.Sz = 0.f;
+    bool moreWork = n > 0;
+    uint32_t localNext = 0u, localEnd = 0u;
+    uint32_t window = 0u, windowBase = 0xffffffffu;
+    while (true) {
+        const unsigned long long idle = __ballot(st == SG_IDLE);
+        if (moreWork && ((uint32_t)__popcll(idle) >= refillMin || idle == ~0ull)) {
+            if (localNext >= localEnd) {
+                uint32_t base = 0u;
+                if (lane == 0) base = atomicAdd(workCounter, chunk);
+                base = __builtin_amdgcn_readfirstlane(base);
+                localNext = base < n ? base : n;
+                localEnd = (base + chunk < n) ? base + chunk : n;
+                if (localNext >= localEnd) moreWork = false;
+                windowBase = 0xffffffffu;
+            }
+            const uint32_t want = (uint32_t)__popcll(idle);
+            const uint32_t base = localNext;
+            localNext = (localNext + want < localEnd) ? localNext + want : localEnd;
+            const uint32_t rank = __builtin_amdgcn_mbcnt_hi((uint32_t)(idle >> 32), __builtin_amdgcn_mbcnt_lo((uint32_t)idle, 0u));
+            uint32_t slotW = 0u;
+            if (queue) {
+                if (windowBase != base) { window = (base + lane < localEnd) ? queue[base + lane] : 0u; windowBase = base; }
+                slotW = __shfl(window, (int)rank);
+                window = (localNext + lane < localEnd) ? queue[localNext + lane] : 0u;
+                windowBase = localNext;
+            }
+            if (st == SG_IDLE) {
+                const uint32_t idx = base + rank;
+                if (idx < localEnd) { slot = queue ? slotW : idx; hit = false; st = SG_RAY; }
+            }
+        }
+        if (__ballot(st != SG_IDLE) == 0ull) {
+            if (!moreWork) break;
+            continue;
+        }
+        u32x4 r0 = {0u, 0u, 0u, 0u}, r1 = {0u, 0u, 0u, 0u}, r2 = {0u, 0u, 0u, 0u};
+        u32x4 r3 = {0u, 0u, 0u, 0u};
+        const uint32_t pi = ePrim & SG_PRIM_MASK;
+        if (st == SG_TEST) {
+            r0 = __builtin_amdgcn_raw_buffer_load_b128(triRsrc, pi * 48u, 0, 0);
+            r1 = __builtin_amdgcn_raw_buffer_load_b128(triRsrc, pi * 48u + 16u, 0, 0);
+            r2 = __builtin_amdgcn_raw_buffer_load_b128(triRsrc, pi * 48u + 32u, 0, 0);
+            if (i + 1u < end) r3 = __builtin_amdgcn_raw_buffer_load_b128(entRsrc, (i + 1u) * 8u, 0, 0);
+        } else if (st == SG_RAY) {
+            r0 = __builtin_bit_cast(u32x4, rays.a[slot]);
+            r1 = __builtin_bit_cast(u32x4, rays.b[slot]);
+        } else if (st == SG_HEAD) {
+            const u32x2 h = __builtin_amdgcn_raw_buffer_load_b64(cellRsrc, i * 4u, 0, 0);
+            r3.x = h.x; r3.y = h.y;
+        } else if (st == SG_FIRST) {
+            r3 = __builtin_amdgcn_raw_buffer_load_b128(entRsrc, i * 8u, 0, 0);
+        } else if (st == SG_BOX) {
+            r0 = __builtin_amdgcn_raw_buffer_load_b128(boxRsrc, pi * 32u, 0, 0);
+            r1 = __builtin_amdgcn_raw_buffer_load_b128(boxRsrc, pi * 32u + 16u, 0, 0);
+        }
+        asm volatile("" : "+v"(r0), "+v"(r1), "+v"(r2), "+v"(r3));
+        auto leaf_reached = [&](float lx, float ly, float lz, float hx, float hy, float hz) -> bool {
+            float tEn;
+            return slab_test(lx, hx, ly, hy, lz, hz, ro, invDir, invDir.x < 0, invDir.y < 0, invDir.z < 0, robust, &tEn) && tEn < rayTMax;
+        };
+        bool done = false;
+        bool haveNext = false;
+        if (st == SG_RAY) {
+            ro = vec3(__uint_as_float(r0.x), __uint_as_float(r0.y), __uint_as_float(r0.z));
+            rayTMax = __uint_as_float(r0.w);
+            const vec3 d(__uint_as_float(r1.x), __uint_as_float(r1.y), __uint_as_float(r1.z));
+            invDir = vec3(1 / d.x, 1 / d.y, 1 / d.z);
+            shear = ray_shear(d, invDir);
+            const float dist2 = d.x * d.x + d.y * d.y + d.z * d.z;
+            lim = rayTMax <= 1.f ? dist2 * (1.f + 0x1p-20f) : HPRT_INF;
+            i = sg_cell(d, g.R, fineScale, &sub);
+            st = SG_HEAD;
+        } else if (st == SG_HEAD) {
+            if (g.nNear != 0u) { i = 0u; end = g.nNear; i2 = r3.x; end2 = r3.y; }
+            else { i = r3.x; end = r3.y; i2 = end2 = 0u; }
+            st = SG_FIRST;
+            if (i >= end) done = true;
+        } else if (st == SG_FIRST) {
+            haveNext = true;
+        } else if (st == SG_TEST) {
+            asm volatile("" : "+v"(r0), "+v"(r1), "+v"(r2));
+            const vec3 p0(__uint_as_float(r0.x), __uint_as_float(r0.y), __uint_as_float(r0.z)), p1(__uint_as_float(r1.x), __uint_as_float(r1.y), __uint_as_float(r1.z)),
+                       p2(__uint_as_float(r2.x), __uint_as_float(r2.y), __uint_as_float(r2.z));
+            float b0, b1, b2, t;
+            bool boxWanted = false;
+            if (tri_test(p0, p1, p2, ro, rayTMax, shear, &b0, &b1, &b2, &t)) {
+                if (ePrim & SG_SINGLE) {
+                    if (leaf_reached(fminf(fminf(p0.x, p1.x), p2.x), fminf(fminf(p0.y, p1.y), p2.y), fminf(fminf(p0.z, p1.z), p2.z),
+                                     fmaxf(fmaxf(p0.x, p1.x), p2.x), fmaxf(fmaxf(p0.y, p1.y), p2.y), fmaxf(fmaxf(p0.z, p1.z), p2.z))) { hit = true; done = true; }
+                } else boxWanted = true;
+            }
+            if (boxWanted) st = SG_BOX;
+            else if (!done) { ++i; haveNext = true; }
+        } else if (st == SG_BOX) {
+            if (leaf_reached(__uint_as_float(r0.x), __uint_as_float(r0.y), __uint_as_float(r0.z), __uint_as_float(r0.w), __uint_as_float(r1.x), __uint_as_float(r1.y))) { hit = true; done = true; }
+            else { ++i; st = SG_FIRST; if (i >= end) { i = i2; end = end2; i2 = end2 = 0u; if (i >= end) done = true; } }
+        }
+        if (haveNext) {
+            const bool in0 = i < end && !(__uint_as_float(r3.y & SG_KEY_MASK) > lim);
+            const bool in1 = in0 && i + 1u < end && !(__uint_as_float(r3.w & SG_KEY_MASK) > lim);
+            if (in0 && sg_reaches(r3.y, sub)) { ePrim = r3.x; st = SG_TEST; }
+            else if (in1 && sg_reaches(r3.w, sub)) { ePrim = r3.z; ++i; st = SG_TEST; }
+            else if (in1) { i += 2u; st = SG_FIRST; if (i >= end) { i = i2; end = end2; i2 = end2 = 0u; if (i >= end) done = true; } }
+            else { i = i2; end = end2; i2 = end2 = 0u; st = SG_FIRST; if (i >= end) done = true; }
+        }
+        if (done) { occ[slot] = hit ? 1 : 0; st = SG_IDLE; }
+    }
+}
+
+void LaunchShadowGrid(hipStream_t st, const DevScene &sc, const DevShadowGrid &g, const uint32_t *queue, const uint32_t *countPtr,
+                      uint32_t countImm, uint32_t gridItems, const RayStream &rays, uint8_t *occ, uint32_t *workCounter) {
+    if (gridItems == 0) return;
+    (void)hipMemsetAsync(workCounter, 0, sizeof(uint32_t), st);
+    static const uint32_t blockCap = [] { const char *e = getenv("HPRT_TRACE_MAX_BLOCKS"); return e ? (uint32_t)std::max(1, atoi(e)) : 0xffffffffu; }();
+    static const uint32_t perCu = [] { const char *e = getenv("HPRT_SHADOW_GRID_PER_CU"); return e ? (uint32_t)std::min((int)HPRT_SHADOW_GRID_WAVES, std::max(1, atoi(e))) : (uint32_t)HPRT_SHADOW_GRID_WAVES; }();
+    static const uint32_t chunkMax = [] { const char *e = getenv("HPRT_TRACE_CHUNK_MAX"); return e ? (uint32_t)atoi(e) : 512u; }();
+    static const uint32_t refillMin = [] { const char *e = getenv("HPRT_SHADOW_GRID_REFILL"); return e ? (uint32_t)std::min(64, std::max(1, atoi(e))) : 32u; }();
+    const uint32_t blocks = std::min((uint32_t)(((size_t)gridItems + HPRT_TRACE_BLOCK - 1) / HPRT_TRACE_BLOCK), std::min(256u * perCu, blockCap));
+    const uint32_t nWaves = blocks * (HPRT_TRACE_BLOCK / 64);
+    uint32_t chunk = gridItems / (nWaves * 4u);
+    chunk = std::max(64u, std::min(chunkMax, chunk)) & ~63u;
+    hipLaunchKernelGGL(k_shadow_grid, dim3(blocks), dim3(HPRT_TRACE_BLOCK), 0, st, sc, g, queue, countPtr, countImm, rays, occ, workCounter, chunk, refillMin);
+}
+
+}
diff --git a/thesis-pbrt-v3_amd/csrc/device_state.h b/thesis-pbrt-v3_amd/csrc/device_state.h
--- a/thesis-pbrt-v3_amd/csrc/device_state.h
+++ b/thesis-pbrt-v3_amd/csrc/device_state.h
@@ -14,6 +14,7 @@
 #include "device/kdinst_walk.h"
 #include "device/rbspinst_walk.h"
 #include "device/bsppaperinst_walk.h"
+#include "device/shadow_grid.h"
 #include "hprt_internal.h"
 
 #define HIP_TRY(expr)                                                                                   \
@@ -64,6 +65,8 @@
     hprt::DevBuf nodes, tris, primVtx, primN, vUV, vS, shapes, materials, lights, spheres, instances, topEntry, topEntryWide, lightFunc, lightCdf, perms, primes, primeSums, primeMagic;
     hprt::DevBuf envLights, envData;
     hprt::DevBuf wide, leafBox;
+    hprt::DevBuf sgCells, sgEntries; hprt::DevShadowGrid sg{};
+    struct ShadowGridInfo { uint32_t longest = 0; double buildSeconds = 0, eps = 0; size_t bytes = 0; float light[3] = {0, 0, 0}; uint64_t renderLaunches = 0; } sgInfo;
     hprt::DevBuf counters, workCounter, deepStack;
     struct Capture { int bounce = -1, kind = 0; float *out7 = nullptr; size_t cap = 0, n = 0; } capture;
     bool shadeCountsOn = false; uint64_t shadeDeferred = 0, shadeRetried = 0;
diff --git a/thesis-pbrt-v3_amd/csrc/scene_layout.cpp b/thesis-pbrt-v3_amd/csrc/scene_layout.cpp
--- a/thesis-pbrt-v3_amd/csrc/scene_layout.cpp
+++ b/thesis-pbrt-v3_amd/csrc/scene_layout.cpp
@@ -493,7 +493,7 @@
         if (g.nNodes == 0) continue;
         const BvhNode *nd = g.nodes;
         std::vector<int32_t> leafRefW(g.nNodes, WIDE_NONE);
-        if (L.leafBox.empty()) L.leafBox.assign(2 * (size_t)L.nPrims, make_float4(0.f, 0.f, 0.f, 0.f));
+        if (L.leafBox.empty()) { L.leafBox.assign(2 * (size_t)L.nPrims, make_float4(0.f, 0.f, 0.f, 0.f)); L.primSingle.assign(L.nPrims, 0); }
         for (uint32_t i = 0; i < g.nNodes; ++i) {
             if ((nd[i].countAxis & 3u) != 3u) continue;
             const uint32_t firstPrim = w.primBase[ai] + (uint32_t)nd[i].offset, count = nd[i].countAxis >> 2;
@@ -510,6 +510,7 @@
             }
             uint32_t r = ~firstPrim;
             if (!single) r &= ~WIDE_LEAF_BOXED;
+            else L.primSingle[firstPrim] = 1;
             leafRefW[i] = (int32_t)r;
             for (uint32_t k = 0; k < count; ++k) {
                 L.leafBox[2 * (size_t)(firstPrim + k)] = make_float4(nd[i].bmin[0], nd[i].bmin[1], nd[i].bmin[2], nd[i].bmax[0]);
@@ -521,7 +522,20 @@
         if (!BuildWide(nd, g.nNodes, leafRefW.data(), &L.wide, &need)) wideOk = false;
         if (ai == 0) wideNeedTop = need; else wideNeedObject = std::max(wideNeedObject, need);
     }
-    if (!wideOk || wideNeedTop + (w.d.n_instances ? 1 + wideNeedObject : 0) > HPRT_WIDE_STACK_MAX || w.wideBase[0] != 0) { L.wide.clear(); L.leafBox.clear(); }
+    if (!wideOk || wideNeedTop + (w.d.n_instances ? 1 + wideNeedObject : 0) > HPRT_WIDE_STACK_MAX || w.wideBase[0] != 0) { L.wide.clear(); L.leafBox.clear(); L.primSingle.clear(); }
+    return HPRT_OK;
+}
+
+int LayoutShadowGrid(Work &w) {
+    SceneLayout &L = w.L;
+    const int mode = ShadowGridModeFromEnv();
+    if (mode == 0 || w.d.n_lights != 1 || L.lights.size() != 1 || L.lights[0].type != 0 || w.d.n_instances != 0 || w.d.n_objects != 0 ||
+        !L.spheres.empty() || L.wide.empty() || L.nPrims == 0 || L.nPrims >= (1u << 28))
+        return HPRT_OK;
+    for (uint32_t i = 0; i < L.nPrims; ++i) if ((f2u(L.tris[3 * (size_t)i].w) & TAG_KIND_MASK) != 0u) return HPRT_OK;
+    static_assert(sizeof(float4) == 16, "triangle records are read as 12 floats per primitive");
+    const size_t capMb = [] { const char *e = getenv("HPRT_SHADOW_GRID_MAX_MB"); return e ? (size_t)std::max(1l, atol(e)) : (size_t)1024; }();
+    BuildShadowGrid(&L.tris[0].x, L.primSingle.data(), L.nPrims, L.lights[0].pos, L.wbMin, L.wbMax, ShadowGridResFromEnv(), capMb * ((1u << 20) / sizeof(SgEntry)), mode < 0 ? SG_MAX_CANDIDATES : 0.0, &L.shadowGrid);
     return HPRT_OK;
 }
 
@@ -576,7 +590,7 @@
     }
     for (uint32_t i = 0; i < d.n_instances; ++i) out->instanceObject.push_back(d.instances[i].object);
     for (int (*stage)(Work &) : {LayoutShapes, LayoutPrimitives, LayoutMaterials, LayoutTextures, LayoutLights, LayoutEnvLights,
-                                 LayoutLightDistribution, LayoutPairs, LayoutWide, LayoutInstances})
+                                 LayoutLightDistribution, LayoutPairs, LayoutWide, LayoutInstances, LayoutShadowGrid})
         if (int rc = stage(w)) return rc;
     return HPRT_OK;
 }
diff --git a/thesis-pbrt-v3_amd/csrc/scene_layout.h b/thesis-pbrt-v3_amd/csrc/scene_layout.h
--- a/thesis-pbrt-v3_amd/csrc/scene_layout.h
+++ b/thesis-pbrt-v3_amd/csrc/scene_layout.h
@@ -3,6 +3,7 @@
 #include <vector>
 #include "../../include/hprt.h"
 #include "device/dev_scene.h"
+#include "shadow_grid.h"
 
 namespace hprt {
 
@@ -34,6 +35,8 @@
     std::vector<uint32_t> objectPrimBase;
     std::vector<int32_t> instanceObject;
     bool instanced = false, hasSubstrateBin = false;
+    std::vector<uint8_t> primSingle;
+    ShadowGrid shadowGrid;
 };
 
 int BuildSceneLayout(const HprtSceneDesc &d, SceneLayout *out);
diff --git a/thesis-pbrt-v3_amd/csrc/shadow_grid.cpp b/thesis-pbrt-v3_amd/csrc/shadow_grid.cpp
--- /dev/null
+++ b/thesis-pbrt-v3_amd/csrc/shadow_grid.cpp
@@ -0,0 +1,151 @@
+#include "shadow_grid.h"
+#include <algorithm>
+#include <chrono>
+#include <cmath>
+#include <cstdlib>
+#include <cstring>
+
+namespace hprt {
+
+int ShadowGridModeFromEnv() { const char *e = getenv("HPRT_SHADOW_GRID"); return !e ? -1 : atoi(e) == 0 ? 0 : 1; }
+uint32_t ShadowGridResFromEnv() {
+    const char *e = getenv("HPRT_SHADOW_GRID_RES");
+    const long v = e ? atol(e) : (long)SG_DEFAULT_RES;
+    return (uint32_t)std::min(2048l, std::max(1l, v));
+}
+
+namespace {
+
+struct D3 { double x, y, z; };
+inline D3 operator-(D3 a, D3 b) { return {a.x - b.x, a.y - b.y, a.z - b.z}; }
+inline D3 operator+(D3 a, D3 b) { return {a.x + b.x, a.y + b.y, a.z + b.z}; }
+inline D3 operator*(D3 a, double s) { return {a.x * s, a.y * s, a.z * s}; }
+inline double dot(D3 a, D3 b) { return a.x * b.x + a.y * b.y + a.z * b.z; }
+inline D3 cross(D3 a, D3 b) { return {a.y * b.z - a.z * b.y, a.z * b.x - a.x * b.z, a.x * b.y - a.y * b.x}; }
+inline double comp(D3 a, int k) { return k == 0 ? a.x : k == 1 ? a.y : a.z; }
+
+double seg_dist2(D3 a, D3 b) {
+    const D3 ab = b - a;
+    const double l2 = dot(ab, ab);
+    double t = l2 > 0 ? -dot(a, ab) / l2 : 0.0;
+    t = std::min(1.0, std::max(0.0, t));
+    const D3 p = a + ab * t;
+    return dot(p, p);
+}
+double tri_dist2(D3 a, D3 b, D3 c) {
+    double best = std::min(seg_dist2(a, b), std::min(seg_dist2(b, c), seg_dist2(c, a)));
+    const D3 n = cross(b - a, c - a);
+    const double n2 = dot(n, n);
+    if (n2 > 0) {
+        const double s = dot(a, n) / n2;
+        const D3 q = n * s;
+        const double e0 = dot(cross(b - a, q - a), n), e1 = dot(cross(c - b, q - b), n), e2 = dot(cross(a - c, q - c), n);
+        if (e0 >= 0 && e1 >= 0 && e2 >= 0) best = std::min(best, dot(q, q));
+    }
+    return best;
+}
+
+bool face_rect(const D3 *poly, int n, int f, double lam, double r[4]) {
+    const int ax = f >> 1; const double sg = (f & 1) ? -1.0 : 1.0;
+    D3 out[8]; int no = 0;
+    for (int i = 0; i < n; ++i) {
+        const D3 p = poly[i], q = poly[(i + 1) % n];
+        const double mp = sg * comp(p, ax) - lam, mq = sg * comp(q, ax) - lam;
+        if (mp >= 0) out[no++] = p;
+        if ((mp >= 0) != (mq >= 0)) { const double t = mp / (mp - mq); out[no++] = p + (q - p) * t; }
+    }
+    if (no == 0) return false;
+    r[0] = r[2] = 1e300; r[1] = r[3] = -1e300;
+    for (int i = 0; i < no; ++i) {
+        const double m = std::max(sg * comp(out[i], ax), lam);
+        const double u = comp(out[i], (ax + 1) % 3) / m, v = comp(out[i], (ax + 2) % 3) / m;
+        r[0] = std::min(r[0], u); r[1] = std::max(r[1], u); r[2] = std::min(r[2], v); r[3] = std::max(r[3], v);
+    }
+    return true;
+}
+
+inline uint32_t f2u(float f) { uint32_t u; memcpy(&u, &f, 4); return u; }
+
+}
+
+void BuildShadowGrid(const float *tris, const uint8_t *single, uint32_t nPrims, const float light[3], const float bmin[3],
+                     const float bmax[3], uint32_t R, size_t maxEntries, double maxCandidates, ShadowGrid *out) {
+    const auto t0 = std::chrono::steady_clock::now();
+    ShadowGrid &g = *out;
+    g = ShadowGrid();
+    for (int a = 0; a < 3; ++a) g.light[a] = light[a];
+    double extent = 0;
+    for (int a = 0; a < 3; ++a) extent = std::max(extent, (double)std::max(bmax[a], light[a]) - (double)std::min(bmin[a], light[a]));
+    const double eps = SG_EPS_FACTOR * std::ldexp(1.0, -23) * extent;
+    g.eps = eps;
+    const D3 L = {light[0], light[1], light[2]};
+    std::vector<SgEntry> nearList;
+    struct Cover { uint32_t prim, key; double u0, u1, v0, v1; uint16_t face; };
+    std::vector<Cover> covers;
+    covers.reserve((size_t)nPrims * 2);
+    for (uint32_t i = 0; i < nPrims; ++i) {
+        const float *t = tris + 12 * (size_t)i;
+        const D3 v[3] = {D3{t[0], t[1], t[2]} - L, D3{t[4], t[5], t[6]} - L, D3{t[8], t[9], t[10]} - L};
+        const uint32_t word = i | ((single && single[i]) ? SG_SINGLE : 0u);
+        const D3 n = cross(v[1] - v[0], v[2] - v[0]);
+        const double d2 = tri_dist2(v[0], v[1], v[2]);
+        const double D = std::sqrt(d2) - eps;
+        const bool finite = std::isfinite(d2) && std::isfinite(dot(n, n));
+        const double margin = D > 0 ? 4.0 * eps / D + std::ldexp(1.0, -20) : 1e300;
+        if (!finite || dot(n, n) == 0 || !(D > 0) || margin > 0.5) { nearList.push_back({word, SG_RECT_ALL}); continue; }
+        float kf = (float)(D * D);
+        uint32_t kb = f2u(kf); kb = kb >= 2u ? kb - 2u : 0u;
+        const double lam = D / 4;
+        for (int f = 0; f < 6; ++f) {
+            double r[4];
+            if (!face_rect(v, 3, f, lam, r)) continue;
+            r[0] -= margin; r[1] += margin; r[2] -= margin; r[3] += margin;
+            if (r[1] < -1 || r[0] > 1 || r[3] < -1 || r[2] > 1) continue;
+            covers.push_back({word, kb, r[0], r[1], r[2], r[3], (uint16_t)f});
+        }
+    }
+    g.nNear = (uint32_t)nearList.size();
+    if (maxCandidates > 0 && (double)nearList.size() > maxCandidates) { g = ShadowGrid(); return; }
+    for (;; R = std::max(1u, R / 2)) {
+        const double fineScale = 8.0 * R;
+        auto fine = [&](double u) { const double c = std::floor((u + 1.0) * fineScale); return (uint32_t)std::min(16.0 * R - 1.0, std::max(0.0, c)); };
+        const size_t nCells = (size_t)6 * R * R;
+        std::vector<uint32_t> count(nCells + 1, 0u);
+        size_t total = 0;
+        bool over = false;
+        for (const Cover &c : covers) {
+            const uint32_t iu0 = fine(c.u0) >> 4, iu1 = fine(c.u1) >> 4, iv0 = fine(c.v0) >> 4, iv1 = fine(c.v1) >> 4;
+            total += (size_t)(iu1 - iu0 + 1) * (iv1 - iv0 + 1);
+            if (total > maxEntries) { over = true; break; }
+            for (uint32_t iv = iv0; iv <= iv1; ++iv) for (uint32_t iu = iu0; iu <= iu1; ++iu) ++count[((size_t)c.face * R + iv) * R + iu];
+        }
+        if (over && R > 1) continue;
+        if (over) { g = ShadowGrid(); return; }
+        if (maxCandidates > 0 && (double)nearList.size() + (double)total / (double)nCells > maxCandidates) { g = ShadowGrid(); return; }
+        g.R = R;
+        g.cellStart.assign(nCells + 1, 0u);
+        uint32_t at = g.nNear;
+        for (size_t c = 0; c < nCells; ++c) { g.cellStart[c] = at; at += count[c]; g.longest = std::max(g.longest, count[c]); }
+        g.cellStart[nCells] = at;
+        g.entries.resize(at);
+        std::copy(nearList.begin(), nearList.end(), g.entries.begin());
+        std::vector<uint32_t> fill(g.cellStart.begin(), g.cellStart.end() - 1);
+        for (const Cover &c : covers) {
+            const uint32_t fu0 = fine(c.u0), fu1 = fine(c.u1), fv0 = fine(c.v0), fv1 = fine(c.v1);
+            for (uint32_t iv = fv0 >> 4; iv <= fv1 >> 4; ++iv)
+                for (uint32_t iu = fu0 >> 4; iu <= fu1 >> 4; ++iu) {
+                    const uint32_t su0 = iu == fu0 >> 4 ? fu0 & 15u : 0u, su1 = iu == fu1 >> 4 ? fu1 & 15u : 15u;
+                    const uint32_t sv0 = iv == fv0 >> 4 ? fv0 & 15u : 0u, sv1 = iv == fv1 >> 4 ? fv1 & 15u : 15u;
+                    g.entries[fill[((size_t)c.face * R + iv) * R + iu]++] = {c.prim, (c.key & SG_KEY_MASK) | su0 | (su1 << 4) | (sv0 << 8) | (sv1 << 12)};
+                }
+        }
+        for (size_t c = 0; c < nCells; ++c)
+            std::sort(g.entries.begin() + g.cellStart[c], g.entries.begin() + g.cellStart[c + 1],
+                      [](const SgEntry &a, const SgEntry &b) { return (a.key & SG_KEY_MASK) != (b.key & SG_KEY_MASK) ? (a.key & SG_KEY_MASK) < (b.key & SG_KEY_MASK) : (a.prim & SG_PRIM_MASK) < (b.prim & SG_PRIM_MASK); });
+        break;
+    }
+    g.eligible = true;
+    g.buildSeconds = std::chrono::duration<double>(std::chrono::steady_clock::now() - t0).count();
+}
+
+}
diff --git a/thesis-pbrt-v3_amd/csrc/shadow_grid.h b/thesis-pbrt-v3_amd/csrc/shadow_grid.h
--- /dev/null
+++ b/thesis-pbrt-v3_amd/csrc/shadow_grid.h
@@ -0,0 +1,31 @@
+#pragma once
+#include <cstddef>
+#include <cstdint>
+#include <vector>
+
+namespace hprt {
+
+enum : uint32_t { SG_SINGLE = 0x80000000u, SG_PRIM_MASK = 0x0fffffffu, SG_KEY_MASK = 0xffff0000u, SG_RECT_ALL = 0xf0f0u };
+struct SgEntry { uint32_t prim, key; };
+constexpr double SG_EPS_FACTOR = 128.0;
+constexpr uint32_t SG_DEFAULT_RES = 512u;
+
+struct ShadowGrid {
+    bool eligible = false;
+    uint32_t R = 0;
+    float light[3] = {0, 0, 0};
+    std::vector<uint32_t> cellStart;
+    std::vector<SgEntry> entries;
+    uint32_t nNear = 0, longest = 0;
+    double eps = 0, buildSeconds = 0;
+    size_t bytes() const { return cellStart.size() * sizeof(uint32_t) + entries.size() * sizeof(SgEntry); }
+};
+
+void BuildShadowGrid(const float *tris, const uint8_t *single, uint32_t nPrims, const float light[3], const float bmin[3],
+                     const float bmax[3], uint32_t R, size_t maxEntries, double maxCandidates, ShadowGrid *out);
+
+int ShadowGridModeFromEnv();
+constexpr double SG_MAX_CANDIDATES = 14.0;
+uint32_t ShadowGridResFromEnv();
+
+}
```
